# Fastaxx/Penguin.jl

Hardware: AMD Instinct MI355X
Metric: time-steps/sec + SpMV GB/s (% HBM roofline), 3D mono diffusion 512^3 (higher is better)
Workload: dtype f64

## Files before the change

### penguin/jl_amd/csrc/pg_common.h

```cpp
#pragma once
#include <hip/hip_runtime.h>
#include "pg_rccl.h"

#include <chrono>
#include <cstdint>
#include <cstdio>
#include <cstring>
#include <stdexcept>
#include <string>
#include <vector>

#include "../../../include/penguin_hip.h"

namespace pg {

using i64 = int64_t;
using i32 = int32_t;

struct Error : std::runtime_error {
  using std::runtime_error::runtime_error;
};

void set_last_error(const std::string& msg);

#define PG_HIP(expr)                                                                              \
  do {                                                                                            \
    hipError_t _e = (expr);                                                                       \
    if (_e != hipSuccess)                                                                         \
      throw pg::Error(std::string("HIP error: ") + hipGetErrorString(_e) + " at " + __FILE__ + ":" + \
                      std::to_string(__LINE__) + " (" #expr ")");                                 \
  } while (0)

#define PG_NCCL(expr)                                                                             \
  do {                                                                                            \
    ncclResult_t _e = (expr);                                                                     \
    if (_e != ncclSuccess)                                                                        \
      throw pg::Error(std::string("RCCL error: ") + pg::rccl::api().GetErrorString(_e) + " at " + __FILE__ + ":" + \
                      std::to_string(__LINE__) + " (" #expr ")");                                 \
  } while (0)

#define PG_REQUIRE(cond, msg)                                   \
  do {                                                          \
    if (!(cond)) throw pg::Error(std::string(msg));             \
  } while (0)

#define PG_API_BEGIN try {
#define PG_API_END                                  \
  return 0;                                         \
  }                                                 \
  catch (const std::exception& e) {                 \
    pg::set_last_error(e.what());                   \
    return 1;                                       \
  }                                                 \
  catch (...) {                                     \
    pg::set_last_error("unknown exception");        \
    return 2;                                       \
  }

struct Config {
  bool debug = false;
  int alloc_poison = 0;
  int async_alloc = 0;
  int alloc_guard = 0;
  long long pool_limit_mb = 0;
  bool poly = true;
  int poly_degree = 6;
  bool poly_adapt = true;
  double poly_margin = 1.0;
  double poly_slack = -1.0;
  int poly_hist = 3;
  bool poly_trend = true;
  int poly_maxdeg = 0;
  int poly_mindeg = 4;
  bool poly_f32 = true;
  int poly_f32_tail = -1;
  int profile_sample = 3;
  bool gamma_elim = true;
  bool diag_elim = true;
  double diag_elim_frac = 0.0005;
  int spmv_variant = 70;
  int spmv_xcd = 1;
  int spmv_strip = 16;
  int spmv_march_k = 0;
  int spmv_minrun = 24;
  bool spmv_march = true;
  bool spmv_edges = true;
  int spmv_tile_units = 0;
  int spmv_blocks_per_cu = 0;
  bool halo_overlap = true;
  int guess_n = 4;
  int guess_depth = 7;
  bool guess_defer = true;
  bool guess_always = false;
  int guess_monitor = 256;
  double guess_pass_cost = 0.34;
  double guess_gain = 0.8;
  bool speculate_product = true;
  int mg_tail_rows = 2048;
  int unit_order = 0;
};
const Config& config();

struct LocalComm;

struct Context {
  bool inited = false;
  LocalComm* local = nullptr;
  int device = 0;
  hipStream_t stream = nullptr;
  hipStream_t comm_stream = nullptr;
  hipEvent_t ev_fork = nullptr, ev_join = nullptr;
  int rank = 0, nranks = 1;
  ncclComm_t comm = nullptr;
  ncclComm_t comm_halo = nullptr;
  bool profiling = false;
  std::string device_name;
};
Context& ctx();
void require_init();
void set_thread_context(Context* c);
Context* thread_context();
LocalComm* local_comm_create(int nranks);
void local_comm_destroy(LocalComm* c);
void comm_allreduce_sum_f64(double* dev, int count, hipStream_t st);
void comm_allreduce_max_f64(double* dev, int count, hipStream_t st);
void comm_allreduce_sum_u64(unsigned long long* dev, i64 count, hipStream_t st);

void* dev_alloc(size_t bytes);
void dev_free(void* p);
void dev_cache_release();
struct AsyncAllocScope {
  AsyncAllocScope();
  ~AsyncAllocScope();
};

template <class T>
struct DevBuf {
  T* p = nullptr;
  i64 n = 0;
  DevBuf() = default;
  explicit DevBuf(i64 n_) { alloc(n_); }
  DevBuf(const DevBuf&) = delete;
  DevBuf& operator=(const DevBuf&) = delete;
  DevBuf(DevBuf&& o) noexcept : p(o.p), n(o.n) { o.p = nullptr; o.n = 0; }
  DevBuf& operator=(DevBuf&& o) noexcept {
    if (this != &o) { release(); p = o.p; n = o.n; o.p = nullptr; o.n = 0; }
    return *this;
  }
  ~DevBuf() { release(); }
  void release() {
    if (p) dev_free(p);
    p = nullptr; n = 0;
  }
  void alloc(i64 n_) {
    release();
    n = n_;
    if (n > 0) p = static_cast<T*>(dev_alloc(sizeof(T) * static_cast<size_t>(n) + 64));
  }
  void zero() {
    if (n > 0) PG_HIP(hipMemsetAsync(p, 0, sizeof(T) * static_cast<size_t>(n), ctx().stream));
  }
  void upload(const T* h, i64 count, i64 offset = 0) {
    if (count > 0) {
      PG_HIP(hipMemcpyAsync(p + offset, h, sizeof(T) * static_cast<size_t>(count), hipMemcpyHostToDevice, ctx().stream));
      PG_HIP(hipStreamSynchronize(ctx().stream));
    }
  }
  void download(T* h, i64 count, i64 offset = 0) const {
    if (count > 0) {
      PG_HIP(hipMemcpyAsync(h, p + offset, sizeof(T) * static_cast<size_t>(count), hipMemcpyDeviceToHost, ctx().stream));
      PG_HIP(hipStreamSynchronize(ctx().stream));
    }
  }
};

inline void* pinned_scratch(int slot, size_t bytes) {
  static thread_local void* buf[2] = {nullptr, nullptr};
  static thread_local size_t cap[2] = {0, 0};
  if (bytes > cap[slot]) {
    if (buf[slot]) (void)hipHostFree(buf[slot]);
    PG_HIP(hipHostMalloc(&buf[slot], bytes + (bytes >> 2)));
    cap[slot] = bytes + (bytes >> 2);
  }
  return buf[slot];
}

struct Laps {
  bool on;
  std::chrono::steady_clock::time_point t0;
  explicit Laps() : on(config().debug), t0(std::chrono::steady_clock::now()) {}
  void lap(const char* what) {
    if (!on) return;
    (void)hipDeviceSynchronize();
    const auto t1 = std::chrono::steady_clock::now();
    fprintf(stderr, "[pg_laps] %-34s %8.2f ms\n", what, std::chrono::duration<double, std::milli>(t1 - t0).count());
    t0 = t1;
  }
};

struct EventPair {
  hipEvent_t e0 = nullptr, e1 = nullptr;
  EventPair() {
    PG_HIP(hipEventCreate(&e0));
    if (hipEventCreate(&e1) != hipSuccess) {
      (void)hipEventDestroy(e0);
      throw Error("hipEventCreate failed");
    }
  }
  ~EventPair() {
    if (e0) (void)hipEventDestroy(e0);
    if (e1) (void)hipEventDestroy(e1);
  }
  EventPair(const EventPair&) = delete;
  EventPair& operator=(const EventPair&) = delete;
};

inline int grid_for(i64 n, int block, int cap = 256 * 8) {
  i64 g = (n + block - 1) / block;
  if (g < 1) g = 1;
  if (g > cap) g = cap;
  return static_cast<int>(g);
}

constexpr int CAP_HALO = 3;

struct Slab {
  int N = 0;
  i64 n[3] = {1, 1, 1};
  i64 ext[3] = {1, 1, 1};
  i64 stride[3] = {1, 1, 1};
  i64 plane = 1;
  i64 nplanes = 1;
  i64 M = 1;
  i64 p0 = 0, p1 = 1;
  i64 s0 = 0, s1 = 1;
  i64 Mloc() const { return (s1 - s0) * plane; }
  i64 first_cell() const { return s0 * plane; }
  void set_own(i64 a, i64 b) {
    p0 = a; p1 = b;
    s0 = p0 - CAP_HALO; if (s0 < 0) s0 = 0;
    s1 = p1 + CAP_HALO; if (s1 > nplanes) s1 = nplanes;
  }
};

}

struct pg_mesh {
  int N = 0;
  pg::i64 n[3] = {1, 1, 1};
// ... 29 lines not shown
```

### penguin/jl_amd/csrc/pg_context.hip

```cpp
#include "pg_common.h"

#include <cxxabi.h>
#include <execinfo.h>

#include <atomic>
#include <map>
#include <mutex>
#include <unordered_map>
#include <unordered_set>
#include "pg_host_algos.h"

#include <algorithm>
#include <array>
#include <memory>
#include <set>

namespace pg {

static thread_local std::string g_last_error;
void set_last_error(const std::string& msg) { g_last_error = msg; }

Context& ctx() {
  static Context c;
  Context* t = thread_context();
  return t ? *t : c;
}

const Config& config() {
  static const Config c = [] {
    Config k;
    auto geti = [](const char* name, long long dflt) { const char* v = getenv(name); return v ? atoll(v) : dflt; };
    auto getd = [](const char* name, double dflt) { const char* v = getenv(name); return v ? atof(v) : dflt; };
    k.debug = getenv("PG_DEBUG") != nullptr;
    k.alloc_poison = (int)geti("PG_ALLOC_POISON", 0);
    k.async_alloc = (int)geti("PG_ASYNC_ALLOC", 0);
    k.alloc_guard = (int)geti("PG_ALLOC_GUARD", 0);
    k.pool_limit_mb = geti("PG_POOL_LIMIT_MB", 0);
    k.poly = geti("PG_POLY", 1) != 0;
    k.poly_degree = (int)geti("PG_POLY_DEGREE", 6);
    k.poly_adapt = geti("PG_POLY_ADAPT", getenv("PG_POLY_DEGREE") ? 0 : 1) != 0;
    k.poly_margin = getd("PG_POLY_MARGIN", 1.0);
    k.poly_slack = getd("PG_POLY_SLACK", -1.0);
    k.poly_hist = (int)std::max<long long>(1, std::min<long long>(3, geti("PG_POLY_HIST", 3)));
    k.poly_maxdeg = (int)geti("PG_POLY_MAXDEG", 0);
    k.poly_mindeg = (int)std::max<long long>(2, std::min<long long>(8, geti("PG_POLY_MINDEG", 4)));
    k.poly_trend = geti("PG_POLY_TREND", 1) != 0;
    k.poly_f32 = geti("PG_POLY_F32", 1) != 0;
    k.poly_f32_tail = (int)std::max<long long>(-1, std::min<long long>(64, geti("PG_POLY_F32_TAIL", -1)));
    k.profile_sample = (int)std::max<long long>(1, geti("PG_PROFILE_SAMPLE", 3));
    k.gamma_elim = geti("PG_GAMMA_ELIM", 1) != 0;
    k.diag_elim = geti("PG_DIAG_ELIM", 1) != 0;
    k.diag_elim_frac = getd("PG_DIAG_ELIM_FRAC", 0.0005);
    k.spmv_variant = (int)geti("PG_SPMV_VARIANT", 70);
    k.spmv_xcd = (int)geti("PG_SPMV_XCD", 1);
    k.spmv_strip = (int)geti("PG_SPMV_STRIP", 16);
    k.spmv_march_k = (int)geti("PG_SPMV_MARCH_K", 0);
    k.spmv_minrun = (int)geti("PG_SPMV_MINRUN", 24);
    k.spmv_march = geti("PG_SPMV_MARCH", 1) != 0;
    k.spmv_edges = geti("PG_SPMV_EDGES", 1) != 0;
    k.spmv_tile_units = (int)geti("PG_SPMV_TILE_UNITS", 0);
    k.spmv_blocks_per_cu = (int)geti("PG_SPMV_BLOCKS_PER_CU", 0);
    k.halo_overlap = geti("PG_HALO_OVERLAP", 1) != 0;
    k.speculate_product = geti("PG_SPECULATE", 1) != 0;
    k.guess_n = (int)std::max<long long>(0, std::min<long long>(4, geti("PG_GUESS_STATES", 4)));
    k.guess_depth = (int)std::max<long long>(1, std::min<long long>(7, geti("PG_GUESS_DEPTH", 7)));
    k.mg_tail_rows = (int)std::max<long long>(0, geti("PG_MG_TAIL_ROWS", 2048));
    k.guess_monitor = (int)std::max<long long>(1, geti("PG_GUESS_MONITOR", 256));
    k.guess_pass_cost = getd("PG_GUESS_PASS_COST", 0.34);
    k.guess_always = geti("PG_GUESS_ALWAYS", 0) != 0;
    k.guess_defer = geti("PG_GUESS_DEFER", 1) != 0;
    k.guess_gain = getd("PG_GUESS_GAIN", 0.8);
    k.unit_order = (int)geti("PG_SPMV_UNIT_ORDER", 0);
    return k;
  }();
  return c;
}

void require_init() {
  if (!ctx().inited)
    throw Error("penguin_hip: not initialised (call pg_init / pg_init_distributed first)");
}

static void init_device(int device_id) {
  Context& c = ctx();
  int ndev = 0;
  hipError_t e = hipGetDeviceCount(&ndev);
  if (e != hipSuccess || ndev <= 0)
    throw Error("penguin_hip: no HIP device visible -- this library has no CPU fallback");
  PG_REQUIRE(device_id >= 0 && device_id < ndev, "penguin_hip: device id out of range");
  PG_HIP(hipSetDevice(device_id));
  hipDeviceProp_t prop;
  PG_HIP(hipGetDeviceProperties(&prop, device_id));
  c.device = device_id;
  c.device_name = std::string(prop.name) + " (" + prop.gcnArchName + ")";
  if (!c.stream) PG_HIP(hipStreamCreateWithFlags(&c.stream, hipStreamNonBlocking));
  if (!c.comm_stream) PG_HIP(hipStreamCreateWithFlags(&c.comm_stream, hipStreamNonBlocking));
  c.inited = true;
}

}

using namespace pg;

namespace pg {
namespace {
thread_local int t_async_scope = 0;
std::mutex g_alloc_mutex;
struct BlockCache {
  std::multimap<size_t, void*> free_blocks;
  std::unordered_map<void*, size_t> owned;
  size_t free_bytes = 0;
};
BlockCache g_cache;
constexpr size_t CACHE_TRIM_BYTES = (size_t)48 << 30;

size_t round_block(size_t bytes) {
  const size_t q = bytes >= ((size_t)2 << 20) ? ((size_t)2 << 20) : 4096;
  return (bytes + q - 1) / q * q;
}

bool cache_wanted(const Context& c, size_t bytes) {
  const int mode = config().async_alloc;
  if (mode < 0 || !c.inited || !c.stream || c.local) return false;
  if (!(t_async_scope > 0 || mode > 0)) return false;
  const long long lim = config().pool_limit_mb;
  return lim <= 0 || bytes < ((size_t)lim << 20);
}

void poison(void* p, size_t bytes) {
  if (!config().alloc_poison || !p || bytes == 0) return;
  Context& c = ctx();
  if (c.inited && c.stream) PG_HIP(hipMemsetAsync(p, 0xFF, bytes, c.stream));
  else PG_HIP(hipMemset(p, 0xFF, bytes));
}

void cache_trim_locked() {
  if (g_cache.free_blocks.empty()) return;
  (void)hipDeviceSynchronize();
  for (auto& kv : g_cache.free_blocks) {
    g_cache.owned.erase(kv.second);
    (void)hipFree(kv.second);
  }
  g_cache.free_blocks.clear();
  g_cache.free_bytes = 0;
}

void* dev_alloc_raw(size_t bytes) {
  void* p = nullptr;
  Context& c = ctx();
  if (cache_wanted(c, bytes)) {
    const size_t want = round_block(bytes);
    {
      std::lock_guard<std::mutex> lk(g_alloc_mutex);
      auto it = g_cache.free_blocks.lower_bound(want);
      if (it != g_cache.free_blocks.end() && it->first <= want + want / 8) {
        p = it->second;
        g_cache.free_bytes -= it->first;
        g_cache.free_blocks.erase(it);
      }
    }
    if (!p) {
      if (hipMalloc(&p, want) != hipSuccess || !p) {
        (void)hipGetLastError();
        { std::lock_guard<std::mutex> lk(g_alloc_mutex); cache_trim_locked(); }
        PG_HIP(hipMalloc(&p, want));
      }
      std::lock_guard<std::mutex> lk(g_alloc_mutex);
      g_cache.owned[p] = want;
    }
    poison(p, bytes);
    return p;
  }
  PG_HIP(hipMalloc(&p, bytes));
  poison(p, bytes);
  return p;
}

void dev_free_raw(void* p) {
  if (!p) return;
  {
    std::lock_guard<std::mutex> lk(g_alloc_mutex);
    auto it = g_cache.owned.find(p);
    if (it != g_cache.owned.end()) {
      g_cache.free_blocks.emplace(it->second, p);
      g_cache.free_bytes += it->second;
      if (g_cache.free_bytes > CACHE_TRIM_BYTES) cache_trim_locked();
      return;
    }
  }
  (void)hipFree(p);
}

constexpr size_t GUARD = 4096;
struct GuardInfo { char* raw; size_t bytes; unsigned long long seq; std::string where; };
std::unordered_map<void*, GuardInfo> g_guarded;
unsigned long long g_alloc_seq = 0;
std::string call_stack() {
  void* frames[24];
  const int nf = backtrace(frames, 24);
  char** sym = backtrace_symbols(frames, nf);
  std::string s;
  for (int i = 2; sym && i < nf && i < 12; ++i) {
    std::string f = sym[i];
    const size_t a = f.find('('), b = f.find('+', a == std::string::npos ? 0 : a);
    if (a != std::string::npos && b != std::string::npos && b > a + 1) {
      std::string mangled = f.substr(a + 1, b - a - 1);
      int st = 0;
      char* dem = abi::__cxa_demangle(mangled.c_str(), nullptr, nullptr, &st);
      f = st == 0 && dem ? dem : mangled;
      free(dem);
      const size_t par = f.find('(');
      if (par != std::string::npos) f = f.substr(0, par);
    }
    s += (s.empty() ? "" : " <- ") + f;
  }
  free(sym);
  return s;
}
}

AsyncAllocScope::AsyncAllocScope() { ++t_async_scope; }
AsyncAllocScope::~AsyncAllocScope() { --t_async_scope; }

void dev_cache_release() {
  std::lock_guard<std::mutex> lk(g_alloc_mutex);
  cache_trim_locked();
}

void* dev_alloc(size_t bytes) {
  if (!config().alloc_guard) return dev_alloc_raw(bytes);
  char* raw = static_cast<char*>(dev_alloc_raw(bytes + 2 * GUARD));
  Context& c = ctx();
  hipStream_t st = (c.inited && c.stream) ? c.stream : nullptr;
  PG_HIP(hipMemsetAsync(raw, 0xA5, GUARD, st));
  PG_HIP(hipMemsetAsync(raw + GUARD + bytes, 0xA5, GUARD, st));
  void* user = raw + GUARD;
  std::lock_guard<std::mutex> lk(g_alloc_mutex);
  g_guarded[user] = GuardInfo{raw, bytes, ++g_alloc_seq, call_stack()};
  return user;
}

void dev_free(void* p) {
  if (!config().alloc_guard) { dev_free_raw(p); return; }
  GuardInfo gi;
  {
    std::lock_guard<std::mutex> lk(g_alloc_mutex);
    auto it = g_guarded.find(p);
    if (it == g_guarded.end()) { gi.raw = nullptr; }
    else { gi = it->second; g_guarded.erase(it); }
  }
  if (!gi.raw) { dev_free_raw(p); return; }
  (void)hipDeviceSynchronize();
  std::vector<unsigned char> lo(GUARD), hi(GUARD);
  (void)hipMemcpy(lo.data(), gi.raw, GUARD, hipMemcpyDeviceToHost);
  (void)hipMemcpy(hi.data(), gi.raw + GUARD + gi.bytes, GUARD, hipMemcpyDeviceToHost);
  auto first_bad = [](const std::vector<unsigned char>& g, bool from_end) -> long {
    if (from_end) { for (long i = (long)g.size() - 1; i >= 0; --i) if (g[i] != 0xA5) return i; }
    else { for (size_t i = 0; i < g.size(); ++i) if (g[i] != 0xA5) return (long)i; }
    return -1;
  };
  const long bl = first_bad(lo, true), bh = first_bad(hi, false);
  if (bl >= 0 || bh >= 0) {
    long nl = 0, nh = 0;
    for (unsigned char v : lo) nl += v != 0xA5;
    for (unsigned char v : hi) nh += v != 0xA5;
    fprintf(stderr, "[pg_alloc] GUARD DAMAGED: block #%llu of %zu bytes (incl. 64 of slack): %ld bytes written BELOW it (nearest %ld bytes "
            "before the start), %ld bytes written ABOVE it (first %ld bytes past the end); allocated by: %s\n", gi.seq, gi.bytes, nl,
            bl >= 0 ? (long)GUARD - bl : 0, nh, bh >= 0 ? bh : 0, gi.where.c_str());
  }
  dev_free_raw(gi.raw);
}
}

extern "C" {

int32_t pg_last_error(char* buf, size_t n) {
  if (buf && n > 0) {
    std::strncpy(buf, g_last_error.c_str(), n - 1);
    buf[n - 1] = 0;
  }
  return 0;
}

int32_t pg_init(int32_t device_id) {
  PG_API_BEGIN
  Context& c = ctx();
  init_device(device_id);
  c.rank = 0;
  c.nranks = 1;
  PG_API_END
}

int32_t pg_get_unique_id(void* out128) {
  PG_API_BEGIN
  static_assert(sizeof(ncclUniqueId) == 128, "ncclUniqueId is expected to be 128 bytes");
  ncclUniqueId id;
  PG_NCCL(rccl::api().GetUniqueId(&id));
  std::memcpy(out128, &id, sizeof(id));
  PG_API_END
}

int32_t pg_init_distributed(int32_t device_id, int32_t rank, int32_t nranks, const void* unique_id128) {
  PG_API_BEGIN
  Context& c = ctx();
  PG_REQUIRE(nranks >= 1 && rank >= 0 && rank < nranks, "pg_init_distributed: bad rank / nranks");
  init_device(device_id);
  c.rank = rank;
  c.nranks = nranks;
  if (nranks > 1 || unique_id128 != nullptr) {
    PG_REQUIRE(unique_id128 != nullptr, "pg_init_distributed: unique id required when nranks > 1");
    ncclUniqueId id;
    std::memcpy(&id, unique_id128, sizeof(id));
    const rccl::Api& R = rccl::api();
    PG_NCCL(R.CommInitRank(&c.comm, nranks, id, rank));
    bool split_ok = false;
    if (R.CommSplit) {
      split_ok = R.CommSplit(c.comm, 0, rank, &c.comm_halo, nullptr) == ncclSuccess && c.comm_halo != nullptr;
      if (!split_ok) c.comm_halo = nullptr;
    }
    if (!split_ok) {
      ncclUniqueId id2;
      if (rank == 0) PG_NCCL(R.GetUniqueId(&id2));
      DevBuf<char> buf((i64)sizeof(id2));
      if (rank == 0) buf.upload(reinterpret_cast<const char*>(&id2), (i64)sizeof(id2));
      PG_NCCL(R.Broadcast(buf.p, buf.p, sizeof(id2), ncclChar, 0, c.comm, c.stream));
      buf.download(reinterpret_cast<char*>(&id2), (i64)sizeof(id2));
      PG_NCCL(R.CommInitRank(&c.comm_halo, nranks, id2, rank));
    }
  }
  PG_API_END
}

int32_t pg_finalize(void) {
  PG_API_BEGIN
  Context& c = ctx();
  if (c.inited) {
    (void)hipDeviceSynchronize();
    if (c.comm_halo) { (void)rccl::api().CommDestroy(c.comm_halo); c.comm_halo = nullptr; }
    if (c.comm) { (void)rccl::api().CommDestroy(c.comm); c.comm = nullptr; }
    dev_cache_release();
    if (c.stream) { (void)hipStreamDestroy(c.stream); c.stream = nullptr; }
    if (c.comm_stream) { (void)hipStreamDestroy(c.comm_stream); c.comm_stream = nullptr; }
    if (c.ev_fork) { (void)hipEventDestroy(c.ev_fork); c.ev_fork = nullptr; }
    if (c.ev_join) { (void)hipEventDestroy(c.ev_join); c.ev_join = nullptr; }
    c.inited = false;
  }
  PG_API_END
}

int32_t pg_device_synchronize(void) {
  PG_API_BEGIN
  require_init();
  PG_HIP(hipDeviceSynchronize());
  PG_API_END
}

int32_t pg_set_profiling(int32_t on) {
  PG_API_BEGIN
  ctx().profiling = on != 0;
  PG_API_END
}

int32_t pg_config_string(char* buf, size_t n) {
  PG_API_BEGIN
  const Config& k = config();
  char tmp[1024];
  snprintf(tmp, sizeof(tmp),
           "spmv_variant=%d spmv_xcd=%d spmv_strip=%d spmv_unit_order=%d spmv_march=%d spmv_edges=%d spmv_march_k=%d spmv_minrun=%d spmv_tile_units=%d "
           "spmv_blocks_per_cu=%d halo_overlap=%d speculate=%d poly=%d poly_degree=%d poly_adapt=%d "
           "poly_margin=%g poly_slack=%g poly_hist=%d poly_trend=%d poly_maxdeg=%d poly_f32=%d poly_f32_tail=%d gamma_elim=%d diag_elim=%d "
           "guess_states=%d guess_depth=%d guess_defer=%d async_alloc=%d cache_limit_mb=%lld alloc_poison=%d alloc_guard=%d profile_sample=%d debug=%d",
           k.spmv_variant, k.spmv_xcd, k.spmv_strip, k.unit_order, (int)k.spmv_march, (int)k.spmv_edges, k.spmv_march_k, k.spmv_minrun, k.spmv_tile_units,
           k.spmv_blocks_per_cu, (int)k.halo_overlap, (int)k.speculate_product, (int)k.poly, k.poly_degree, (int)k.poly_adapt,
           k.poly_margin, k.poly_slack, k.poly_hist, (int)k.poly_trend, k.poly_maxdeg, (int)k.poly_f32, k.poly_f32_tail,
           (int)k.gamma_elim, (int)k.diag_elim, k.guess_n, k.guess_depth, (int)k.guess_defer, k.async_alloc, k.pool_limit_mb, k.alloc_poison, k.alloc_guard, k.profile_sample, (int)k.debug);
  if (buf && n > 0) {
    std::strncpy(buf, tmp, n - 1);
    buf[n - 1] = 0;
  }
  PG_API_END
}

int32_t pg_device_name(char* buf, size_t n) {
  PG_API_BEGIN
  require_init();
  if (buf && n > 0) {
    std::strncpy(buf, ctx().device_name.c_str(), n - 1);
    buf[n - 1] = 0;
  }
  PG_API_END
}

int32_t pg_mesh_create(int32_t N, const int64_t* n, const double* L, const double* x0, pg_mesh** out) {
  PG_API_BEGIN
  PG_REQUIRE(N >= 1 && N <= 3, "pg_mesh_create: N must be 1, 2 or 3");
  PG_REQUIRE(out != nullptr, "pg_mesh_create: out is NULL");
  PG_REQUIRE(n != nullptr && L != nullptr, "pg_mesh_create: n / L is NULL");
  std::unique_ptr<pg_mesh> guard(new pg_mesh());
  pg_mesh* m = guard.get();
  m->N = N;
  for (int d = 0; d < N; ++d) {
    PG_REQUIRE(n[d] >= 1, "pg_mesh_create: n_d must be >= 1");
    m->n[d] = n[d];
    m->L[d] = L[d];
    m->x0[d] = x0 ? x0[d] : 0.0;
    const double h = L[d] / static_cast<double>(n[d]);
    m->centers[d].resize(n[d]);
    m->nodes[d].resize(n[d] + 1);
    for (i64 j = 0; j < n[d]; ++j) m->centers[d][j] = m->x0[d] + static_cast<double>(j) * h;
    for (i64 j = 0; j <= n[d]; ++j) m->nodes[d][j] = m->x0[d] + (static_cast<double>(j) + 0.5) * h;
  }
  if (ctx().inited) {
    for (int d = 0; d < N; ++d) {
      m->d_nodes[d].alloc(n[d] + 1);
      m->d_nodes[d].upload(m->nodes[d].data(), n[d] + 1);
    }
  }
  *out = guard.release();
  PG_API_END
}

int32_t pg_mesh_destroy(pg_mesh* m) {
  PG_API_BEGIN
  delete m;
  PG_API_END
}

int32_t pg_mesh_get_centers(const pg_mesh* m, int32_t d, double* out, int64_t len) {
  PG_API_BEGIN
  PG_REQUIRE(m && d >= 0 && d < m->N && len == m->n[d], "pg_mesh_get_centers: bad arguments");
  std::memcpy(out, m->centers[d].data(), sizeof(double) * len);
  PG_API_END
}

int32_t pg_mesh_get_nodes(const pg_mesh* m, int32_t d, double* out, int64_t len) {
  PG_API_BEGIN
  PG_REQUIRE(m && d >= 0 && d < m->N && len == m->n[d] + 1, "pg_mesh_get_nodes: bad arguments");
  std::memcpy(out, m->nodes[d].data(), sizeof(double) * len);
  PG_API_END
}

int32_t pg_mesh_num_border_cells(const pg_mesh* m, int64_t* out) {
  PG_API_BEGIN
  PG_REQUIRE(m && out, "pg_mesh_num_border_cells: bad arguments");
  i64 all = 1, inner = 1;
  for (int d = 0; d < m->N; ++d) {
    all *= m->n[d];
    inner *= std::max<i64>(m->n[d] - 2, 0);
  }
  *out = all - inner;
  PG_API_END
}

int32_t pg_mesh_get_border_cells(const pg_mesh* mc, int64_t* idx, double* pos, int32_t* key) {
  PG_API_BEGIN
  PG_REQUIRE(mc, "pg_mesh_get_border_cells: mesh is NULL");
  pg_mesh* m = const_cast<pg_mesh*>(mc);
  mesh_build_border(m);
  const size_t nb = m->border_key.size();
  if (idx) std::memcpy(idx, m->border_idx.data(), sizeof(i64) * nb * m->N);
  if (pos) std::memcpy(pos, m->border_pos.data(), sizeof(double) * nb * m->N);
  if (key) std::memcpy(key, m->border_key.data(), sizeof(i32) * nb);
  PG_API_END
}

int32_t pg_partition_planes(const int64_t* weight, int64_t nplanes, int32_t nranks, int64_t* bounds) {
  PG_API_BEGIN
  PG_REQUIRE(weight && bounds && nplanes >= 1 && nranks >= 1, "pg_partition_planes: bad arguments");
  PG_REQUIRE(nplanes >= nranks, "pg_partition_planes: fewer planes than ranks");
  pghost::partition_planes(weight, nplanes, nranks, bounds);
  PG_API_END
}

int32_t pg_slab_numbering_host(int32_t K, int64_t plane, int64_t nplanes, int64_t p0, int64_t p1, const uint8_t* active,
                               int64_t* out) {
  PG_API_BEGIN
  PG_REQUIRE(K >= 1 && K <= pghost::SLAB_MAX_KINDS && plane >= 1 && nplanes >= 1 && p0 >= 0 && p1 > p0 && p1 <= nplanes && active && out,
             "pg_slab_numbering_host: bad arguments");
  const pghost::SlabPlanes g = pghost::slab_planes(p0, p1, nplanes, CAP_HALO);
  const i64 Mloc = (g.s1 - g.s0) * plane;
  const i64 lcA0 = (g.a0 - g.s0) * plane, lcA1 = (g.a1 - g.s0) * plane;
  const i64 lcO = (p0 - g.s0) * plane, lcU = (p1 - g.s0) * plane, lcFE = (p0 + 1 - g.s0) * plane, lcLB = (p1 - 1 - g.s0) * plane;
  i64 posO[pghost::SLAB_MAX_KINDS], posU[pghost::SLAB_MAX_KINDS], posFE[pghost::SLAB_MAX_KINDS], posLB[pghost::SLAB_MAX_KINDS],
      tot[pghost::SLAB_MAX_KINDS];
  for (int k = 0; k < K; ++k) {
    i64 c = 0;
    posO[k] = posU[k] = posFE[k] = posLB[k] = -1;
    for (i64 lc = 0; lc <= Mloc; ++lc) {
      if (lc == lcO) posO[k] = c;
      if (lc == lcU) posU[k] = c;
      if (lc == lcFE) posFE[k] = c;
      if (lc == lcLB) posLB[k] = c;
      if (lc < Mloc && lc >= lcA0 && lc < lcA1 && active[(i64)k * Mloc + lc]) ++c;
    }
    tot[k] = c;
  }
  pghost::SlabNumbering sn;
  pghost::slab_numbering(K, posO, posU, posFE, posLB, tot, p0 > 0, p1 < nplanes, sn);
  i64 q = 0;
  out[q++] = sn.n_own;
  out[q++] = sn.n_ghost;
  const i64* arrays[10] = {sn.cnt_own, sn.off_own, sn.cntL, sn.offL, sn.cntU, sn.offU, sn.sendL_off, sn.sendL_cnt, sn.sendU_off, sn.sendU_cnt};
  for (const i64* a : arrays)
    for (int k = 0; k < K; ++k) out[q++] = a[k];
  PG_API_END
}

}

namespace pg {

void mesh_build_border(pg_mesh* m) {
  if (m->border_built) return;
  const int N = m->N;
  std::vector<i64>& bi = m->border_idx;
  std::set<std::array<i64, 3>> seen;
  auto emit = [&](i64 i0, i64 i1, i64 i2) {
    std::array<i64, 3> key{i0, i1, i2};
    if (!seen.insert(key).second) return;
    const i64 id[3] = {i0, i1, i2};
    for (int d = 0; d < N; ++d) {
      bi.push_back(id[d] + 1);
      m->border_pos.push_back(m->centers[d][id[d]]);
    }
    m->border_key.push_back(border_key_of(N, m->n, i0, i1, i2));
  };
  for (int d = 0; d < N; ++d) {
    const i64 faces[2] = {0, m->n[d] - 1};
// ... 32 lines not shown
```

### penguin/jl_amd/csrc/pg_precond.hip

```cpp
#include "pg_scan.h"
#include "pg_system.h"

using namespace pg;

namespace {

struct RowSegs {
  int K;
  i64 off_own[MAX_KINDS];
};

__device__ inline int row_kind_of(const RowSegs& s, i64 r) {
  int k = 0;
  while (k + 1 < s.K && r >= s.off_own[k + 1]) ++k;
  return k;
}

constexpr int NSLOT = 7;

__device__ inline int slot_of(const CapView& c, i64 lc, i64 cl) {
  if (cl == lc) return 0;
  for (int d = 0; d < c.N; ++d) {
    if (cl == lc + c.stride[d]) return 1 + 2 * d;
    if (cl == lc - c.stride[d]) return 2 + 2 * d;
// ... 164 lines not shown
    for (int a = 0; a < MAX_KINDS; ++a) {
      blk_idx[q * MAX_KINDS + a] = a < cb.nk ? cb.rows[a] : -1;
      blk_coef[q * MAX_KINDS + a] = a < cb.nk ? cb.binv[me][a] * cb.dsk[a] : 0.0;
      blk_fw[q * MAX_KINDS + a] = a < cb.nk ? cb.bfw[me][a] : 0.0;
      double cn = 0.0;
      if (a < cb.nk) {
        if (P.nphase == 1) cn = a == me ? 1.0 : 0.0;
        else
          for (int j = 0; j < cb.nk; ++j)
            if ((cb.kinds[j] & 1) == 0) cn += cb.binv[me][j] * cb.bfw[j][a];
      }
      blk_cn[q * MAX_KINDS + a] = cn;
    }
  }
}

__global__ void k_count_ghost_refs(i64 nnz, i64 n_own, const int* __restrict__ col, unsigned long long* __restrict__ out) {
  unsigned long long c = 0;
  for (i64 k = blockIdx.x * (i64)blockDim.x + threadIdx.x; k < nnz; k += (i64)gridDim.x * blockDim.x) c += col[k] >= n_own ? 1 : 0;
  if (c) atomicAdd(out, c);
}

__global__ void k_gershgorin(i64 n, const int* __restrict__ rowptr, const int* __restrict__ col,
                             const double* __restrict__ val, const double* __restrict__ ds, double* __restrict__ out) {
  double worst = 0.0;
  for (i64 r = blockIdx.x * (i64)blockDim.x + threadIdx.x; r < n; r += (i64)gridDim.x * blockDim.x) {
    const int a = rowptr[r], b = rowptr[r + 1];
    if (b - a <= 1) {
      const double d = b > a && col[a] == r ? fabs(1.0 - val[a]) : 1.0;
      worst = d > worst ? d : worst;
      continue;
    }
    double diag = 0.0, off = 0.0;
    for (int k = a; k < b; ++k) {
      const int c = col[k];
      if (c == r) { diag = val[k]; continue; }
      if (c < n && rowptr[c + 1] - rowptr[c] == 1 && col[rowptr[c]] == c) continue;
      off += fabs(val[k]) * (ds[r] / ds[c]);
    }
    const double rad = fabs(1.0 - diag) + off;
    worst = rad > worst ? rad : worst;
  }
  for (int o = 32; o > 0; o >>= 1) {
    const double other = __shfl_down(worst, o, 64);
    worst = other > worst ? other : worst;
  }
  if ((threadIdx.x & 63) == 0)
    atomicMax(reinterpret_cast<unsigned long long*>(out), (unsigned long long)__double_as_longlong(worst));
}

__global__ void k_pl_simple(i64 n, const double* __restrict__ ds, const double* __restrict__ in, double* __restrict__ out) {
  for (i64 r = blockIdx.x * (i64)blockDim.x + threadIdx.x; r < n; r += (i64)gridDim.x * blockDim.x) out[r] = ds[r] * in[r];
}

__global__ void k_pl_block(i64 nblk, const int* __restrict__ blk_rows, const int* __restrict__ blk_idx,
                           const double* __restrict__ blk_coef, const double* __restrict__ in, double* __restrict__ out) {
  for (i64 q = blockIdx.x * (i64)blockDim.x + threadIdx.x; q < nblk; q += (i64)gridDim.x * blockDim.x) {
    double s = 0.0;
#pragma unroll
    for (int a = 0; a < MAX_KINDS; ++a) {
      const int j = blk_idx[q * MAX_KINDS + a];
      if (j >= 0) s += blk_coef[q * MAX_KINDS + a] * in[j];
    }
    out[blk_rows[q]] = s;
  }
}

__global__ void k_point_scale(SysParams P, int K, i64 Mloc, const int* red, double* ds) {
  const CapView& c = P.cap[0];
  const i64 total = (i64)K * Mloc;
  for (i64 q = blockIdx.x * (i64)blockDim.x + threadIdx.x; q < total; q += (i64)gridDim.x * blockDim.x) {
    const int r = red[q];
    if (r < 0) continue;
    const int k = (int)(q / Mloc);
    const i64 lc = q % Mloc;
    i64 idx[3];
    decode_cell(c.N, c.ext, c.plane, c.s0, lc, idx);
    double diag = 0.0, rowmax = 0.0;
    eval_row(P, k, lc, idx, [&](int ck, i64 cl, double v) {
      if (ck == k && cl == lc) diag = v;
      rowmax = fmax(rowmax, fabs(v));
    });
    const double a = fabs(diag);
    ds[r] = (a > 1e-13 * rowmax && a < 1e300) ? 1.0 / sqrt(a) : 1.0;
  }
}

}

namespace pg {

static void set_geo(CsrMatrix& A, const Slab& slab, const Numbering& nb) {
  A.geo_cell = nb.row_cell.p;
  A.geo_map = nullptr;
  A.geo_ext0 = slab.N == 3 ? slab.ext[0] : 0;
  A.geo_lines = slab.N == 3 ? slab.ext[1] : 0;
}

void assemble_csr_preconditioned(const SysParams& P, const Slab& s, const Numbering& nb, CsrMatrix& A,
                                 const bool* inherit_halo) {
  hipStream_t st = ctx().stream;
  Laps laps;
  const i64 n = nb.n_own;
  A.n = n;
  A.rowptr.alloc(n + 1);
  A.ds.alloc(nb.n_vec() > 0 ? nb.n_vec() : 1);
  A.n_blk = 0;
  A.halo_needed = true;
  RowSegs seg;
  seg.K = nb.K;
  for (int k = 0; k < MAX_KINDS; ++k) seg.off_own[k] = nb.off_own[k];
  if (n == 0) {
    A.rowptr.zero();
    A.nnz = 0;
    if (inherit_halo) A.halo_needed = *inherit_halo;
    else if (ctx().nranks > 1) {
      DevBuf<unsigned long long> nref(1);
      nref.zero();
      comm_allreduce_sum_u64(nref.p, 1, st);
      unsigned long long h = 0;
      nref.download(&h, 1);
      A.halo_needed = h != 0;
    }
    decide_poly(A);
    return;
  }
  hipLaunchKernelGGL(k_point_scale, dim3(grid_for((i64)nb.K * nb.Mloc, 256, 256 * 16)), dim3(256), 0, st, P, nb.K, nb.Mloc,
                     nb.red.p, A.ds.p);
  PG_HIP(hipGetLastError());
  DevBuf<int> cnt(n);
  A.isblk.alloc(n);
  DevBuf<unsigned char>& isblk = A.isblk;
  DevBuf<unsigned long long> nraw(1);
  nraw.zero();
  const int gr = grid_for(n, 256, 256 * 16);
  hipLaunchKernelGGL(HIP_KERNEL_NAME(k_asm_p<false>), dim3(gr), dim3(256), 0, st, P, seg, nb.Mloc, n, nb.row_cell.p, nb.red.p,
                     A.ds.p, cnt.p, isblk.p, nraw.p, (const int*)nullptr, (int*)nullptr, (double*)nullptr);
  PG_HIP(hipGetLastError());
  scan_exclusive<int>(cnt.p, A.rowptr.p, n, A.rowptr.p + n, st);
  int nnz = 0;
  A.rowptr.download(&nnz, 1, n);
  PG_REQUIRE(nnz >= 0, "nnz overflow");
  A.nnz = nnz;
  unsigned long long hraw = 0;
  nraw.download(&hraw, 1);
  A.nnz_raw = (i64)hraw;
  A.col.alloc(nnz + 8);
  A.val.alloc(nnz + 8);
  A.col.zero();
  A.val.zero();
  hipLaunchKernelGGL(HIP_KERNEL_NAME(k_asm_p<true>), dim3(gr), dim3(256), 0, st, P, seg, nb.Mloc, n, nb.row_cell.p, nb.red.p,
                     A.ds.p, (int*)nullptr, (unsigned char*)nullptr, (unsigned long long*)nullptr, (const int*)A.rowptr.p, A.col.p, A.val.p);
  PG_HIP(hipGetLastError());
  DevBuf<int> pos(n), total(1);
  scan_exclusive<unsigned char>(isblk.p, pos.p, n, total.p, st);
  int nblk = 0;
  total.download(&nblk, 1);
  A.n_blk = nblk;
  A.blk_rows.alloc(nblk > 0 ? nblk : 1);
  A.blk_idx.alloc((i64)MAX_KINDS * (nblk > 0 ? nblk : 1));
  A.blk_coef.alloc((i64)MAX_KINDS * (nblk > 0 ? nblk : 1));
  A.blk_cn.alloc((i64)MAX_KINDS * (nblk > 0 ? nblk : 1));
  A.blk_fw.alloc((i64)MAX_KINDS * (nblk > 0 ? nblk : 1));
  if (nblk > 0) {
    hipLaunchKernelGGL(k_blk_table, dim3(gr), dim3(256), 0, st, P, seg, nb.Mloc, n, nb.row_cell.p, nb.red.p, A.ds.p, isblk.p,
                       pos.p, A.blk_rows.p, A.blk_idx.p, A.blk_coef.p, A.blk_cn.p, A.blk_fw.p);
    PG_HIP(hipGetLastError());
  }
  PG_HIP(hipStreamSynchronize(st));
  if (inherit_halo) A.halo_needed = *inherit_halo;
  else if (ctx().nranks > 1) {
    DevBuf<unsigned long long> nref(1);
    nref.zero();
    hipLaunchKernelGGL(k_count_ghost_refs, dim3(grid_for(nnz, 256, 4096)), dim3(256), 0, st, (i64)nnz, n, A.col.p, nref.p);
    PG_HIP(hipGetLastError());
    comm_allreduce_sum_u64(nref.p, 1, st);
    unsigned long long h = 0;
    nref.download(&h, 1);
    A.halo_needed = h != 0;
    if (config().debug)
      fprintf(stderr, "[pg_precond] rank %d: %llu ghost-column references over all ranks => halo %s\n", ctx().rank, h,
              A.halo_needed ? "exchanged" : "skipped");
  }
  laps.lap("  asm: count/fill/table kernels");
  set_geo(A, s, nb);
  build_spmv_chunks(A);
  laps.lap("  asm: SpMV chunks + slices");
  decide_poly(A);
}

__global__ void k_structure_differs(i64 n, const int* __restrict__ cnt, const int* __restrict__ rowptr,
                                    const unsigned char* __restrict__ blk_a, const unsigned char* __restrict__ blk_b,
                                    unsigned long long* __restrict__ out) {
  unsigned long long c = 0;
  for (i64 r = blockIdx.x * (i64)blockDim.x + threadIdx.x; r < n; r += (i64)gridDim.x * blockDim.x)
    c += (cnt[r] != rowptr[r + 1] - rowptr[r] || blk_a[r] != blk_b[r]) ? 1 : 0;
  if (c) atomicAdd(out, c);
}

void assemble_csr_like(const SysParams& P, const Slab& s, const Numbering& nb, const CsrMatrix& T, CsrMatrix& A) {
  hipStream_t st = ctx().stream;
  Laps laps;
  const i64 n = nb.n_own;
  const bool halo = T.halo_needed;
  if (n == 0 || T.n != n || !T.rowptr.p) {
    assemble_csr_preconditioned(P, s, nb, A, &halo);
    return;
  }
  RowSegs seg;
  seg.K = nb.K;
  for (int k = 0; k < MAX_KINDS; ++k) seg.off_own[k] = nb.off_own[k];
  A.n = n;
  A.ds.alloc(nb.n_vec() > 0 ? nb.n_vec() : 1);
  hipLaunchKernelGGL(k_point_scale, dim3(grid_for((i64)nb.K * nb.Mloc, 256, 256 * 16)), dim3(256), 0, st, P, nb.K, nb.Mloc,
                     nb.red.p, A.ds.p);
  PG_HIP(hipGetLastError());
  DevBuf<int> cnt(n);
  A.isblk.alloc(n);
  DevBuf<unsigned long long> nraw(2);
  nraw.zero();
  const int gr = grid_for(n, 256, 256 * 16);
  hipLaunchKernelGGL(HIP_KERNEL_NAME(k_asm_p<false>), dim3(gr), dim3(256), 0, st, P, seg, nb.Mloc, n, nb.row_cell.p, nb.red.p,
                     A.ds.p, cnt.p, A.isblk.p, nraw.p, (const int*)nullptr, (int*)nullptr, (double*)nullptr);
  hipLaunchKernelGGL(k_structure_differs, dim3(grid_for(n, 256, 4096)), dim3(256), 0, st, n, cnt.p, T.rowptr.p, A.isblk.p,
                     T.isblk.p, nraw.p + 1);
  PG_HIP(hipGetLastError());
  unsigned long long h[2] = {0, 0};
  nraw.download(h, 2);
  if (h[1] != 0) {
    assemble_csr_preconditioned(P, s, nb, A, &halo);
    return;
  }
  A.nnz = T.nnz;
  A.nnz_raw = (i64)h[0];
  A.halo_needed = halo;
  A.rowptr.alloc(n + 1);
  PG_HIP(hipMemcpyAsync(A.rowptr.p, T.rowptr.p, sizeof(int) * (n + 1), hipMemcpyDeviceToDevice, st));
  A.col.alloc(A.nnz + 8);
  A.val.alloc(A.nnz + 8);
  A.col.zero();
  A.val.zero();
  hipLaunchKernelGGL(HIP_KERNEL_NAME(k_asm_p<true>), dim3(gr), dim3(256), 0, st, P, seg, nb.Mloc, n, nb.row_cell.p, nb.red.p,
                     A.ds.p, (int*)nullptr, (unsigned char*)nullptr, (unsigned long long*)nullptr, (const int*)A.rowptr.p, A.col.p, A.val.p);
  PG_HIP(hipGetLastError());
  const i64 nblk = T.n_blk, nb1 = nblk > 0 ? nblk : 1;
  A.n_blk = nblk;
  A.blk_rows.alloc(nb1);
  A.blk_idx.alloc((i64)MAX_KINDS * nb1);
  A.blk_coef.alloc((i64)MAX_KINDS * nb1);
  A.blk_cn.alloc((i64)MAX_KINDS * nb1);
  A.blk_fw.alloc((i64)MAX_KINDS * nb1);
  if (nblk > 0) {
    DevBuf<int> pos(n), total(1);
    scan_exclusive<unsigned char>(A.isblk.p, pos.p, n, total.p, st);
    hipLaunchKernelGGL(k_blk_table, dim3(gr), dim3(256), 0, st, P, seg, nb.Mloc, n, nb.row_cell.p, nb.red.p, A.ds.p, A.isblk.p,
                       pos.p, A.blk_rows.p, A.blk_idx.p, A.blk_coef.p, A.blk_cn.p, A.blk_fw.p);
    PG_HIP(hipGetLastError());
    PG_HIP(hipStreamSynchronize(st));
  }
  laps.lap("  asm-like: values on the ctor matrix' pattern");
  set_geo(A, s, nb);
  if (!build_slices_like(T, A)) build_spmv_chunks(A);
  laps.lap("  asm-like: slices");
  decide_poly(A);
}

void decide_poly(CsrMatrix& A) {
  hipStream_t st = ctx().stream;
  DevBuf<double> worst(1);
  worst.zero();
  if (A.n > 0) {
    hipLaunchKernelGGL(k_gershgorin, dim3(grid_for(A.n, 256, 4096)), dim3(256), 0, st, A.n, A.rowptr.p, A.col.p, A.val.p, A.ds.p,
                       worst.p);
    PG_HIP(hipGetLastError());
  }
  comm_allreduce_max_f64(worst.p, 1, st);
  double h = 0.0;
  worst.download(&h, 1);
  A.gersh = h;
  A.est = SpecEst();
  A.poly_gave_up = false;
  A.poly_ok = h < 0.95;
  if (config().debug && !(h < 1e300) && A.n > 0) {
    std::vector<int> rp(A.n + 1), cl(A.nnz);
    std::vector<double> vl(A.nnz), dsv(A.ds.n);
    A.rowptr.download(rp.data(), A.n + 1); A.col.download(cl.data(), A.nnz); A.val.download(vl.data(), A.nnz);
    A.ds.download(dsv.data(), A.ds.n);
    int shown = 0;
    for (i64 r = 0; r < A.n && shown < 4; ++r) {
      bool bad = !(dsv[r] > 0.0) || !(dsv[r] < 1e300);
      for (int k = rp[r]; k < rp[r + 1]; ++k) bad = bad || !(std::fabs(vl[k]) < 1e300);
      if (!bad) continue;
      ++shown;
      fprintf(stderr, "[pg_precond] row %lld: ds %.3e entries", (long long)r, dsv[r]);
      for (int k = rp[r]; k < rp[r + 1]; ++k) fprintf(stderr, " (%d: %.3e, ds %.3e)", cl[k], vl[k], dsv[cl[k]]);
      fprintf(stderr, "\n");
    }
  }
  if (config().debug)
    fprintf(stderr, "[pg_precond] rank %d: largest Gershgorin radius %.4f => Neumann preconditioner %s\n", ctx().rank, h,
            A.poly_ok ? "admissible" : "not used");
}

void apply_left(const CsrMatrix& A, const double* in, double* out, hipStream_t st) {
  if (A.n == 0) return;
  hipLaunchKernelGGL(k_pl_simple, dim3(grid_for(A.n, 256)), dim3(256), 0, st, A.n, A.ds.p, in, out);
  if (A.n_blk > 0)
    hipLaunchKernelGGL(k_pl_block, dim3(grid_for(A.n_blk, 256)), dim3(256), 0, st, A.n_blk, A.blk_rows.p, A.blk_idx.p,
                       A.blk_coef.p, in, out);
  PG_HIP(hipGetLastError());
}

}
```

### penguin/jl_amd/csrc/pg_solver.hip

```cpp
#include <algorithm>
#include <cmath>
#include <memory>

#include "pg_krylov.h"
#include "pg_reduce.h"
#include "pg_multigrid.h"
#include "pg_program.h"
#include "pg_scan.h"
#include "pg_solver_internal.h"
#include "pg_spmv.h"
#include "pg_specest.h"

using namespace pg;

namespace pg { extern double g_host_wait_us; }

struct pg_solver {
  int nphase = 1;
  pg_capacity* cap[2] = {nullptr, nullptr};
  pg_diffops* ops[2] = {nullptr, nullptr};
  Slab slab;
  int K = 2;
  i64 Mloc = 0, M = 0;
  double dt = 0.0, t = 0.0;
  int scheme_ctor = PG_SCHEME_BE;
  pg_bc_desc bc_i{};
  pg_jump_desc ic{};
  int border_kind[6] = {0, 0, 0, 0, 0, 0};
  double border_value[6] = {0, 0, 0, 0, 0, 0};
  double inv_dx = 0.0;
  DevBuf<double> Id[2];
  DevBuf<double> f_n[2], f_np1[2];
  DevBuf<double> g_n, g_np1;
  DevBuf<double> g_arr, h_arr;
  Numbering nb;
  CsrMatrix A_ctor, A_run;
  GammaElim elim_ctor, elim_run;
  DiagElim diag_ctor, diag_run;
  bool have_run = false;
  int scheme_run = -1;
  DevBuf<double> mass, bconst, bcv;
  DevBuf<unsigned char> fixed;
  int bconst_scheme = -1;
  bool bconst_dirty = true;
  long long bconst_version = 0;
  struct TdSlot {
    int K = 0;
    i64 nrows = 0;
    DevBuf<double> mode[PG_TD_MAX_TERMS];
    std::vector<double> coef;
    struct Prog {
      pg_program prog;
      int key = -1;
      i64 n = 0;
      DevBuf<int> row;
      DevBuf<double> w, p[3];
      i64 nrows = 0;
      std::vector<double> times;
    };
    std::vector<Prog> progs;
    bool empty() const { return K == 0 && progs.empty(); }
  };
  TdSlot td[4];
  DevBuf<double> td_base;
  int td_base_scheme = -1;
  i64 td_cursor = 0;
  i64 td_row = -1;
  DevBuf<double> blk_wz, blk_c0;
  const CsrMatrix* blk_cache_matrix = nullptr;
  int blk_cache_scheme = -1;
  long long blk_cache_version = -1;
  DevBuf<double> x, b, y;
  DevBuf<double> z, ysol;
  bool x_valid = true;
  const CsrMatrix* z_matrix = nullptr;
  DevBuf<double> T0pad;
  KrylovWork work;
  MgHierarchy mg;
  MgHierarchy mg_cell;
  bool spec_y_valid = false, spec_pending = false, hint_more_steps = false;
  const CsrMatrix* spec_matrix = nullptr;
  DevBuf<double> zh[8], yh[8], guess_coef, guess_partials;
  DevBuf<unsigned> guess_ticket;
  int hist_cnt = 0, hist_k = 0;
  bool plain_guess_on[2] = {false, false};
  double plain_last_products[2] = {0.0, 0.0};
  const void* hist_de = nullptr;
  bool initial_done = false;
  std::vector<DevBuf<double>> states;
  i64 steps_done = 0;
  DevBuf<double> red_scratch;
  DevBuf<i64> border_cells_lin;
  bool moving = false;
  DevBuf<double> psi_p[2], psi_m[2];
  bool advdiff = false;
  bool convection = false;
  DevBuf<double> psi_cp[2], psi_cm[2];
  bool stefan = false;
  bool solved_once = false;
  pg_solver* init_from = nullptr;
  struct Monitors {
    int K = 0;
    int kind[PG_MON_MAX] = {};
    bool sparse[PG_MON_MAX] = {};
    i64 stored[PG_MON_MAX] = {};
    DevBuf<double> w[PG_MON_MAX];
    DevBuf<int> row[PG_MON_MAX];
    int G = 0;
    DevBuf<double> series;
    i64 rows = 0, cap = 0;
    std::vector<double> times;
  };
  Monitors mon;
  MgHierarchy mg_step[2];
};

namespace {

using pg::BLOCK;

struct RowSegs {
  int K;
  i64 off_own[MAX_KINDS];
};

__device__ inline int seg_kind(const RowSegs& s, i64 r) {
  int k = 0;
  while (k + 1 < s.K && r >= s.off_own[k + 1]) ++k;
  return k;
}

RowSegs make_segs(const Numbering& nb) {
  RowSegs s;
  s.K = nb.K;
  for (int k = 0; k < MAX_KINDS; ++k) s.off_own[k] = nb.off_own[k];
  return s;
}

struct KeyVals {
  double v[6];
};

__global__ void k_row_static(SysParams P, RowSegs seg, i64 n_own, const int* row_cell, KeyVals kv, double* mass,
                             unsigned char* fixed, double* bcv) {
  const CapView& c = P.cap[0];
  for (i64 r = blockIdx.x * (i64)blockDim.x + threadIdx.x; r < n_own; r += (i64)gridDim.x * blockDim.x) {
    const int k = seg_kind(seg, r);
    const i64 lc = row_cell[r];
    i64 idx[3];
    decode_cell(c.N, c.ext, c.plane, c.s0, lc, idx);
    double m = 0.0, bv = 0.0;
    unsigned char fx = 0;
    if ((k & 1) == 0) {
      const int ph = k >> 1;
      int key = -1;
      const int bk = border_row_kind(P, ph, lc, idx, &key);
      if (bk != PG_BC_NONE) {
        fx = 1;
        bv = (bk == PG_BC_PERIODIC) ? 0.0 : kv.v[key];
      } else {
        m = P.mv_psi_w[0] ? P.mv_v1[ph][lc] : P.mass * P.cap[ph].V[lc];
      }
    } else if (P.nphase == 2) {
      fx = 1;
    }
    mass[r] = m;
    fixed[r] = fx;
    bcv[r] = bv;
  }
}

struct SrcView {
  const double* f_n[2];
  const double* f_np1[2];
  const double* g_n;
  const double* g_np1;
  double g_const, h_const;
};

__global__ void k_bconst(SysParams P, RowSegs seg, i64 n_own, const int* row_cell, SrcView s, int scheme, double dt,
                         const unsigned char* fixed, const double* bcv, double* bconst, int moving) {
  for (i64 r = blockIdx.x * (i64)blockDim.x + threadIdx.x; r < n_own; r += (i64)gridDim.x * blockDim.x) {
    const int k = seg_kind(seg, r);
    const i64 lc = row_cell[r];
    const int ph = k >> 1;
    double v;
    if ((k & 1) == 0) {
      if (fixed[r]) v = bcv[r];
      else {
        const double V = P.cap[ph].V[lc];
        const double f1 = s.f_np1[ph] ? s.f_np1[ph][lc] : 0.0;
        if (scheme == PG_SCHEME_CN) {
          const double f0 = s.f_n[ph] ? s.f_n[ph][lc] : f1;
          v = dt / 2 * V * (f0 + f1);
        } else {
          v = dt * V * f1;
        }
      }
    } else if (P.nphase == 1) {
      const double G = P.cap[0].G[lc];
      const double g1 = s.g_np1 ? s.g_np1[lc] : s.g_const;
      if (scheme == PG_SCHEME_CN && !moving) {
        const double g0 = s.g_n ? s.g_n[lc] : s.g_const;
        v = dt / 2 * G * (g0 + g1);
      } else {
        v = G * g1;
      }
    } else if (k == 1 || P.mv_stefan) {
      v = s.g_n ? s.g_n[lc] : s.g_const;
    } else {
      v = P.cap[1].G[lc] * (s.g_np1 ? s.g_np1[lc] : s.h_const);
    }
    bconst[r] = v;
  }
}

__global__ void k_rhs(i64 n, int scheme, const double* __restrict__ x, const double* __restrict__ yhat,
                      const double* __restrict__ ds, const double* __restrict__ mass, const double* __restrict__ bconst,
                      const unsigned char* __restrict__ fixed, double* __restrict__ b) {
  for (i64 r = blockIdx.x * (i64)blockDim.x + threadIdx.x; r < n; r += (i64)gridDim.x * blockDim.x) {
    double v;
    if (fixed[r]) v = ds[r] * bconst[r];
    else if (scheme == PG_SCHEME_CN) v = ds[r] * (2.0 * (mass[r] * x[r]) + bconst[r]) - yhat[r];
    else v = ds[r] * (mass[r] * x[r] + bconst[r]);
    b[r] = v;
  }
}

__global__ void k_rhs_block(i64 nblk, int scheme, const int* __restrict__ blk_rows, const int* __restrict__ blk_idx,
                            const double* __restrict__ blk_coef, const double* __restrict__ blk_cn,
                            const double* __restrict__ x, const double* __restrict__ ds, const double* __restrict__ yhat,
                            const double* __restrict__ mass, const double* __restrict__ bconst,
                            const unsigned char* __restrict__ fixed, double* __restrict__ b) {
  const double fac = scheme == PG_SCHEME_CN ? 2.0 : 1.0;
  for (i64 q = blockIdx.x * (i64)blockDim.x + threadIdx.x; q < nblk; q += (i64)gridDim.x * blockDim.x) {
    double v = 0.0;
#pragma unroll
    for (int a = 0; a < MAX_KINDS; ++a) {
      const int j = blk_idx[q * MAX_KINDS + a];
      if (j < 0) continue;
      const double xj = ds ? ds[j] * x[j] : x[j];
      const double cj = fixed[j] ? bconst[j] : fac * (mass[j] * xj) + bconst[j];
      v += blk_coef[q * MAX_KINDS + a] * cj;
      if (scheme == PG_SCHEME_CN) v -= blk_cn[q * MAX_KINDS + a] * yhat[j];
    }
    b[blk_rows[q]] = v;
  }
}

__global__ void k_blk_cache(i64 nblk, int scheme, const int* __restrict__ blk_idx, const double* __restrict__ blk_coef,
                            const double* __restrict__ ds, const double* __restrict__ mass, const double* __restrict__ bconst,
                            const unsigned char* __restrict__ fixed, double* __restrict__ wz, double* __restrict__ c0) {
  const double fac = scheme == PG_SCHEME_CN ? 2.0 : 1.0;
  for (i64 q = blockIdx.x * (i64)blockDim.x + threadIdx.x; q < nblk; q += (i64)gridDim.x * blockDim.x) {
    double c = 0.0;
#pragma unroll
    for (int a = 0; a < MAX_KINDS; ++a) {
      const int j = blk_idx[q * MAX_KINDS + a];
      double w = 0.0;
      if (j >= 0) {
        const double cf = blk_coef[q * MAX_KINDS + a];
        c += cf * bconst[j];
        if (!fixed[j]) w = cf * (fac * (mass[j] * ds[j]));
      }
      wz[q * MAX_KINDS + a] = w;
    }
    c0[q] = c;
  }
}

__global__ void k_rhs_block_c(i64 nblk, int scheme, const int* __restrict__ blk_rows, const int* __restrict__ blk_idx,
                              const double* __restrict__ wz, const double* __restrict__ c0, const double* __restrict__ blk_cn,
                              const double* __restrict__ z, const double* __restrict__ yhat, double* __restrict__ b) {
  for (i64 q = blockIdx.x * (i64)blockDim.x + threadIdx.x; q < nblk; q += (i64)gridDim.x * blockDim.x) {
    int j[MAX_KINDS];
    double zz[MAX_KINDS], yy[MAX_KINDS];
#pragma unroll
    for (int a = 0; a < MAX_KINDS; ++a) j[a] = blk_idx[q * MAX_KINDS + a];
#pragma unroll
    for (int a = 0; a < MAX_KINDS; ++a) {
      zz[a] = j[a] >= 0 ? z[j[a]] : 0.0;
      yy[a] = (j[a] >= 0 && scheme == PG_SCHEME_CN) ? yhat[j[a]] : 0.0;
    }
    double v = c0[q];
#pragma unroll
    for (int a = 0; a < MAX_KINDS; ++a) v += wz[q * MAX_KINDS + a] * zz[a] - (scheme == PG_SCHEME_CN ? blk_cn[q * MAX_KINDS + a] * yy[a] : 0.0);
    b[blk_rows[q]] = v;
  }
}

__global__ void k_rhs_block_mf(SysParams P, RowSegs seg, i64 Mloc, i64 nblk, const int* __restrict__ blk_rows,
                               const int* __restrict__ blk_idx, const double* __restrict__ blk_coef,
                               const int* __restrict__ row_cell, const int* __restrict__ red, const double* __restrict__ ds,
                               const double* __restrict__ z, const double* __restrict__ mass, const double* __restrict__ bconst,
                               const unsigned char* __restrict__ fixed, double* __restrict__ b) {
  const CapView& c = P.cap[0];
  for (i64 q = blockIdx.x * (i64)blockDim.x + threadIdx.x; q < nblk; q += (i64)gridDim.x * blockDim.x) {
    const i64 lc = row_cell[blk_rows[q]];
    i64 idx[3];
    decode_cell(c.N, c.ext, c.plane, c.s0, lc, idx);
    double v = 0.0;
    for (int a = 0; a < MAX_KINDS; ++a) {
      const int j = blk_idx[q * MAX_KINDS + a];
      if (j < 0) continue;
      const int k = seg_kind(seg, j);
      double ca;
      if (fixed[j]) {
        ca = bconst[j];
      } else {
        double ax = 0.0;
        eval_row(P, k, lc, idx, [&](int ck, i64 cl, double val) {
          const int col = red[(i64)ck * Mloc + cl];
          if (val != 0.0 && col >= 0) ax += val * (ds[col] * z[col]);
        });
        ca = 2.0 * (mass[j] * (ds[j] * z[j])) + bconst[j] - ax;
      }
      v += blk_coef[q * MAX_KINDS + a] * ca;
    }
    b[blk_rows[q]] = v;
  }
}

struct GuessArgs {
  const double* zr[8];
  const double* yr[8];
  double* znew;
  double* coef;
  int defer;
};
constexpr int GUESS_USED = 64;

__device__ inline const double* ring_pick(const double* const (&r)[8], int i) {
  const double* p = r[0];
#pragma unroll
  for (int q = 1; q < 8; ++q) p = i == q ? r[q] : p;
  return p;
}

typedef double rd2_t __attribute__((ext_vector_type(2)));
typedef unsigned char ruc2_t __attribute__((ext_vector_type(2)));

__device__ inline void rhs_init_one(int scheme, double z, double yh, double d, double ms, double bc, bool fx, bool blk, double bold,
                                    double& bi, double& ri) {
  if (blk) bi = bold;
  else if (fx) bi = d * bc;
  else if (scheme == PG_SCHEME_CN) bi = d * (2.0 * (ms * (d * z)) + bc) - yh;
  else bi = d * (ms * (d * z) + bc);
  ri = bi - yh;
}

template <int KH>
__global__ __launch_bounds__(BLOCK) void k_rhs_init(i64 n, i64 nvec, int scheme, const double* __restrict__ z,
                                                    const double* __restrict__ yhat, const double* __restrict__ ds,
                                                    const double* __restrict__ mass, const double* __restrict__ bconst,
                                                    const unsigned char* __restrict__ fixed,
                                                    const unsigned char* __restrict__ isblk, double* __restrict__ b,
                                                    double* __restrict__ r, double* __restrict__ rhat,
                                                    double* __restrict__ p, double* __restrict__ partials, GuessArgs g) {
  __shared__ double s_red[BLOCK / 64];
  double acc = 0.0, accb = 0.0, accw = 0.0;
  double cj[KH > 0 ? KH : 1];
  const double* zo[KH > 0 ? KH : 1];
  const double* yo[KH > 0 ? KH : 1];
  int ku = 0;
  if (KH > 0) {
    ku = min(KH, (int)g.coef[4]);
#pragma unroll
    for (int j = 0; j < KH; ++j) {
      const int sel = j < ku ? (int)g.coef[5 + j] : 0;
      cj[j] = j < ku ? g.coef[j] : 0.0;
      zo[j] = ring_pick(g.zr, sel);
      yo[j] = ring_pick(g.yr, sel);
    }
    if (blockIdx.x == 0 && threadIdx.x == 0) g.coef[13] += (double)ku;
  }
  const i64 npair = (nvec + 1) / 2;
  for (i64 q = blockIdx.x * (i64)BLOCK + threadIdx.x; q < npair; q += (i64)gridDim.x * BLOCK) {
    const i64 i = 2 * q;
    if (i + 1 < n) {
      const rd2_t yh = __builtin_nontemporal_load(reinterpret_cast<const rd2_t*>(yhat + i));
      const rd2_t d = __builtin_nontemporal_load(reinterpret_cast<const rd2_t*>(ds + i));
      const rd2_t bc = __builtin_nontemporal_load(reinterpret_cast<const rd2_t*>(bconst + i));
      const rd2_t ms = __builtin_nontemporal_load(reinterpret_cast<const rd2_t*>(mass + i));
      const rd2_t zz = *reinterpret_cast<const rd2_t*>(z + i);
      const ruc2_t fx = *reinterpret_cast<const ruc2_t*>(fixed + i);
      const ruc2_t bk = *reinterpret_cast<const ruc2_t*>(isblk + i);
      rd2_t bold;
      bold.x = 0.0; bold.y = 0.0;
      if (bk.x | bk.y) bold = *reinterpret_cast<const rd2_t*>(b + i);
      double b0, r0, b1, r1;
      rhs_init_one(scheme, zz.x, yh.x, d.x, ms.x, bc.x, fx.x != 0, bk.x != 0, bold.x, b0, r0);
      rhs_init_one(scheme, zz.y, yh.y, d.y, ms.y, bc.y, fx.y != 0, bk.y != 0, bold.y, b1, r1);
      if (KH > 0) {
        rd2_t zg = zz;
#pragma unroll
        for (int j = 0; j < KH; ++j) {
          if (j < ku) {
            const rd2_t a = *reinterpret_cast<const rd2_t*>(zo[j] + i);
            const rd2_t y2 = *reinterpret_cast<const rd2_t*>(yo[j] + i);
            r0 -= cj[j] * (y2.x - yh.x); r1 -= cj[j] * (y2.y - yh.y);
            zg.x += cj[j] * (a.x - zz.x); zg.y += cj[j] * (a.y - zz.y);
          }
        }
        *reinterpret_cast<rd2_t*>(g.znew + i) = zg;
      }
      rd2_t bi, ri;
      bi.x = b0; bi.y = b1; ri.x = r0; ri.y = r1;
      __builtin_nontemporal_store(bi, reinterpret_cast<rd2_t*>(b + i));
      *reinterpret_cast<rd2_t*>(r + i) = ri;
      *reinterpret_cast<rd2_t*>(rhat + i) = ri;
      *reinterpret_cast<rd2_t*>(p + i) = ri;
      acc += ri.x * ri.x + ri.y * ri.y;
      accb += (d.x * bi.x) * (d.x * bi.x) + (d.y * bi.y) * (d.y * bi.y);
      accw += (d.x * ri.x) * (d.x * ri.x) + (d.y * ri.y) * (d.y * ri.y);
    } else {
      for (i64 k = i; k < i + 2 && k < nvec; ++k) {
        if (k < n) {
          double bi, ri;
          rhs_init_one(scheme, z[k], yhat[k], ds[k], mass[k], bconst[k], fixed[k] != 0, isblk[k] != 0, isblk[k] ? b[k] : 0.0, bi, ri);
          if (KH > 0) {
            double zg = z[k];
#pragma unroll
            for (int j = 0; j < KH; ++j)
              if (j < ku) { ri -= cj[j] * (yo[j][k] - yhat[k]); zg += cj[j] * (zo[j][k] - z[k]); }
            g.znew[k] = zg;
          }
          b[k] = bi;
          r[k] = ri; rhat[k] = ri; p[k] = ri;
          acc += ri * ri;
          accb += (ds[k] * bi) * (ds[k] * bi);
          accw += (ds[k] * ri) * (ds[k] * ri);
        } else {
          p[k] = 0.0;
        }
      }
    }
  }
  const double t = block_sum(acc, s_red);
  if (threadIdx.x == 0) partials[blockIdx.x] = t;
  const double tb = block_sum(accb, s_red);
  if (threadIdx.x == 0) partials[gridDim.x + blockIdx.x] = tb;
  const double tw = block_sum(accw, s_red);
  if (threadIdx.x == 0) partials[2 * (size_t)gridDim.x + blockIdx.x] = tw;
}

template <int KH>
__global__ __launch_bounds__(BLOCK) void k_rhs_init_c(i64 n, int scheme, const double* z,
                                                      const double* __restrict__ yhat, const double* __restrict__ ds,
                                                      const double* __restrict__ mass, const double* __restrict__ bconst,
                                                      const unsigned char* __restrict__ fixed,
                                                      const unsigned char* __restrict__ isblk, const int* __restrict__ cmap,
                                                      double* __restrict__ b, const double* __restrict__ gdiag,
                                                      double* __restrict__ delta, int* __restrict__ flag, int stamp,
                                                      double* __restrict__ rhat, double* __restrict__ partials,
                                                      unsigned* __restrict__ ticket, double* __restrict__ sc, double reltol2,
                                                      double abstol2, int coupled, GuessArgs g) {
  __shared__ double s_red[BLOCK / 64];
  double acc = 0.0, accb = 0.0, accw = 0.0, acch = 0.0;
  const bool hold = ticket != nullptr;
  double cj[KH > 0 ? KH : 1];
  const double* zo[KH > 0 ? KH : 1];
  const double* yo[KH > 0 ? KH : 1];
  int ku = 0;
  const bool defer = KH > 0 && g.defer != 0;
  if (KH > 0) {
    ku = min(KH, (int)g.coef[4]);
#pragma unroll
    for (int j = 0; j < KH; ++j) {
      const int sel = j < ku ? (int)g.coef[5 + j] : 0;
      cj[j] = j < ku ? g.coef[j] : 0.0;
      zo[j] = ring_pick(g.zr, sel);
      yo[j] = ring_pick(g.yr, sel);
    }
    if (defer && blockIdx.x == 0 && threadIdx.x < 9) g.coef[GUESS_USED + threadIdx.x] = g.coef[threadIdx.x];
  }
  int moved = 0;
  double* zw = KH > 0 ? g.znew : const_cast<double*>(z);
  auto one = [&](i64 i, double zi, double yh, double d, double ms, double bc, bool fx, bool blk, double bold, int c, double& bi,
                 const double* zh, const double* yv) {
    double ri;
    rhs_init_one(scheme, zi, yh, d, ms, bc, fx, blk, bold, bi, ri);
    accb += (d * bi) * (d * bi);
    if (c >= 0) {
      if (KH > 0) {
        double zg = zi, corr = 0.0;
#pragma unroll
        for (int j = 0; j < KH; ++j) {
          corr += cj[j] * (yv[j] - yh);
          zg += cj[j] * (zh[j] - zi);
        }
        ri -= corr;
        if (!defer) zw[i] = zg;
      }
      rhat[c] = ri;
      acc += ri * ri;
      accw += (d * ri) * (d * ri);
    } else {
      const int e = -1 - c;
      double dl = ri / gdiag[e];
      const bool beyond = fabs(dl) > 1e-12 * fabs(zi);
      if (hold && !beyond) {
        acch += (d * ri) * (d * ri);
        dl = 0.0;
      }
      delta[e] = dl;
      if (KH > 0 || dl != 0.0) zw[i] = zi + dl;
      if (coupled ? dl != 0.0 : beyond) moved = 1;
    }
  };
  const i64 npair = (n + 1) / 2;
  for (i64 q = blockIdx.x * (i64)BLOCK + threadIdx.x; q < npair; q += (i64)gridDim.x * BLOCK) {
    const i64 i = 2 * q;
    double zh0[KH > 0 ? KH : 1], zh1[KH > 0 ? KH : 1], yv0[KH > 0 ? KH : 1], yv1[KH > 0 ? KH : 1];
    if (i + 1 < n) {
      const rd2_t yh = __builtin_nontemporal_load(reinterpret_cast<const rd2_t*>(yhat + i));
      const rd2_t d = __builtin_nontemporal_load(reinterpret_cast<const rd2_t*>(ds + i));
      const rd2_t bc = __builtin_nontemporal_load(reinterpret_cast<const rd2_t*>(bconst + i));
      const rd2_t ms = __builtin_nontemporal_load(reinterpret_cast<const rd2_t*>(mass + i));
      const rd2_t zz = *reinterpret_cast<const rd2_t*>(z + i);
      const ruc2_t fx = *reinterpret_cast<const ruc2_t*>(fixed + i);
      const ruc2_t bk = *reinterpret_cast<const ruc2_t*>(isblk + i);
      const int c0 = cmap[i], c1 = cmap[i + 1];
      if (KH > 0) {
#pragma unroll
        for (int j = 0; j < KH; ++j) {
          rd2_t a = zz, y2 = yh;
          if (j < ku && (c0 >= 0 || c1 >= 0)) {
            if (!defer) a = *reinterpret_cast<const rd2_t*>(zo[j] + i);
            y2 = *reinterpret_cast<const rd2_t*>(yo[j] + i);
          }
          zh0[j] = a.x; zh1[j] = a.y; yv0[j] = y2.x; yv1[j] = y2.y;
        }
      }
      rd2_t bold;
      bold.x = 0.0; bold.y = 0.0;
      if (bk.x | bk.y) bold = *reinterpret_cast<const rd2_t*>(b + i);
      rd2_t bi;
      double b0, b1;
      one(i, zz.x, yh.x, d.x, ms.x, bc.x, fx.x != 0, bk.x != 0, bold.x, c0, b0, zh0, yv0);
      one(i + 1, zz.y, yh.y, d.y, ms.y, bc.y, fx.y != 0, bk.y != 0, bold.y, c1, b1, zh1, yv1);
      bi.x = b0; bi.y = b1;
      __builtin_nontemporal_store(bi, reinterpret_cast<rd2_t*>(b + i));
    } else if (i < n) {
      const double zi = z[i], yh = yhat[i];
      if (KH > 0) {
#pragma unroll
        for (int j = 0; j < KH; ++j) {
          zh0[j] = (j < ku && !defer) ? zo[j][i] : zi;
          yv0[j] = j < ku ? yo[j][i] : yh;
        }
      }
      double b0;
      one(i, zi, yh, ds[i], mass[i], bconst[i], fixed[i] != 0, isblk[i] != 0, isblk[i] ? b[i] : 0.0, cmap[i], b0, zh0, yv0);
      b[i] = b0;
    }
  }
  if (__any(moved) && (threadIdx.x & 63) == 0) atomicMax(flag, stamp);
  const double t = block_sum(acc, s_red);
  const double tb = block_sum(accb, s_red);
  const double tw = block_sum(accw, s_red);
  if (!ticket) {
    if (threadIdx.x == 0) {
      partials[blockIdx.x] = t;
      partials[gridDim.x + blockIdx.x] = tb;
      partials[2 * (size_t)gridDim.x + blockIdx.x] = tw;
      if (KH > 0 && blockIdx.x == 0) g.coef[13] += (double)ku;
    }
    return;
  }
  if (threadIdx.x == 0) {
    pg::store_partial(partials + blockIdx.x, t);
    pg::store_partial(partials + gridDim.x + blockIdx.x, tb);
    pg::store_partial(partials + 2 * (size_t)gridDim.x + blockIdx.x, tw);
  }
  const double th = block_sum(acch, s_red);
  if (threadIdx.x == 0) pg::store_partial(partials + 3 * (size_t)gridDim.x + blockIdx.x, th);
  if (!pg::last_block_arrives(ticket, gridDim.x, s_red)) return;
  if (threadIdx.x < pg::S_COUNT) sc[threadIdx.x] = threadIdx.x == pg::S_RELTOL2 ? reltol2 : (threadIdx.x == pg::S_ABSTOL2 ? abstol2 : 0.0);
  __syncthreads();
  for (int sl = 0; sl < 4; ++sl) {
    double a = 0.0;
    for (int i = threadIdx.x; i < (int)gridDim.x; i += BLOCK) a += pg::load_partial(partials + (size_t)sl * gridDim.x + i);
    const double sum = block_sum(a, s_red);
    if (threadIdx.x == 0) sc[pg::S_RED0 + sl] = sum;
  }
  if (threadIdx.x == 0) {
    pg::derive(pg::PH_INIT, sc);
    sc[pg::S_MOVED] = __hip_atomic_load(flag, __ATOMIC_RELAXED, __HIP_MEMORY_SCOPE_AGENT) == stamp ? 1.0 : 0.0;
    const double held = sc[pg::S_RED0 + 3];
    if (held > 0.0) {
      if (2.0 * held >= sc[pg::S_TOL2]) sc[pg::S_MOVED] = 1.0;
      else {
        sc[pg::S_HELD] = held;
        sc[pg::S_TOL2] -= held;
        sc[pg::S_DONE] = sc[pg::S_RR] <= sc[pg::S_TOL2] ? 1.0 : 0.0;
      }
    }
    if (KH > 0) g.coef[13] += (double)ku;
  }
}

constexpr int GUESS_RM = 7;
constexpr int GUESS_NS = GUESS_RM * (GUESS_RM + 1) / 2 + GUESS_RM + 2;
struct GuessFit {
  const double* yr[8];
  double* partials;
  unsigned* ticket;
  double* coef;
  int stride, avail, kmax;
  double rate2, pass_cost, gain;
  double* sums;
};

__device__ inline int guess_tri(int j, int l) { return j * GUESS_RM - j * (j - 1) / 2 + (l - j); }

__device__ inline void guess_decide(const double* s_g, const GuessFit& f) {
  constexpr int RM = GUESS_RM, NS = GUESS_NS;
  __shared__ double s_left[128], s_net[128];
  __shared__ double s_c[128][4];
  const double ru = s_g[NS - 2], rw = s_g[NS - 1];
  if (threadIdx.x < 128) {
    const int mask = threadIdx.x, m = __popc(mask);
    double left = ru, cc[4] = {0.0, 0.0, 0.0, 0.0};
    if (mask != 0 && m <= f.kmax && m <= 4 && (mask >> f.avail) == 0 && ru > 0.0) {
      int idx[4] = {0, 0, 0, 0};
      for (int j = 0, a = 0; j < RM; ++j) if (mask >> j & 1) { if (a < 4) idx[a] = j; ++a; }
      double L[4][4], wv[4];
      bool ok = true;
#pragma unroll
      for (int a = 0; a < 4; ++a) {
        wv[a] = 0.0;
#pragma unroll
        for (int e = 0; e < 4; ++e) L[a][e] = 0.0;
      }
#pragma unroll
      for (int a = 0; a < 4; ++a) {
        if (a >= m || !ok) continue;
        const double g0 = s_g[guess_tri(idx[a], idx[a])];
        double dj = g0;
#pragma unroll
        for (int e = 0; e < 4; ++e) if (e < a) dj -= L[a][e] * L[a][e];
        if (!(g0 > 0.0) || !(dj > 1e-12 * g0)) { ok = false; continue; }
        const double lj = sqrt(dj);
        L[a][a] = lj;
#pragma unroll
        for (int l = 0; l < 4; ++l) {
          if (l <= a || l >= m) continue;
          double v = s_g[guess_tri(idx[a], idx[l])];
#pragma unroll
          for (int e = 0; e < 4; ++e) if (e < a) v -= L[l][e] * L[a][e];
          L[l][a] = v / lj;
        }
        double v = s_g[RM * (RM + 1) / 2 + idx[a]];
#pragma unroll
        for (int e = 0; e < 4; ++e) if (e < a) v -= L[a][e] * wv[e];
        wv[a] = v / lj;
        left -= wv[a] * wv[a];
      }
      if (ok) {
#pragma unroll
        for (int aa = 0; aa < 4; ++aa) {
          const int a = 3 - aa;
          if (a >= m) continue;
          double v = wv[a];
#pragma unroll
          for (int e = 0; e < 4; ++e) if (e > a && e < m) v -= L[e][a] * cc[e];
          cc[a] = v / L[a][a];
        }
#pragma unroll
        for (int a = 0; a < 4; ++a) ok = ok && isfinite(cc[a]) && fabs(cc[a]) < 256.0;
      }
      if (!ok) { left = ru; cc[0] = cc[1] = cc[2] = cc[3] = 0.0; }
      if (!(left > 1e-30 * ru)) left = 1e-30 * ru;
    }
    s_left[threadIdx.x] = left;
#pragma unroll
    for (int a = 0; a < 4; ++a) s_c[threadIdx.x][a] = cc[a];
    const bool live = ru > 0.0 && f.rate2 > 0.0 && rw <= ru * (1.0 + 1e-12) && left < ru;
    s_net[threadIdx.x] = live ? f.gain * log(ru / left) / f.rate2 - 2.0 * m * f.pass_cost : 0.0;
  }
  __syncthreads();
  if (threadIdx.x < 64) {
    int pick = threadIdx.x;
    double best = s_net[pick];
    if (s_net[pick + 64] > best) { best = s_net[pick + 64]; pick += 64; }
#pragma unroll
    for (int off = 32; off > 0; off >>= 1) {
      const double ob = __shfl_down(best, off, 64);
      const int op = __shfl_down(pick, off, 64);
      if (ob > best || (ob == best && op < pick)) { best = ob; pick = op; }
    }
    if (!(best > 0.0)) pick = 0;
    if (threadIdx.x != 0) return;
    int a = 0;
    for (int j = 0; j < RM; ++j)
      if (pick >> j & 1) { f.coef[a] = s_c[pick][a]; f.coef[5 + a] = (double)j; ++a; }
    f.coef[4] = (double)a;
    for (; a < 4; ++a) { f.coef[a] = 0.0; f.coef[5 + a] = 0.0; }
    f.coef[9] = ru; f.coef[10] = rw; f.coef[11] = pick ? s_left[pick] : ru;
  }
}

__global__ __launch_bounds__(BLOCK) void k_guess_fit(i64 n, const int* __restrict__ cmap, const double* __restrict__ ds,
                                                     const double* __restrict__ b, const double* __restrict__ yn,
                                                     const double* __restrict__ rhat, GuessFit f) {
  constexpr int RM = GUESS_RM, NS = GUESS_NS;
  __shared__ double s_red[BLOCK / 64];
  __shared__ double s_g[NS];
  double gs[NS];
#pragma unroll
  for (int j = 0; j < NS; ++j) gs[j] = 0.0;
  const i64 nchunk = (n + BLOCK - 1) / BLOCK;
  for (i64 ch = (i64)blockIdx.x * f.stride; ch < nchunk; ch += (i64)gridDim.x * f.stride) {
    const i64 i = ch * BLOCK + threadIdx.x;
    const int c = i < n ? (cmap ? cmap[i] : (int)i) : -1;
    if (c < 0) continue;
    const double d = ds[i], w = d * d, y0 = yn[i], ru = b[i] - y0, ra = rhat[c];
    double q[RM];
#pragma unroll
    for (int j = 0; j < RM; ++j) q[j] = j < f.avail ? f.yr[j][i] - y0 : 0.0;
    int t = 0;
#pragma unroll
    for (int j = 0; j < RM; ++j)
#pragma unroll
      for (int l = j; l < RM; ++l) gs[t++] += w * q[j] * q[l];
#pragma unroll
    for (int j = 0; j < RM; ++j) gs[t++] += w * q[j] * ru;
    gs[t++] += w * ru * ru;
    gs[t] += w * ra * ra;
  }
  {
    __shared__ double s_w[BLOCK / 64][NS];
    const int lane = threadIdx.x & 63, wave = threadIdx.x >> 6;
#pragma unroll
    for (int off = 32; off > 0; off >>= 1)
#pragma unroll
      for (int j = 0; j < NS; ++j) gs[j] += __shfl_down(gs[j], off, 64);
    if (lane == 0) {
#pragma unroll
      for (int j = 0; j < NS; ++j) s_w[wave][j] = gs[j];
    }
    __syncthreads();
    if (threadIdx.x < NS) {
      double a = 0.0;
#pragma unroll
      for (int q = 0; q < BLOCK / 64; ++q) a += s_w[q][threadIdx.x];
      pg::store_partial(f.partials + (size_t)threadIdx.x * gridDim.x + blockIdx.x, a);
    }
  }
  if (!pg::last_block_arrives(f.ticket, gridDim.x, s_red)) return;
  {
    constexpr int PW = (NS + BLOCK / 64 - 1) / (BLOCK / 64);
    const int lane = threadIdx.x & 63, wave = threadIdx.x >> 6, G = (int)gridDim.x;
    double a0[PW], a1[PW];
#pragma unroll
    for (int k = 0; k < PW; ++k) {
      const int sl = wave + k * (BLOCK / 64);
      a0[k] = (sl < NS && lane < G) ? pg::load_partial(f.partials + (size_t)sl * G + lane) : 0.0;
      a1[k] = (sl < NS && lane + 64 < G) ? pg::load_partial(f.partials + (size_t)sl * G + lane + 64) : 0.0;
    }
#pragma unroll
    for (int k = 0; k < PW; ++k) a0[k] += a1[k];
#pragma unroll
    for (int off = 32; off > 0; off >>= 1)
#pragma unroll
      for (int k = 0; k < PW; ++k) a0[k] += __shfl_down(a0[k], off, 64);
    if (lane == 0) {
#pragma unroll
      for (int k = 0; k < PW; ++k) {
        const int sl = wave + k * (BLOCK / 64);
        if (sl < NS) s_g[sl] = a0[k];
      }
    }
  }
  __syncthreads();
  if (f.sums) {
    if (threadIdx.x < NS) f.sums[threadIdx.x] = s_g[threadIdx.x];
    return;
  }
  guess_decide(s_g, f);
}

__global__ __launch_bounds__(BLOCK) void k_guess_decide(GuessFit f) {
  __shared__ double s_g[GUESS_NS];
  if (threadIdx.x < GUESS_NS) s_g[threadIdx.x] = f.sums[threadIdx.x];
  __syncthreads();
  guess_decide(s_g, f);
}

__global__ void k_rescale_state(i64 n, const double* __restrict__ ds_old, const double* __restrict__ ds_new,
                                double* __restrict__ z) {
  for (i64 r = blockIdx.x * (i64)blockDim.x + threadIdx.x; r < n; r += (i64)gridDim.x * blockDim.x)
    z[r] = (ds_old[r] * z[r]) / ds_new[r];
}

__global__ void k_scale_state(i64 n, const double* __restrict__ ds, const double* __restrict__ in, double* __restrict__ out,
                              int divide) {
  for (i64 r = blockIdx.x * (i64)blockDim.x + threadIdx.x; r < n; r += (i64)gridDim.x * blockDim.x)
    out[r] = divide ? in[r] / ds[r] : in[r] * ds[r];
}

__global__ void k_rhs_first(RowSegs seg, i64 n, i64 Mloc, int scheme, const int* row_cell, const double* T0pad,
                            const double* ypad, const double* mass, const double* bconst,
                            const unsigned char* fixed, double* braw, double* x0, int moving) {
  for (i64 r = blockIdx.x * (i64)blockDim.x + threadIdx.x; r < n; r += (i64)gridDim.x * blockDim.x) {
    const int k = seg_kind(seg, r);
    const i64 q = (i64)k * Mloc + row_cell[r];
    const double T = T0pad[q];
    double v;
    if (fixed[r]) v = bconst[r];
    else if (moving && (k & 1)) v = bconst[r];
    else if (moving && ypad) v = mass[r] * T - ypad[q] + bconst[r];
    else if (scheme == PG_SCHEME_CN) v = 2.0 * (mass[r] * T) - ypad[q] + bconst[r];
    else v = mass[r] * T + bconst[r];
    braw[r] = v;
    x0[r] = T;
  }
}

__global__ void k_psi(i64 Mloc, int scheme, const double* __restrict__ vn_1 , const double* __restrict__ vn,
                      double* __restrict__ psip, double* __restrict__ psim, double* __restrict__ psicp,
                      double* __restrict__ psicm) {
  for (i64 i = blockIdx.x * (i64)blockDim.x + threadIdx.x; i < Mloc; i += (i64)gridDim.x * blockDim.x) {
    const bool z1 = vn[i] == 0.0, z2 = vn_1[i] == 0.0;
    double pp, pm;
    if (scheme == PG_SCHEME_CN) {
      pp = (z1 && z2) ? 0.0 : (!z1 && !z2) ? 0.5 : (z1 && !z2) ? 0.5 : 1.0;
      pm = (z1 && z2) ? 0.0 : (!z1 && !z2) ? 0.5 : (z1 && !z2) ? 0.5 : 0.0;
    } else {
      pp = (z1 && z2) ? 0.0 : 1.0;
      pm = 0.0;
    }
    psip[i] = pp;
    psim[i] = pm;
    if (psicp) {
      psicp[i] = (z1 && !z2) ? 1.0 : 0.0;
      psicm[i] = (!z1 && !z2) || (!z1 && z2) ? 1.0 : 0.0;
    }
  }
}

__global__ void k_scatter_active(RowSegs seg, i64 n, i64 Mloc, const int* row_cell, const double* x, double* padded) {
  for (i64 r = blockIdx.x * (i64)blockDim.x + threadIdx.x; r < n; r += (i64)gridDim.x * blockDim.x) {
    const int k = seg_kind(seg, r);
    padded[(i64)k * Mloc + row_cell[r]] = x[r];
  }
}

__global__ void k_maxabs(i64 n, const double* x, const double* ds , double* partials) {
  __shared__ double sh[BLOCK];
  double m = 0.0;
  for (i64 i = blockIdx.x * (i64)blockDim.x + threadIdx.x; i < n; i += (i64)gridDim.x * blockDim.x) {
    const double a = fabs(ds ? ds[i] * x[i] : x[i]);
    m = a > m ? a : m;
  }
  sh[threadIdx.x] = m;
  __syncthreads();
  for (int s = BLOCK / 2; s > 0; s >>= 1) {
    if ((int)threadIdx.x < s) sh[threadIdx.x] = sh[threadIdx.x] > sh[threadIdx.x + s] ? sh[threadIdx.x] : sh[threadIdx.x + s];
    __syncthreads();
  }
  if (threadIdx.x == 0) partials[blockIdx.x] = sh[0];
}

constexpr int STEFAN_OUT = 8;
constexpr int STEFAN_BLOCKS = 64;
struct StefanArgs {
  SysParams P[2];
  const double* v0[2];
  const double* v1[2];
  const double* Id[2];
  const int* red;
  const double* x;
  const double* ds;
  const double* Tpad;
  i64 Mloc;
  int nphase;
};

__global__ __launch_bounds__(BLOCK) void k_stefan_partials(StefanArgs a, double* __restrict__ partials) {
  double acc[STEFAN_OUT];
#pragma unroll
  for (int j = 0; j < STEFAN_OUT; ++j) acc[j] = 0.0;
  const CapView& c = a.P[0].cap[0];
  for (i64 lc = blockIdx.x * (i64)blockDim.x + threadIdx.x; lc < a.Mloc; lc += (i64)gridDim.x * blockDim.x) {
    i64 idx[3];
    decode_cell(c.N, c.ext, c.plane, c.s0, lc, idx);
    for (int ph = 0; ph < a.nphase; ++ph) {
      const int* red = a.red + (i64)(2 * ph) * a.Mloc;
      double row = 0.0;
      eval_row(a.P[ph], 1, lc, idx, [&](int k, i64 col, double v) {
        const i64 q = (i64)k * a.Mloc + col;
        if (a.Tpad) {
          row += v * a.Tpad[(i64)(2 * ph) * a.Mloc + q];
        } else {
          const int r = red[q];
          if (r >= 0) row += v * (a.ds ? a.ds[r] * a.x[r] : a.x[r]);
        }
      });
      const double q = (a.Id[ph] ? a.Id[ph][lc] : 1.0) * row;
      acc[4 * ph + 0] += a.v0[ph][lc];
      acc[4 * ph + 1] += a.v1[ph][lc];
      acc[4 * ph + 2] += q;
      acc[4 * ph + 3] = fmax(acc[4 * ph + 3], fabs(q));
    }
  }
#pragma unroll
  for (int j = 0; j < STEFAN_OUT; ++j)
    for (int off = 32; off > 0; off >>= 1) {
      const double o = __shfl_down(acc[j], off, 64);
      acc[j] = (j & 3) == 3 ? fmax(acc[j], o) : acc[j] + o;
    }
  __shared__ double sh[BLOCK / 64][STEFAN_OUT];
  const int wave = threadIdx.x >> 6, lane = threadIdx.x & 63;
  if (lane == 0)
#pragma unroll
    for (int j = 0; j < STEFAN_OUT; ++j) sh[wave][j] = acc[j];
  __syncthreads();
  if (threadIdx.x < STEFAN_OUT) {
    const int j = threadIdx.x;
    double v = sh[0][j];
    for (int w = 1; w < BLOCK / 64; ++w) v = (j & 3) == 3 ? fmax(v, sh[w][j]) : v + sh[w][j];
    partials[(i64)blockIdx.x * STEFAN_OUT + j] = v;
  }
}

__global__ void k_stefan_final(const double* __restrict__ partials, int nblk, double* __restrict__ out) {
  if (threadIdx.x < STEFAN_OUT) {
    const int j = threadIdx.x;
    double v = partials[j];
    for (int b = 1; b < nblk; ++b) v = (j & 3) == 3 ? fmax(v, partials[(i64)b * STEFAN_OUT + j]) : v + partials[(i64)b * STEFAN_OUT + j];
    out[j] = v;
  }
// ... 658 lines not shown

void mon_reserve(pg_solver* s, i64 more) {
  pg_solver::Monitors& M = s->mon;
  if (M.K == 0 || M.rows + more <= M.cap) return;
  hipStream_t st = ctx().stream;
  const i64 per_row = (i64)M.G * M.K;
  i64 cap = M.cap > 0 ? 2 * M.cap : 64;
  while (cap < M.rows + more) cap *= 2;
  DevBuf<double> grown(cap * per_row);
  if (M.rows > 0)
    PG_HIP(hipMemcpyAsync(grown.p, M.series.p, sizeof(double) * (size_t)(M.rows * per_row), hipMemcpyDeviceToDevice, st));
  M.series = std::move(grown);
  M.cap = cap;
}

void mon_record(pg_solver* s) {
  pg_solver::Monitors& M = s->mon;
  if (M.K == 0) return;
  hipStream_t st = ctx().stream;
  const i64 per_row = (i64)M.G * M.K;
  mon_reserve(s, 1);
  mon_launch(s, M.series.p + M.rows * per_row, st);
  M.times.push_back(s->t);
  ++M.rows;
}

pg_krylov_opts default_opts() {
  pg_krylov_opts o;
  o.method = PG_METHOD_BICGSTAB;
  o.reltol = 1e-12;
  o.abstol = 0.0;
  o.maxiter = 0;
  o.check_every = 4;
  o.warm_start = 1;
  o.restart = 0;
  o.precond = 0;
  return o;
}

void mg_conditions(const pg_solver* s, int method, MgRule rule = MG_RULE_KIND) {
  const std::string who = std::string("multigrid preconditioner (precond = ") + mg_precond_name(rule) + ") refused: ";
  mg_require_one_rank(rule);
  PG_REQUIRE(s->scheme_ctor == PG_SCHEME_STEADY && !s->moving,
             who + (rule == MG_RULE_CELL ? "the system is an unsteady one (steady monophasic diffusion only)"
                                         : "the system is an unsteady one (steady monophasic diffusion and the stream-function solve only)"));
  PG_REQUIRE(s->nphase == 1, who + "the system is diphasic (its jump rows need the cell-block left preconditioner)");
  PG_REQUIRE(!s->advdiff && !(s->ops[0] && s->ops[0]->has_velocity), who + "the operator is a ConvectionOps (DiffusionOps only)");
  PG_REQUIRE(rule == MG_RULE_CELL || s->bc_i.kind == PG_BC_DIRICHLET,
             who + (s->bc_i.kind == PG_BC_ROBIN ? "the interface condition is Robin (Dirichlet only)"
                                                : "the interface condition is Neumann (Dirichlet only)"));
  PG_REQUIRE(method == PG_METHOD_BICGSTAB, who + krylov_method_refusal(method));
}

MgHierarchy& mg_of(pg_solver* s, MgRule rule) { return rule == MG_RULE_CELL ? s->mg_cell : s->mg; }

MgHierarchy& mg_ensure(pg_solver* s, MgRule rule = MG_RULE_KIND) {
  MgHierarchy& H = mg_of(s, rule);
  if (H.matrix != &s->A_ctor || H.lev.empty()) mg_build(H, s->A_ctor, s->nb, s->slab, rule);
  return H;
}

MgHierarchy* mg_prepare(pg_solver* s, const pg_krylov_opts& o) {
  if (!mg_is_precond(o.precond)) return nullptr;
  const MgRule rule = mg_rule_of(o.precond);
  mg_conditions(s, o.method, rule);
  return &mg_ensure(s, rule);
}

void mg_step_conditions(const pg_solver* s, int method) {
  const std::string who = "multigrid preconditioner (precond = PG_PRECOND_MG_STEP) refused: ";
  mg_require_one_rank_of(PG_PRECOND_MG_STEP);
  PG_REQUIRE(s->scheme_ctor != PG_SCHEME_STEADY,
             who + "the system is a steady one (the time loop of the unsteady monophasic diffusion solver only; steady solves are "
                   "served by PG_PRECOND_MG and PG_PRECOND_MG_CELL)");
  PG_REQUIRE(!s->moving, who + "a moving-body solver (every space-time slab is a new matrix that is solved once)");
  PG_REQUIRE(!s->solved_once, who + "the vorticity solver of a pg_streamvort step (a new matrix every step, solved once)");
  PG_REQUIRE(!s->advdiff && !s->convection && !(s->ops[0] && s->ops[0]->has_velocity),
             who + "the operator is a ConvectionOps (DiffusionOps only)");
  PG_REQUIRE(method == PG_METHOD_BICGSTAB, who + krylov_method_refusal(method));
}

MgHierarchy& mg_step_ensure(pg_solver* s, const CsrMatrix& A) {
  MgHierarchy& H = s->mg_step[&A == &s->A_ctor ? 0 : 1];
  if (H.matrix == &A && !H.lev.empty()) return H;
  try {
    mg_build(H, A, s->nb, s->slab, MG_RULE_CELL);
  } catch (...) {
    H = MgHierarchy();
    throw;
  }
  return H;
}

void specest_conditions(const pg_solver* s, int method) {
  const std::string who = "estimated polynomial preconditioner (precond = PG_PRECOND_POLY_EST) refused: ";
  specest_require_one_rank();
  PG_REQUIRE(!s->moving, who + "a moving-body solver (every space-time slab is a new matrix that is solved once)");
  PG_REQUIRE(!s->advdiff && !s->convection, who + "the operator is a ConvectionOps (DiffusionOps only)");
  PG_REQUIRE(method == PG_METHOD_BICGSTAB, who + krylov_method_refusal(method));
}

void specest_prepare(pg_solver* s, const CsrMatrix& A, const pg_krylov_opts& o) {
  if (o.precond != PG_PRECOND_POLY_EST) return;
  specest_conditions(s, o.method);
  if (A.poly_ok || A.est.tried || A.poly_gave_up) return;
  specest_run(const_cast<CsrMatrix&>(A), s->nb, s->slab);
}

void solve_ctor_system(pg_solver* s, const pg_krylov_opts& o, SolveStats& st, bool from_state, bool first, MgHierarchy* mg) {
  const i64 n = s->nb.n_own;
  KrylovCall call;
  call.mg = mg;
  if (from_state) {
    hipStream_t stream = ctx().stream;
    if (first) hipLaunchKernelGGL(k_scale_state, dim3(grid_for(n, BLOCK)), dim3(BLOCK), 0, stream, n, s->A_ctor.ds.p, s->x.p, s->z.p, 1);
    spmv_halo(s->A_ctor, s->nb, s->slab, s->z.p, s->y.p, stream);
    PG_HIP(hipGetLastError());
    call.x0 = s->z.p; call.Ax0 = s->y.p;
  }
  krylov_solve(s->A_ctor, s->nb, s->slab, s->b.p, s->ysol.p, s->work, o, st, call);
  std::swap(s->z.p, s->ysol.p);
  s->z_matrix = &s->A_ctor;
  s->x_valid = false;
  if (!first) return;
  s->initial_done = true;
  s->diag_ctor.snapped_version = s->diag_run.snapped_version = -1;
  s->hist_cnt = 0;
  s->spec_y_valid = false;
}

void do_initial(pg_solver* s, const pg_krylov_opts* opts, SolveStats& st) {
  const pg_krylov_opts o = opts ? *opts : default_opts();
  MgHierarchy* mg = mg_prepare(s, o);
  if (mg_is_step(o.precond)) {
    mg_step_conditions(s, o.method);
    mg = &mg_step_ensure(s, s->A_ctor);
  }
  specest_prepare(s, s->A_ctor, o);
  const bool from_state = s->moving && o.warm_start != 0 && o.method == PG_METHOD_BICGSTAB && s->nb.n_own > 0;
  solve_ctor_system(s, o, st, from_state, true, mg);
}

void guess_policy(bool& on, double last_products, double bytes_per_product) {
  const Config& cfg = config();
  if (on || cfg.guess_n <= 0 || last_products <= 0.0) return;
  const double t_prod_us = std::max(5.0, bytes_per_product / 5.0e6);
  if (cfg.guess_always || (bytes_per_product >= 256.0 * 1024.0 && last_products >= 6.0 + 3.0 * (20.0 / t_prod_us))) on = true;
}

struct GuessPlan {
  int KH = 0, R = 0, hist_had = 0;
  bool refit = true;
  GuessArgs ga{};
};

GuessPlan guess_prepare(pg_solver* s, const void* owner, bool allowed, double last_products, hipStream_t stream) {
  const Config& cfg = config();
  GuessPlan gp;
  gp.refit = last_products > 4.0 || s->steps_done % 8 == 0;
  gp.KH = allowed ? cfg.guess_n : 0;
  gp.R = gp.KH > 0 ? cfg.guess_depth : 0;
  gp.hist_had = (s->hist_de == owner && s->hist_k == gp.R) ? s->hist_cnt : 0;
  s->hist_cnt = 0;
  if (gp.KH == 0) return gp;
  const int R = gp.R;
  const i64 nva = s->z.n;
  if (s->guess_coef.n == 0) { s->guess_coef.alloc(GUESS_USED + 16); s->guess_coef.zero(); s->guess_ticket.alloc(1); s->guess_ticket.zero(); }
  for (int j = 0; j <= R; ++j) {
    if (j < R && s->zh[j].n != nva) { s->zh[j].alloc(nva); s->zh[j].zero(); }
    if (s->yh[j].n != nva) { s->yh[j].alloc(nva); s->yh[j].zero(); }
  }
  if (gp.hist_had == 0) PG_HIP(hipMemsetAsync(s->guess_coef.p, 0, 12 * sizeof(double), stream));
  for (int j = 0; j < 8; ++j) { gp.ga.zr[j] = s->zh[std::min(j, R - 1)].p; gp.ga.yr[j] = s->yh[std::min(j, R - 1)].p; }
  gp.ga.znew = s->zh[R - 1].p;
  gp.ga.coef = s->guess_coef.p;
  return gp;
}

void guess_after_rhs(pg_solver* s, const GuessPlan& gp, i64 n, const int* cmap, const double* ds, const double* rhat, bool single,
                     KrylovWork& w, hipStream_t stream) {
  if (gp.KH == 0) return;
  const Config& cfg = config();
  const int R = gp.R;
  if (gp.hist_had > 0 && gp.refit) {
    GuessFit gf{};
    for (int j = 0; j < 8; ++j) gf.yr[j] = s->yh[std::min(j, R - 1)].p;
    const i64 nchunk = (n + BLOCK - 1) / BLOCK;
    gf.stride = (int)std::max<i64>(1, std::min<i64>(cfg.guess_monitor, nchunk / 128));
    const int gfit = (int)std::min<i64>(128, (nchunk + gf.stride - 1) / gf.stride);
    if (s->guess_partials.n != (i64)GUESS_NS * std::max(gfit, 1)) s->guess_partials.alloc((i64)GUESS_NS * std::max(gfit, 1));
    gf.partials = s->guess_partials.p;
    gf.ticket = s->guess_ticket.p;
    gf.coef = s->guess_coef.p;
    gf.avail = std::min(gp.hist_had, GUESS_RM);
    gf.kmax = gp.KH;
    gf.rate2 = w.last_rate2;
    gf.pass_cost = cfg.guess_pass_cost;
    gf.gain = cfg.guess_gain;
    gf.sums = single ? nullptr : s->guess_coef.p + 16;
    hipLaunchKernelGGL(k_guess_fit, dim3(std::max(gfit, 1)), dim3(BLOCK), 0, stream, n, cmap, ds, (const double*)s->b.p,
                       (const double*)s->y.p, rhat, gf);
    if (!single) {
      comm_allreduce_sum_f64(gf.sums, GUESS_NS, stream);
      hipLaunchKernelGGL(k_guess_decide, dim3(1), dim3(BLOCK), 0, stream, gf);
    }
    PG_HIP(hipGetLastError());
  }
  double* znew = s->zh[R - 1].p;
  double* yspare = s->yh[R].p;
  double* yretire = s->yh[R - 1].p;
  for (int j = R - 1; j > 0; --j) { s->zh[j].p = s->zh[j - 1].p; s->yh[j].p = s->yh[j - 1].p; }
  s->zh[0].p = s->z.p; s->z.p = znew;
  s->yh[0].p = s->y.p; s->y.p = yspare;
  s->yh[R].p = yretire;
}

void guess_commit(pg_solver* s, const GuessPlan& gp, const void* owner) {
  if (gp.KH == 0) return;
  if (config().debug) {
    double hc[16];
    s->guess_coef.download(hc, 16);
    fprintf(stderr, "[pg_solver] extrapolated start: %d older states kept; sampled (r,r)_W plain %.3e, taken %.3e; next step: %d states",
            gp.hist_had, hc[9], hc[10], (int)hc[4]);
    for (int j = 0; j < (int)hc[4]; ++j) fprintf(stderr, " z(n-%d)*%.4f", (int)hc[5 + j] + 1, hc[j]);
    fprintf(stderr, ", fit leaves %.3e\n", hc[11]);
  }
  s->hist_cnt = std::min(gp.hist_had + 1, gp.R);
  s->hist_k = gp.R;
  s->hist_de = owner;
}

void launch_rhs_block_mf(pg_solver* s, int scheme, const CsrMatrix& A, hipStream_t stream) {
  hipLaunchKernelGGL(k_rhs_block_mf, dim3(grid_for(A.n_blk, BLOCK)), dim3(BLOCK), 0, stream, make_params(s, scheme), make_segs(s->nb),
                     s->Mloc, A.n_blk, A.blk_rows.p, A.blk_idx.p, A.blk_coef.p, s->nb.row_cell.p, s->nb.red.p, A.ds.p,
                     (const double*)s->z.p, s->mass.p, s->bconst.p, s->fixed.p, s->b.p);
}

void step_compact(pg_solver* s, int scheme, const pg_krylov_opts& o, const CsrMatrix& A, DiagElim& DE, const DiagElim*& used_de,
                  SolveStats& st) {
  hipStream_t stream = ctx().stream;
  const i64 n = s->nb.n_own;
  KrylovWork& w = s->work;
  const int stamp = (int)((s->steps_done % 2000000000) + 1);
  const bool single = ctx().nranks == 1 && !ctx().comm;
  const bool same_data = DE.snapped_version == s->bconst_version;
  const bool quiet = same_data && single;
  guess_policy(DE.guess_on, DE.last_products, DE.bytes_per_rank);
  GuessPlan gp = guess_prepare(s, &DE, same_data && DE.guess_on, DE.last_products, stream);
  const int KH = gp.KH;
  const Config& cfg = config();
  const bool defer = KH > 0 && cfg.guess_defer && DE.last_products > 0.0;
  gp.ga.defer = defer ? 1 : 0;
  const GuessArgs& ga = gp.ga;
  const double* zprev = s->z.p;
#define PG_RHS_INIT_C(KHV)                                                                                                        \
  hipLaunchKernelGGL(HIP_KERNEL_NAME(k_rhs_init_c<KHV>), dim3(w.grid), dim3(BLOCK), 0, stream, n, scheme, s->z.p, s->y.p, A.ds.p,   \
                     s->mass.p, s->bconst.p, s->fixed.p, A.isblk.p, DE.cmap.p, s->b.p, (const double*)DE.gdiag.p, DE.delta.p,     \
                     DE.flag.p, stamp, w.rhat.p, w.partials.p, quiet ? w.ticket.p : nullptr, w.sc.p, o.reltol * o.reltol,          \
                     o.abstol * o.abstol, same_data ? 0 : 1, ga)
  switch (KH) {
    case 1: PG_RHS_INIT_C(1); break;
    case 2: PG_RHS_INIT_C(2); break;
    case 3: PG_RHS_INIT_C(3); break;
    case 4: PG_RHS_INIT_C(4); break;
    default: PG_RHS_INIT_C(0); break;
  }
#undef PG_RHS_INIT_C
  PG_HIP(hipGetLastError());
  guess_after_rhs(s, gp, n, (const int*)DE.cmap.p, (const double*)A.ds.p, (const double*)w.rhat.p, single, w, stream);
  if (!same_data) diag_fix(DE, s->nb, s->slab, stamp, !single, w.rhat.p, w.partials.p, w.grid, stream);
  KrylovCall call;
  call.preinit = call.p_in_rhat = true;
  call.start_folded = quiet;
  call.scatter = DE.rlist.p;
  if (same_data && !single) { call.moved_flag = DE.flag.p; call.moved_stamp = stamp; }
  DE.snapped_version = s->bconst_version;
  used_de = &DE;
  s->spec_pending = false;
  if (quiet && s->hint_more_steps && config().speculate_product)
    call.after_first_batch = [s, &A, stream]() {
      spmv_halo(A, s->nb, s->slab, s->z.p, s->y.p, stream);
      s->spec_pending = true;
      s->spec_matrix = &A;
    };
  if (defer) {
    call.xguess.zbase = zprev;
    for (int j = 0; j < 8; ++j) call.xguess.zr[j] = ga.zr[j];
    call.xguess.coef = s->guess_coef.p + GUESS_USED;
  }
  krylov_solve(DE.A, DE.nb, s->slab, nullptr, s->z.p, w, o, st, call);
  s->spec_y_valid = s->spec_pending && st.polls == 1 && st.converged && st.poly_degree >= 0;
  s->spec_pending = false;
  const bool solved = st.poly_degree >= 0;
  DE.last_products = (double)st.products;

  const bool moved_unseen = solved && same_data && w.h_sc[S_MOVED] != 0.0;
  if (!solved || moved_unseen) {
    s->spec_y_valid = false;
    if (!solved) {
      DE.active = false;
      poly_record_stagnation(A);
    }
    used_de = nullptr;
    const SolveStats first = st;
    st = SolveStats();
    spmv_halo(A, s->nb, s->slab, s->z.p, s->y.p, stream);
    KrylovCall full;
    full.x0 = s->z.p; full.Ax0 = s->y.p;
    krylov_solve(A, s->nb, s->slab, s->b.p, s->ysol.p, w, o, st, full);
    std::swap(s->z.p, s->ysol.p);
    st.iters += first.iters;
    st.products += first.products;
  }
  else guess_commit(s, gp, &DE);
  s->x_valid = false;
}

void step_warm(pg_solver* s, int scheme, const pg_krylov_opts& o, const CsrMatrix& A, bool mgs, SolveStats& st) {
  hipStream_t stream = ctx().stream;
  const i64 n = s->nb.n_own;
  KrylovWork& w = s->work;
  GammaElim& E = (&A == &s->A_ctor) ? s->elim_ctor : s->elim_run;
  if (!mgs && !E.tried) build_gamma_elim(A, s->nb, E);
  const bool e_active = !mgs && E.active;
  const bool single = ctx().nranks == 1 && !ctx().comm;
  const int which = (&A == &s->A_ctor) ? 0 : 1;
  if (single && !e_active) guess_policy(s->plain_guess_on[which], s->plain_last_products[which], (double)A.spmv_bytes);
  const GuessPlan gp = guess_prepare(s, &A, single && !e_active && s->plain_guess_on[which], s->plain_last_products[which], stream);
#define PG_RHS_INIT(KHV)                                                                                                          \
  hipLaunchKernelGGL(HIP_KERNEL_NAME(k_rhs_init<KHV>), dim3(w.grid), dim3(BLOCK), 0, stream, n, s->nb.n_vec(), scheme, s->z.p,     \
                     s->y.p, A.ds.p, s->mass.p, s->bconst.p, s->fixed.p, A.isblk.p, s->b.p, w.r.p, w.rhat.p, w.p.p, w.partials.p, \
                     gp.ga)
  switch (gp.KH) {
    case 1: PG_RHS_INIT(1); break;
    case 2: PG_RHS_INIT(2); break;
    case 3: PG_RHS_INIT(3); break;
    case 4: PG_RHS_INIT(4); break;
    default: PG_RHS_INIT(0); break;
  }
#undef PG_RHS_INIT
  PG_HIP(hipGetLastError());
  guess_after_rhs(s, gp, n, nullptr, (const double*)A.ds.p, (const double*)w.rhat.p, true, w, stream);
  KrylovCall call;
  call.preinit = true;
  if (e_active) {
    gamma_fix(E, s->z.p, w.r.p, w.rhat.p, w.p.p, w.partials.p, w.grid, stream);
    pg_krylov_opts oe = o;
    if (oe.precond == PG_PRECOND_POLY_EST) oe.precond = 0;
    krylov_solve(E.A, E.nb, s->slab, s->b.p, s->z.p, w, oe, st, call);
  } else {
    if (mgs) call.mg = &mg_step_ensure(s, A);
    krylov_solve(A, s->nb, s->slab, s->b.p, s->z.p, w, o, st, call);
    s->plain_last_products[which] = (double)st.products;
    guess_commit(s, gp, &A);
  }
  s->x_valid = false;
}

void step_cold(pg_solver* s, int scheme, const pg_krylov_opts& o, const CsrMatrix& A, bool mgs, SolveStats& st) {
  hipStream_t stream = ctx().stream;
  const i64 n = s->nb.n_own;
  s->hist_cnt = 0;
  materialize_x(s);
  const bool idr_warm = o.warm_start != 0 && o.method == PG_METHOD_IDRS && n > 0;
  if (n > 0) {
    if (scheme == PG_SCHEME_CN || idr_warm) {
      hipLaunchKernelGGL(k_scale_state, dim3(grid_for(n, BLOCK)), dim3(BLOCK), 0, stream, n, A.ds.p, s->x.p, s->z.p, 1);
      spmv_halo(A, s->nb, s->slab, s->z.p, s->y.p, stream);
    }
    hipLaunchKernelGGL(k_rhs, dim3(grid_for(n, BLOCK)), dim3(BLOCK), 0, stream, n, scheme, s->x.p, s->y.p, A.ds.p, s->mass.p,
                       s->bconst.p, s->fixed.p, s->b.p);
    if (A.n_blk > 0 && s->nphase == 2 && scheme == PG_SCHEME_CN)
      launch_rhs_block_mf(s, scheme, A, stream);
    else if (A.n_blk > 0)
      hipLaunchKernelGGL(k_rhs_block, dim3(grid_for(A.n_blk, BLOCK)), dim3(BLOCK), 0, stream, A.n_blk, scheme, A.blk_rows.p,
                         A.blk_idx.p, A.blk_coef.p, A.blk_cn.p, s->x.p, (const double*)nullptr, s->y.p, s->mass.p,
                         s->bconst.p, s->fixed.p, s->b.p);
    PG_HIP(hipGetLastError());
  }
  KrylovCall call;
  if (mgs) call.mg = &mg_step_ensure(s, A);
  if (idr_warm) { call.x0 = s->z.p; call.Ax0 = s->y.p; }
  krylov_solve(A, s->nb, s->slab, s->b.p, s->ysol.p, s->work, o, st, call);
  std::swap(s->z.p, s->ysol.p);
  s->z_matrix = &A;
  s->x_valid = false;
}

void do_step(pg_solver* s, int scheme, const pg_krylov_opts* opts, SolveStats& st) {
  PG_REQUIRE(s->scheme_ctor != PG_SCHEME_STEADY, "a steady solver has no time loop");
  PG_REQUIRE(!s->moving, "a moving-body solver is one space-time step: create the next one from the next time slab");
  PG_REQUIRE(s->initial_done, "Solver is not initialized. Call pg_solver_initial_solve first.");
  const pg_krylov_opts o = opts ? *opts : default_opts();
  if (mg_is_precond(o.precond)) mg_conditions(s, o.method, mg_rule_of(o.precond));
  const bool mgs = mg_is_step(o.precond);
  if (mgs) {
    mg_step_conditions(s, o.method);
    ensure_run_matrix(s, scheme);
    mg_step_ensure(s, run_matrix(s));
  }
  for (const auto& t : s->td) {
    PG_REQUIRE(t.K == 0 || s->td_cursor < t.nrows,
               "time-separable data: this step is past the last row of the coefficient table (" + std::to_string(t.nrows) +
               " rows, all consumed); install a longer table with pg_solver_set_separable");
    for (const auto& pr : t.progs)
      PG_REQUIRE(s->td_cursor < pr.nrows,
                 "device function: this step is past the last row of the table of times (" + std::to_string(pr.nrows) +
                 " rows, all consumed); install a longer table with pg_solver_set_program");
  }
  if (td_installed(s)) s->td_row = s->td_cursor++;
  hipStream_t stream = ctx().stream;
  ensure_run_matrix(s, scheme);
  const CsrMatrix& A = run_matrix(s);
  specest_prepare(s, A, o);
  const i64 n = s->nb.n_own;
  const bool warm = o.warm_start != 0 && o.method == PG_METHOD_BICGSTAB && n > 0;
  const DiagElim* used_de = nullptr;
  struct QuietGuard {
    pg_solver* s; const DiagElim*& used;
    ~QuietGuard() {
      if (used != &s->diag_ctor) s->diag_ctor.snapped_version = -1;
      if (used != &s->diag_run) s->diag_run.snapped_version = -1;
    }
  } quiet_guard{s, used_de};
  s->t += s->dt;
  ensure_bconst(s, scheme);
  if (warm) {
    if (s->z_matrix != &A) {
      hipLaunchKernelGGL(k_rescale_state, dim3(grid_for(n, BLOCK)), dim3(BLOCK), 0, stream, n, s->z_matrix->ds.p, A.ds.p, s->z.p);
      s->z_matrix = &A;
    }
    const bool have_y = s->spec_y_valid && s->spec_matrix == &A;
    s->spec_y_valid = false;
    if (!have_y) spmv_halo(A, s->nb, s->slab, s->z.p, s->y.p, stream);
    const bool blk_mf = s->nphase == 2 && scheme == PG_SCHEME_CN;
    if (A.n_blk > 0 && blk_mf) launch_rhs_block_mf(s, scheme, A, stream);
    else if (A.n_blk > 0) {
      if (s->blk_cache_matrix != &A || s->blk_cache_scheme != scheme || s->blk_cache_version != s->bconst_version) {
        if (s->blk_wz.n != A.n_blk * MAX_KINDS) s->blk_wz.alloc(A.n_blk * MAX_KINDS);
        if (s->blk_c0.n != A.n_blk) s->blk_c0.alloc(A.n_blk);
        hipLaunchKernelGGL(k_blk_cache, dim3(grid_for(A.n_blk, BLOCK)), dim3(BLOCK), 0, stream, A.n_blk, scheme, A.blk_idx.p,
                           A.blk_coef.p, A.ds.p, s->mass.p, s->bconst.p, s->fixed.p, s->blk_wz.p, s->blk_c0.p);
        s->blk_cache_matrix = &A; s->blk_cache_scheme = scheme; s->blk_cache_version = s->bconst_version;
      }
      hipLaunchKernelGGL(k_rhs_block_c, dim3(grid_for(A.n_blk, BLOCK)), dim3(BLOCK), 0, stream, A.n_blk, scheme, A.blk_rows.p,
                         A.blk_idx.p, (const double*)s->blk_wz.p, (const double*)s->blk_c0.p, A.blk_cn.p, (const double*)s->z.p,
                         (const double*)s->y.p, s->b.p);
    }
    DiagElim& DE = (&A == &s->A_ctor) ? s->diag_ctor : s->diag_run;
    if (!mgs && !DE.tried) build_diag_elim(A, s->nb, s->slab, DE);
    if (!mgs && DE.active && krylov_uses_polynomial(DE.A, o)) step_compact(s, scheme, o, A, DE, used_de, st);
    else step_warm(s, scheme, o, A, mgs, st);
  } else step_cold(s, scheme, o, A, mgs, st);
  s->steps_done += 1;
}

}

extern "C" {

struct SolverSpec {
  const char* entry;
  int nphase = 1;
  pg_capacity* cap[2] = {nullptr, nullptr};
  pg_diffops* ops[2] = {nullptr, nullptr};
  const double* D[2] = {nullptr, nullptr};
  const double* f_n[2] = {nullptr, nullptr};
  const double* f_np1[2] = {nullptr, nullptr};
  const pg_bc_desc* bc_interface = nullptr;
  const pg_jump_desc* ic = nullptr;
  const pg_border_desc* borders = nullptr;
  int32_t nborders = 0;
  double dt = 1.0;
  const double* T0 = nullptr;
  pg_solver* previous = nullptr;
  int32_t scheme = PG_SCHEME_BE;
  bool steady = false;
  bool moving = false, advdiff = false, stefan = false;
  const pg::SolverDeviceData* dev = nullptr;
  bool solved_once = false;
  pg_solver** out = nullptr;
};

static int32_t create_solver(const SolverSpec& d) {
  PG_API_BEGIN
  require_init();
  const std::string who = std::string(d.entry) + ": ";
  const bool mono = d.nphase == 1;
  std::unique_ptr<AsyncAllocScope> pool(d.moving ? new AsyncAllocScope() : nullptr);
  PG_REQUIRE(d.steady || d.scheme == PG_SCHEME_BE || d.scheme == PG_SCHEME_CN, who + "scheme must be BE or CN");
  PG_REQUIRE(d.out && (mono ? d.bc_interface != nullptr : d.ic != nullptr), who + "NULL argument");
  for (int q = 0; q < d.nphase; ++q) {
    PG_REQUIRE(d.cap[q] && d.ops[q], who + "NULL argument");
    PG_REQUIRE(d.ops[q]->cap == d.cap[q], who + "operators were built from a different capacity");
  }
  if (!mono) {
    PG_REQUIRE(d.cap[0]->mesh == d.cap[1]->mesh, "Phase capacities must share the same mesh.");
    PG_REQUIRE(d.cap[0]->slab.p0 == d.cap[1]->slab.p0 && d.cap[0]->slab.p1 == d.cap[1]->slab.p1,
               who + "phase capacities must share the slab partition");
  }
  if (d.moving) {
    for (int q = 0; q < d.nphase; ++q) {
      PG_REQUIRE(d.cap[q]->spacetime, who + "every phase needs a space-time capacity (pg_capacity_create_spacetime)");
      if (d.advdiff)
        PG_REQUIRE(d.ops[q]->st_velocity, who + "the moving advection-diffusion solver needs the ConvectionOps of its "
                   "space-time capacity (pg_diffops_set_velocity_spacetime)");
      else
        PG_REQUIRE(!d.ops[q]->has_velocity, who + "the moving diffusion solver takes no convection operators");
    }
    PG_REQUIRE(ctx().nranks == 1 && !ctx().comm, who + "space-time steps are single-rank");
    PG_REQUIRE(!d.previous || d.previous->initial_done, who + "the previous slab has not been solved");
  } else {
    PG_REQUIRE(d.dt > 0.0, who + "dt must be positive");
    if (d.previous) {
      PG_REQUIRE(!d.steady, who + "a steady solver has no previous state");
      PG_REQUIRE(ctx().nranks == 1 && !ctx().comm, who + "a state is handed from solver to solver on one rank only");
      PG_REQUIRE(d.previous->initial_done, who + "the previous solver has not been solved");
    }
  }
  auto* s = new pg_solver();
  std::unique_ptr<pg_solver> guard(s);
  s->nphase = d.nphase;
  s->slab = d.cap[0]->slab;
  s->dt = d.moving ? 1.0 : d.dt;
  s->moving = d.moving;
  s->advdiff = d.advdiff;
  s->stefan = d.stefan;
  s->scheme_ctor = d.steady ? PG_SCHEME_STEADY : d.scheme;
  const i64 Ml = s->slab.Mloc();
  for (int q = 0; q < d.nphase; ++q) {
    s->cap[q] = d.cap[q];
    s->ops[q] = d.ops[q];
    s->convection = s->convection || (d.ops[q] && d.ops[q]->has_velocity);
    if (d.moving) {
      s->psi_p[q].alloc(Ml);
      s->psi_m[q].alloc(Ml);
      if (d.advdiff) {
        s->psi_cp[q].alloc(Ml);
        s->psi_cm[q].alloc(Ml);
      }
      hipLaunchKernelGGL(k_psi, dim3(grid_for(Ml, BLOCK)), dim3(BLOCK), 0, ctx().stream, Ml, (int)d.scheme, d.cap[q]->Vt[0].p,
                         d.cap[q]->Vt[1].p, s->psi_p[q].p, s->psi_m[q].p, s->psi_cp[q].p, s->psi_cm[q].p);
      PG_HIP(hipGetLastError());
    }
    if (d.D[q]) upload_local(s->Id[q], d.D[q], s->slab);
    if (d.f_np1[q]) upload_local(s->f_np1[q], d.f_np1[q], s->slab);
    if (d.f_n[q]) upload_local(s->f_n[q], d.f_n[q], s->slab);
  }
  if (d.dev) {
    PG_REQUIRE(mono, who + "device-resident data: one phase only");
    auto take = [&](DevBuf<double>& dst, const double* src) {
      if (!src) return;
      dst.alloc(Ml);
      PG_HIP(hipMemcpyAsync(dst.p, src, sizeof(double) * (size_t)Ml, hipMemcpyDeviceToDevice, ctx().stream));
    };
    take(s->Id[0], d.dev->D);
    take(s->f_n[0], d.dev->f_n);
    take(s->f_np1[0], d.dev->f_np1);
  }
  if (mono) {
    s->bc_i = *d.bc_interface;
    if (d.bc_interface->value_array) {
      upload_local(s->g_np1, d.bc_interface->value_array, s->slab);
      upload_local(s->g_n, d.bc_interface->value_array, s->slab);
    }
    s->bc_i.value_array = nullptr;
    if (d.dev && d.dev->g_np1) {
      s->g_np1.alloc(Ml);
      s->g_n.alloc(Ml);
      PG_HIP(hipMemcpyAsync(s->g_np1.p, d.dev->g_np1, sizeof(double) * (size_t)Ml, hipMemcpyDeviceToDevice, ctx().stream));
      PG_HIP(hipMemcpyAsync(s->g_n.p, d.dev->g_n ? d.dev->g_n : d.dev->g_np1, sizeof(double) * (size_t)Ml, hipMemcpyDeviceToDevice,
                            ctx().stream));
    }
  } else {
    s->ic = *d.ic;
    if (d.ic->g_array) upload_local(s->g_arr, d.ic->g_array, s->slab);
    if (d.ic->h_array) upload_local(s->h_arr, d.ic->h_array, s->slab);
    s->ic.g_array = s->ic.h_array = nullptr;
  }
  s->init_from = d.previous;
  s->A_ctor.want_units = !d.moving && !d.solved_once;
  s->solved_once = d.solved_once;
  setup_common(s, d.borders, d.nborders, d.T0);
  *d.out = guard.release();
  PG_API_END
}

static SolverSpec spec_mono(const char* entry, pg_capacity* c, pg_diffops* o, const pg_bc_desc* bc_interface,
                            const pg_border_desc* borders, int32_t nborders, const double* Dcoef, const double* f_n,
                            const double* f_np1, pg_solver** out) {
  SolverSpec d;
  d.entry = entry;
  d.cap[0] = c; d.ops[0] = o; d.D[0] = Dcoef; d.f_n[0] = f_n; d.f_np1[0] = f_np1;
  d.bc_interface = bc_interface;
  d.borders = borders; d.nborders = nborders;
  d.out = out;
  return d;
}

static SolverSpec spec_diph(const char* entry, pg_capacity* c1, pg_diffops* o1, pg_capacity* c2, pg_diffops* o2,
                            const pg_jump_desc* ic, const pg_border_desc* borders, int32_t nborders, const double* D1,
// ... 1167 lines not shown
             "pg_debug_spmv_apply: mode 8, a separate dot operand and the folded scalar phase exist in the slice kernel (variant 70) only");
  PG_REQUIRE(!fold || (mode >= 1 && mode <= 3), "pg_debug_spmv_apply: only the modes with dots (1, 2, 3) fold a scalar phase");
  PG_REQUIRE((mode == 1 || mode == 3) == (aux != nullptr), "pg_debug_spmv_apply: aux goes with modes 1 and 3, and only with them");
  PG_REQUIRE(!dotx || mode == 2 || mode == 3, "pg_debug_spmv_apply: dotx goes with modes 2 and 3");
  PG_REQUIRE(!base || mode == 8, "pg_debug_spmv_apply: base goes with mode 8");
  i64 nv = 0;
  const CsrMatrix& A = debug_matrix(s, which, &nv);
  const i64 n = A.n;
  PG_REQUIRE(n > 0, "pg_debug_spmv_apply: the matrix has no rows");
  PG_REQUIRE(!slices || A.srec.p, "pg_debug_spmv_apply: the matrix has no slice image");
  nv = std::max(nv, n);
  hipStream_t st = ctx().stream;
  const int grid = spmv_default_grid(n);
  constexpr i64 GUARD = 64;
  double sentinel;
  const unsigned long long sbits = PG_DEBUG_SPMV_SENTINEL;
  std::memcpy(&sentinel, &sbits, sizeof(double));
  DevBuf<double> dx(nv), daux(nv), ddot(nv), dbase(nv), dy(n + GUARD), dpart(5 * (i64)grid), dsc(S_COUNT);
  DevBuf<unsigned> dticket(1);
  daux.zero(); ddot.zero(); dbase.zero(); dsc.zero(); dticket.zero();
  dx.upload(x, nv);
  if (aux) daux.upload(aux, n);
  if (dotx) ddot.upload(dotx, n);
  if (base) dbase.upload(base, n);
  {
    std::vector<double> fill((size_t)std::max<i64>(n + GUARD, 5 * (i64)grid), sentinel);
    dy.upload(fill.data(), n + GUARD);
    if (fold && mode == 3) std::fill(fill.begin() + 2 * (size_t)grid, fill.begin() + 4 * (size_t)grid, 0.0);
    dpart.upload(fill.data(), 5 * (i64)grid);
    std::vector<double> hsc(S_COUNT, 0.0);
    for (int k = 0; k < 5; ++k) hsc[S_RED0 + k] = sentinel;
    hsc[S_DONE] = (double)done;
    dsc.upload(hsc.data(), S_COUNT);
  }
  FinArgs f{fold ? dticket.p : nullptr, fold ? dsc.p : nullptr, PH_NONE, fold ? (mode == 1 ? 1 : (mode == 2 ? 2 : 5)) : 0, 0,
            dotx ? ddot.p : nullptr};
  if (mode == 8) { f.pc0 = pc0; f.pc1 = pc1; f.pc2 = pc2; f.base = base ? dbase.p : dx.p; }
  const bool with_fin = mode == 8 || fold || dotx;
  for (int r = 0; r < repeat; ++r) {
    const bool folded_here = launch_spmv_as(variant, mode, A, dx.p, dy.p, aux ? daux.p : nullptr, mode >= 1 && mode <= 3 ? dpart.p : nullptr,
                                            dsc.p, grid, st, with_fin ? &f : nullptr);
    PG_REQUIRE(folded_here == (fold != 0), "pg_debug_spmv_apply: the launch did not report the scalar phase as asked");
  }
  PG_HIP(hipGetLastError());
  dy.download(y, n + GUARD);
  std::vector<double> hp(5 * (size_t)grid), hsc(S_COUNT);
  dpart.download(hp.data(), 5 * (i64)grid);
  dsc.download(hsc.data(), S_COUNT);
  if (partials) std::memcpy(partials, hp.data(), sizeof(double) * hp.size());
  for (int k = 0; k < 5; ++k) {
    double a = 0.0;
    for (int i = 0; i < grid; ++i) a += hp[(size_t)k * grid + i];
    slot_sums[k] = a;
    folded[k] = hsc[S_RED0 + k];
  }
  unsigned ht = 0;
  dticket.download(&ht, 1);
  *ticket = (int64_t)ht;
  PG_API_END
}

int32_t pg_debug_spmv_apply_typed(pg_solver* s, int32_t which, int32_t kind, const void* x, const void* base, double pc0, double pc1,
                                  double pc2, double sigma, int32_t done, double* y64, float* y32, float* p32) {
  PG_API_BEGIN
  require_init();
  PG_REQUIRE(s && x, "pg_debug_spmv_apply_typed: NULL argument");
  PG_REQUIRE(ctx().nranks == 1 && !ctx().comm, "pg_debug_spmv_apply_typed: one rank");
  PG_REQUIRE(kind == TYPED_FIRST || kind == TYPED_MIDDLE || kind == TYPED_HANDOVER, "pg_debug_spmv_apply_typed: kinds 1 (first), 2 (middle), 3 (hand-over)");
  PG_REQUIRE((kind == TYPED_FIRST) == (base == nullptr), "pg_debug_spmv_apply_typed: the first launch's base is its x; the others take one");
  PG_REQUIRE((kind == TYPED_FIRST) == (p32 != nullptr), "pg_debug_spmv_apply_typed: p32 is the first launch's output, and only its");
  PG_REQUIRE(kind == TYPED_HANDOVER ? (y64 && !y32) : (y32 && !y64), "pg_debug_spmv_apply_typed: y32 for kinds 1 and 2, y64 for kind 3");
  PG_REQUIRE(spmv_supports_typed_chain(), "pg_debug_spmv_apply_typed: the typed launches exist in the slice kernel with the stream hint only");
  i64 nv = 0;
  const CsrMatrix& A = debug_matrix(s, which, &nv);
  const i64 n = A.n;
  PG_REQUIRE(n > 0 && A.srec.p, "pg_debug_spmv_apply_typed: the matrix has no rows or no slice image");
  nv = std::max(nv, n);
  hipStream_t st = ctx().stream;
  const int grid = spmv_default_grid(n);
  constexpr i64 GUARD = 64;
  double sentinel;
  const unsigned long long sbits = PG_DEBUG_SPMV_SENTINEL;
  std::memcpy(&sentinel, &sbits, sizeof(double));
  float sentinel32;
  const unsigned sbits32 = PG_DEBUG_SPMV_SENTINEL_F32;
  std::memcpy(&sentinel32, &sbits32, sizeof(float));
  DevBuf<double> dx64(nv), db64(nv), dy64(n + GUARD), dsc(S_COUNT);
  DevBuf<float> dx32(nv), db32(nv), dy32(n + GUARD), dp32(n + GUARD);
  db64.zero(); db32.zero();
  if (kind == TYPED_FIRST) dx64.upload(static_cast<const double*>(x), nv);
  else dx32.upload(static_cast<const float*>(x), nv);
  if (kind == TYPED_MIDDLE) db32.upload(static_cast<const float*>(base), n);
  if (kind == TYPED_HANDOVER) db64.upload(static_cast<const double*>(base), n);
  {
    std::vector<double> f64((size_t)(n + GUARD), sentinel);
    std::vector<float> f32((size_t)(n + GUARD), sentinel32);
    dy64.upload(f64.data(), n + GUARD);
    dy32.upload(f32.data(), n + GUARD);
    dp32.upload(f32.data(), n + GUARD);
    std::vector<double> hsc(S_COUNT, 0.0);
    hsc[S_DONE] = (double)done;
    dsc.upload(hsc.data(), S_COUNT);
  }
  FinArgs f{nullptr, nullptr, PH_NONE, 0, 0, nullptr};
  f.pc0 = pc0; f.pc1 = pc1; f.pc2 = pc2;
  if (kind == TYPED_FIRST) {
    f.base = dx64.p; f.p32 = dp32.p; f.psig = sigma;
    launch_spmv_typed(kind, A, dx64.p, dy32.p, dsc.p, grid, st, f);
  } else if (kind == TYPED_MIDDLE) {
    f.base = reinterpret_cast<const double*>(db32.p);
    launch_spmv_typed(kind, A, dx32.p, dy32.p, dsc.p, grid, st, f);
  } else {
    f.base = db64.p;
    launch_spmv_typed(kind, A, dx32.p, dy64.p, dsc.p, grid, st, f);
  }
  PG_HIP(hipGetLastError());
  if (y64) dy64.download(y64, n + GUARD);
  if (y32) dy32.download(y32, n + GUARD);
  if (p32) dp32.download(p32, n + GUARD);
  PG_API_END
}

__global__ void k_scale_rows(i64 n_e, const int* __restrict__ elist, double factor, double* __restrict__ z) {
  for (i64 q = blockIdx.x * (i64)blockDim.x + threadIdx.x; q < n_e; q += (i64)gridDim.x * blockDim.x) z[elist[q]] *= factor;
}

int32_t pg_debug_scale_diagonal_rows(pg_solver* s, double factor) {
  PG_API_BEGIN
  require_init();
  PG_REQUIRE(s && s->have_run, "pg_debug_scale_diagonal_rows: no run matrix yet");
  const CsrMatrix& A = run_matrix(s);
  DiagElim& DE = (&A == &s->A_ctor) ? s->diag_ctor : s->diag_run;
  PG_REQUIRE(DE.active && DE.n_e > 0, "pg_debug_scale_diagonal_rows: the loop of this solver is not the compact one");
  hipLaunchKernelGGL(k_scale_rows, dim3(grid_for(DE.n_e, BLOCK)), dim3(BLOCK), 0, ctx().stream, DE.n_e, (const int*)DE.elist.p, factor,
                     s->z.p);
  PG_HIP(hipGetLastError());
  PG_HIP(hipStreamSynchronize(ctx().stream));
  s->x_valid = false;
  s->spec_y_valid = false;
  PG_API_END
}

int32_t pg_solver_guess_info(pg_solver* s, int32_t* kept, int32_t* nstates, int32_t* offsets, double* coef, double* rr_plain,
                             double* rr_taken) {
  PG_API_BEGIN
  require_init();
  PG_REQUIRE(s && kept && nstates && offsets && coef && rr_plain && rr_taken, "pg_solver_guess_info: NULL argument");
  *kept = s->hist_cnt;
  *nstates = 0;
  *rr_plain = *rr_taken = 0.0;
  for (int j = 0; j < 4; ++j) { offsets[j] = 0; coef[j] = 0.0; }
  if (s->guess_coef.n >= 16 && s->hist_cnt > 0) {
    double hc[16];
    s->guess_coef.download(hc, 16);
    *nstates = (int32_t)hc[4];
    for (int j = 0; j < *nstates && j < 4; ++j) { offsets[j] = (int32_t)hc[5 + j] + 1; coef[j] = hc[j]; }
    *rr_plain = hc[9];
    *rr_taken = hc[10];
  }
  PG_API_END
}

int32_t pg_solver_time_spmv(pg_solver* s, int32_t which, int32_t reps, double* avg_ms) {
  PG_API_BEGIN
  require_init();
  PG_REQUIRE(s && avg_ms && reps > 0, "pg_solver_time_spmv: bad arguments");
  const int sel = which & 1, mode = (which & 2048) ? 8 : ((which >> 4) & 7);
  PG_REQUIRE(mode <= 3 || mode == 8, "pg_solver_time_spmv: unknown launch mode");
  if (sel == 1) PG_REQUIRE(s->have_run, "run matrix not assembled yet");
  const CsrMatrix& Afull = sel == 0 ? s->A_ctor : run_matrix(s);
  GammaElim& E = (&Afull == &s->A_ctor) ? s->elim_ctor : s->elim_run;
  if ((which & 512) && !E.tried) build_gamma_elim(Afull, s->nb, E);
  DiagElim& DE = (&Afull == &s->A_ctor) ? s->diag_ctor : s->diag_run;
  if ((which & 4096) && !DE.tried) build_diag_elim(Afull, s->nb, s->slab, DE);
  const CsrMatrix& A = ((which & 4096) && DE.active) ? DE.A : (((which & 512) && E.active) ? E.A : Afull);
  const bool chained = (which & 1024) != 0;
  hipStream_t st = ctx().stream;
  EventPair ev;
  KrylovWork& w = s->work;
  const bool cold = (which & 256) != 0;
  constexpr int RING = 7;
  std::vector<DevBuf<double>> ring;
  const i64 nv = s->nb.n_vec();
  if (cold) {
    ring.resize(RING);
    for (auto& b : ring) {
      b.alloc(nv > 0 ? nv : 1);
      if (nv > 0) PG_HIP(hipMemcpyAsync(b.p, s->z.p, sizeof(double) * (size_t)nv, hipMemcpyDeviceToDevice, st));
    }
  }
  int it = 0;
  auto one = [&]() {
    const double* xin = cold ? ring[it % RING].p : (chained && (it & 1) ? s->y.p : s->z.p);
    double* yout = cold ? ring[(it + 3) % RING].p : (chained && (it & 1) ? s->z.p : s->y.p);
    const double* ax = cold ? ring[(it + 5) % RING].p : w.rhat.p;
    ++it;
    if (mode == 0) spmv(A, xin, yout, st);
    else if (mode == 8) {
      FinArgs f{nullptr, nullptr, PH_NONE, 0, 0, nullptr};
      f.pc0 = 1.0; f.pc1 = -0.5; f.pc2 = 0.5; f.base = s->b.p;
      launch_spmv(8, A, xin, yout, nullptr, nullptr, nullptr, w.grid, st, &f);
    }
    else launch_spmv(mode, A, xin, yout, ax, w.partials.p, nullptr, w.grid, st);
  };
  for (int i = 0; i < 3; ++i) one();
  PG_HIP(hipEventRecord(ev.e0, st));
  for (int i = 0; i < reps; ++i) one();
  PG_HIP(hipEventRecord(ev.e1, st));
  PG_HIP(hipEventSynchronize(ev.e1));
  PG_HIP(hipGetLastError());
  float ms = 0.f;
  PG_HIP(hipEventElapsedTime(&ms, ev.e0, ev.e1));
  *avg_ms = ms / reps;
  PG_API_END
}

}

namespace pg {

int32_t solver_create_unsteady_mono_dev(pg_capacity* c, pg_diffops* o, const pg_bc_desc* bc_interface, const pg_border_desc* borders,
                                        int32_t nborders, const SolverDeviceData& dev, double dt, const double* T0,
                                        pg_solver* previous, int32_t scheme, pg_solver** out) {
  SolverSpec d = spec_mono("pg_streamvort_step", c, o, bc_interface, borders, nborders, nullptr, nullptr, nullptr, out);
  d.dt = dt; d.T0 = T0; d.previous = previous; d.scheme = scheme;
  d.dev = &dev;
  d.solved_once = true;
  return create_solver(d);
}

i64 solver_mloc(const pg_solver* s) { return s->Mloc; }

double* solver_source_dev(pg_solver* s) {
  if (s->f_np1[0].n != s->Mloc) { s->f_np1[0].alloc(s->Mloc); s->f_np1[0].zero(); }
  return s->f_np1[0].p;
}

void solver_data_changed(pg_solver* s) { s->bconst_dirty = true; }

void solver_solve_again(pg_solver* s, const pg_krylov_opts* opts, SolveStats& st) {
  PG_REQUIRE(s->scheme_ctor == PG_SCHEME_STEADY && !s->moving, "solve again: a steady solver is expected");
  if (!s->initial_done) {
    build_first_rhs(s);
    do_initial(s, opts, st);
    return;
  }
  const pg_krylov_opts o = opts ? *opts : default_opts();
  MgHierarchy* const mg = mg_prepare(s, o);
  if (mg_is_step(o.precond)) mg_step_conditions(s, o.method);
  specest_prepare(s, s->A_ctor, o);
  const i64 n = s->nb.n_own;
  ensure_bconst(s, PG_SCHEME_STEADY);
  if (n > 0) apply_left(s->A_ctor, s->bconst.p, s->b.p, ctx().stream);
  const bool from_state = o.warm_start != 0 && (o.method == PG_METHOD_BICGSTAB || o.method == PG_METHOD_IDRS) && n > 0;
  solve_ctor_system(s, o, st, from_state, false, mg);
}

constexpr double REFINE_RELTOL = 1e-6;

__global__ void k_refine_residual(i64 n, i64 nvec, const double* __restrict__ b, const double* __restrict__ y, double* __restrict__ r) {
  for (i64 i = blockIdx.x * (i64)blockDim.x + threadIdx.x; i < nvec; i += (i64)gridDim.x * blockDim.x) r[i] = i < n ? b[i] - y[i] : 0.0;
}

__global__ void k_refine_add(i64 n, const double* __restrict__ d, double* __restrict__ z) {
  for (i64 i = blockIdx.x * (i64)blockDim.x + threadIdx.x; i < n; i += (i64)gridDim.x * blockDim.x) z[i] += d[i];
}

static void refine_once(pg_solver* s, const pg_krylov_opts& o, SolveStats& st) {
  const i64 n = s->nb.n_own, nv = s->nb.n_vec();
  if (n <= 0) return;
  hipStream_t stream = ctx().stream;
  const CsrMatrix& A = s->A_ctor;
  spmv_halo(A, s->nb, s->slab, s->z.p, s->y.p, stream);
  DevBuf<double> r(nv);
  hipLaunchKernelGGL(k_refine_residual, dim3(grid_for(nv, BLOCK)), dim3(BLOCK), 0, stream, n, nv, (const double*)s->b.p,
                     (const double*)s->y.p, r.p);
  PG_HIP(hipGetLastError());
  pg_krylov_opts oc = o;
  oc.reltol = REFINE_RELTOL;
  oc.abstol = 0.0;
  SolveStats more;
  krylov_solve(A, s->nb, s->slab, r.p, s->ysol.p, s->work, oc, more);
  hipLaunchKernelGGL(k_refine_add, dim3(grid_for(n, BLOCK)), dim3(BLOCK), 0, stream, n, (const double*)s->ysol.p, s->z.p);
  PG_HIP(hipGetLastError());
  st.iters += more.iters;
  st.products += more.products + 1;
  s->x_valid = false;
}

void solver_first_solve_from_state(pg_solver* s, const pg_krylov_opts* opts, SolveStats& st) {
  const pg_krylov_opts o = opts ? *opts : default_opts();
  if (mg_is_precond(o.precond)) mg_conditions(s, o.method, mg_rule_of(o.precond));
  if (mg_is_step(o.precond)) mg_step_conditions(s, o.method);
  specest_prepare(s, s->A_ctor, o);
  const i64 n = s->nb.n_own;
  if (!(o.warm_start != 0 && o.method == PG_METHOD_BICGSTAB && n > 0) || s->initial_done) {
    do_initial(s, opts, st);
    refine_once(s, o, st);
    return;
  }
  solve_ctor_system(s, o, st, true, true, nullptr);
  refine_once(s, o, st);
}

void solver_state_padded(pg_solver* s, double* padded) {
  hipStream_t st = ctx().stream;
  materialize_x(s);
// ... 16 lines not shown
```

### penguin/jl_amd/csrc/pg_system.h

```cpp
#pragma once
#include <vector>

#include "pg_stencil.h"

namespace pg {

struct SpecEst {
  bool tried = false;
  bool admitted = false;
  int steps = 0;
  double g_ritz = 0.0, g_used = 0.0;
  double re_min = 0.0, re_max = 0.0, im_max = 0.0;
  double ms = 0.0;
  std::vector<double> H;
};

struct Numbering {
  int K = 2;
  i64 Mloc = 0;
  i64 n_own = 0, n_ghost = 0;
  i64 cnt_own[MAX_KINDS] = {0, 0, 0, 0}, off_own[MAX_KINDS] = {0, 0, 0, 0};
  i64 cntL[MAX_KINDS] = {0, 0, 0, 0}, offL[MAX_KINDS] = {0, 0, 0, 0};
  i64 cntU[MAX_KINDS] = {0, 0, 0, 0}, offU[MAX_KINDS] = {0, 0, 0, 0};
  i64 sendL_off[MAX_KINDS] = {0, 0, 0, 0}, sendL_cnt[MAX_KINDS] = {0, 0, 0, 0};
  i64 sendU_off[MAX_KINDS] = {0, 0, 0, 0}, sendU_cnt[MAX_KINDS] = {0, 0, 0, 0};
  DevBuf<int> red;
  DevBuf<int> row_cell;
  i64 n_vec() const { return n_own + n_ghost; }
  int kind_of_row(i64 r) const {
    int k = 0;
    while (k + 1 < K && r >= off_own[k + 1]) ++k;
    return k;
  }
};

struct CsrMatrix {
  i64 n = 0, nnz = 0;
  int scheme = -1;
  DevBuf<int> rowptr, col;
  DevBuf<double> val;
  DevBuf<double> ds;
  DevBuf<int> chunk_desc;
  i64 nchunks = 0;
  DevBuf<int> srec;
  DevBuf<double> pval;
  DevBuf<int> g_rowid, g_rowptr, g_col;
  DevBuf<double> g_val;
  DevBuf<int> mrec;
  i64 nunits = 0, rows_m = 0;
  DevBuf<int> e_meta;
  DevBuf<double> e_val;
  i64 rows_e = 0, e_slots = 0;
  DevBuf<int> tiles;
  int tiles_per_xcd = 0;
  i64 tile_ns = 0;
  const int* geo_cell = nullptr;
  const int* geo_map = nullptr;
  i64 geo_ext0 = 0, geo_lines = 0;
  bool want_units = true;
  i64 nslices = 0;
  i64 nslices_int = 0;
  DevBuf<unsigned char> rowflags;
  i64 rows_u = 0, rows_p = 0, rows_g = 0, nnz_p = 0, nnz_g = 0;
  i64 spmv_bytes = 0;
  bool halo_needed = true;
  bool poly_ok = false;
  double gersh = 0.0;
  SpecEst est;
  bool poly_gave_up = false;
  i64 n_blk = 0;
  i64 nnz_raw = 0;
  DevBuf<int> blk_rows, blk_idx;
  DevBuf<double> blk_coef, blk_cn, blk_fw;
  DevBuf<unsigned char> isblk;
};
inline void poly_record_stagnation(const CsrMatrix& A) {
  CsrMatrix& M = const_cast<CsrMatrix&>(A);
  M.poly_ok = false;
  M.est.admitted = false;
  M.poly_gave_up = true;
}
constexpr int SPMV_CHUNK_ENTRIES = 508;
void build_spmv_chunks(CsrMatrix& A);

void build_numbering(const SysParams& P, const Slab& slab, Numbering& nb);
void assemble_csr(const SysParams& P, const Slab& slab, const Numbering& nb, CsrMatrix& A, bool scale = true);
void assemble_csr_preconditioned(const SysParams& P, const Slab& slab, const Numbering& nb, CsrMatrix& A,
                                 const bool* inherit_halo = nullptr);
void assemble_csr_like(const SysParams& P, const Slab& slab, const Numbering& nb, const CsrMatrix& T, CsrMatrix& A);
bool build_slices_like(const CsrMatrix& T, CsrMatrix& A);
void decide_poly(CsrMatrix& A);
void apply_left(const CsrMatrix& A, const double* in, double* out, hipStream_t st);
void apply_rows_padded(const SysParams& P, const Slab& slab, const double* x, double* y);

}
```

Baseline: 1346.

## Fuse extrapolated-guess fit and coefficient decision into RHS init kernel

Adds a step_fuse mode, on by default, that runs the initial-guess least-squares fit inside the rhs_init kernel. Extra thread blocks compute the Gram sums in five parts, and the last-arriving block solves the small Cholesky systems and picks the best history subset on the GPU. Block-row RHS values are computed inline through a retained blk_pos map, and the coefficient buffer is double-buffered so the fit can write while the current coefficients are read. This is meant to remove separate fit and reduction launches and extra passes over the vectors on every time step, at the cost of heavier kernels and more complex sync through ticket counters.

```diff
diff --git a/penguin/jl_amd/csrc/pg_common.h b/penguin/jl_amd/csrc/pg_common.h
--- a/penguin/jl_amd/csrc/pg_common.h
+++ b/penguin/jl_amd/csrc/pg_common.h
@@ -95,6 +95,7 @@
   int guess_monitor = 256;
   double guess_pass_cost = 0.34;
   double guess_gain = 0.8;
+  bool step_fuse = true;
   bool speculate_product = true;
   int mg_tail_rows = 2048;
   int unit_order = 0;
diff --git a/penguin/jl_amd/csrc/pg_context.hip b/penguin/jl_amd/csrc/pg_context.hip
--- a/penguin/jl_amd/csrc/pg_context.hip
+++ b/penguin/jl_amd/csrc/pg_context.hip
@@ -70,6 +70,7 @@
     k.guess_always = geti("PG_GUESS_ALWAYS", 0) != 0;
     k.guess_defer = geti("PG_GUESS_DEFER", 1) != 0;
     k.guess_gain = getd("PG_GUESS_GAIN", 0.8);
+    k.step_fuse = geti("PG_STEP_FUSE", 1) != 0;
     k.unit_order = (int)geti("PG_SPMV_UNIT_ORDER", 0);
     return k;
   }();
@@ -369,11 +370,11 @@
            "spmv_variant=%d spmv_xcd=%d spmv_strip=%d spmv_unit_order=%d spmv_march=%d spmv_edges=%d spmv_march_k=%d spmv_minrun=%d spmv_tile_units=%d "
            "spmv_blocks_per_cu=%d halo_overlap=%d speculate=%d poly=%d poly_degree=%d poly_adapt=%d "
            "poly_margin=%g poly_slack=%g poly_hist=%d poly_trend=%d poly_maxdeg=%d poly_f32=%d poly_f32_tail=%d gamma_elim=%d diag_elim=%d "
-           "guess_states=%d guess_depth=%d guess_defer=%d async_alloc=%d cache_limit_mb=%lld alloc_poison=%d alloc_guard=%d profile_sample=%d debug=%d",
+           "guess_states=%d guess_depth=%d guess_defer=%d step_fuse=%d async_alloc=%d cache_limit_mb=%lld alloc_poison=%d alloc_guard=%d profile_sample=%d debug=%d",
            k.spmv_variant, k.spmv_xcd, k.spmv_strip, k.unit_order, (int)k.spmv_march, (int)k.spmv_edges, k.spmv_march_k, k.spmv_minrun, k.spmv_tile_units,
            k.spmv_blocks_per_cu, (int)k.halo_overlap, (int)k.speculate_product, (int)k.poly, k.poly_degree, (int)k.poly_adapt,
            k.poly_margin, k.poly_slack, k.poly_hist, (int)k.poly_trend, k.poly_maxdeg, (int)k.poly_f32, k.poly_f32_tail,
-           (int)k.gamma_elim, (int)k.diag_elim, k.guess_n, k.guess_depth, (int)k.guess_defer, k.async_alloc, k.pool_limit_mb, k.alloc_poison, k.alloc_guard, k.profile_sample, (int)k.debug);
+           (int)k.gamma_elim, (int)k.diag_elim, k.guess_n, k.guess_depth, (int)k.guess_defer, (int)k.step_fuse, k.async_alloc, k.pool_limit_mb, k.alloc_poison, k.alloc_guard, k.profile_sample, (int)k.debug);
   if (buf && n > 0) {
     std::strncpy(buf, tmp, n - 1);
     buf[n - 1] = 0;
diff --git a/penguin/jl_amd/csrc/pg_precond.hip b/penguin/jl_amd/csrc/pg_precond.hip
--- a/penguin/jl_amd/csrc/pg_precond.hip
+++ b/penguin/jl_amd/csrc/pg_precond.hip
@@ -340,7 +340,9 @@
   hipLaunchKernelGGL(HIP_KERNEL_NAME(k_asm_p<true>), dim3(gr), dim3(256), 0, st, P, seg, nb.Mloc, n, nb.row_cell.p, nb.red.p,
                      A.ds.p, (int*)nullptr, (unsigned char*)nullptr, (unsigned long long*)nullptr, (const int*)A.rowptr.p, A.col.p, A.val.p);
   PG_HIP(hipGetLastError());
-  DevBuf<int> pos(n), total(1);
+  A.blk_pos.alloc(n);
+  DevBuf<int>& pos = A.blk_pos;
+  DevBuf<int> total(1);
   scan_exclusive<unsigned char>(isblk.p, pos.p, n, total.p, st);
   int nblk = 0;
   total.download(&nblk, 1);
@@ -439,7 +441,9 @@
   A.blk_cn.alloc((i64)MAX_KINDS * nb1);
   A.blk_fw.alloc((i64)MAX_KINDS * nb1);
   if (nblk > 0) {
-    DevBuf<int> pos(n), total(1);
+    A.blk_pos.alloc(n);
+    DevBuf<int>& pos = A.blk_pos;
+    DevBuf<int> total(1);
     scan_exclusive<unsigned char>(A.isblk.p, pos.p, n, total.p, st);
     hipLaunchKernelGGL(k_blk_table, dim3(gr), dim3(256), 0, st, P, seg, nb.Mloc, n, nb.row_cell.p, nb.red.p, A.ds.p, A.isblk.p,
                        pos.p, A.blk_rows.p, A.blk_idx.p, A.blk_coef.p, A.blk_cn.p, A.blk_fw.p);
diff --git a/penguin/jl_amd/csrc/pg_solver.hip b/penguin/jl_amd/csrc/pg_solver.hip
--- a/penguin/jl_amd/csrc/pg_solver.hip
+++ b/penguin/jl_amd/csrc/pg_solver.hip
@@ -82,6 +82,7 @@
   const CsrMatrix* spec_matrix = nullptr;
   DevBuf<double> zh[8], yh[8], guess_coef, guess_partials;
   DevBuf<unsigned> guess_ticket;
+  int guess_buf = 0;
   int hist_cnt = 0, hist_k = 0;
   bool plain_guess_on[2] = {false, false};
   double plain_last_products[2] = {0.0, 0.0};
@@ -269,24 +270,34 @@
   }
 }
 
-__global__ void k_rhs_block_c(i64 nblk, int scheme, const int* __restrict__ blk_rows, const int* __restrict__ blk_idx,
-                              const double* __restrict__ wz, const double* __restrict__ c0, const double* __restrict__ blk_cn,
-                              const double* __restrict__ z, const double* __restrict__ yhat, double* __restrict__ b) {
-  for (i64 q = blockIdx.x * (i64)blockDim.x + threadIdx.x; q < nblk; q += (i64)gridDim.x * blockDim.x) {
-    int j[MAX_KINDS];
-    double zz[MAX_KINDS], yy[MAX_KINDS];
-#pragma unroll
-    for (int a = 0; a < MAX_KINDS; ++a) j[a] = blk_idx[q * MAX_KINDS + a];
-#pragma unroll
-    for (int a = 0; a < MAX_KINDS; ++a) {
-      zz[a] = j[a] >= 0 ? z[j[a]] : 0.0;
-      yy[a] = (j[a] >= 0 && scheme == PG_SCHEME_CN) ? yhat[j[a]] : 0.0;
-    }
-    double v = c0[q];
-#pragma unroll
-    for (int a = 0; a < MAX_KINDS; ++a) v += wz[q * MAX_KINDS + a] * zz[a] - (scheme == PG_SCHEME_CN ? blk_cn[q * MAX_KINDS + a] * yy[a] : 0.0);
-    b[blk_rows[q]] = v;
-  }
+struct BlkTables {
+  const int* idx;
+  const double* wz;
+  const double* c0;
+  const double* cn;
+  const int* pos;
+};
+
+__device__ inline double rhs_block_row(i64 q, int scheme, const BlkTables& t, const double* z, const double* yhat) {
+  int j[MAX_KINDS];
+  double zz[MAX_KINDS], yy[MAX_KINDS];
+#pragma unroll
+  for (int a = 0; a < MAX_KINDS; ++a) j[a] = t.idx[q * MAX_KINDS + a];
+#pragma unroll
+  for (int a = 0; a < MAX_KINDS; ++a) {
+    zz[a] = j[a] >= 0 ? z[j[a]] : 0.0;
+    yy[a] = (j[a] >= 0 && scheme == PG_SCHEME_CN) ? yhat[j[a]] : 0.0;
+  }
+  double v = t.c0[q];
+#pragma unroll
+  for (int a = 0; a < MAX_KINDS; ++a) v += t.wz[q * MAX_KINDS + a] * zz[a] - (scheme == PG_SCHEME_CN ? t.cn[q * MAX_KINDS + a] * yy[a] : 0.0);
+  return v;
+}
+
+__global__ void k_rhs_block_c(i64 nblk, int scheme, const int* __restrict__ blk_rows, BlkTables t, const double* __restrict__ z,
+                              const double* __restrict__ yhat, double* __restrict__ b) {
+  for (i64 q = blockIdx.x * (i64)blockDim.x + threadIdx.x; q < nblk; q += (i64)gridDim.x * blockDim.x)
+    b[blk_rows[q]] = rhs_block_row(q, scheme, t, z, yhat);
 }
 
 __global__ void k_rhs_block_mf(SysParams P, RowSegs seg, i64 Mloc, i64 nblk, const int* __restrict__ blk_rows,
@@ -325,8 +336,10 @@
   const double* zr[8];
   const double* yr[8];
   double* znew;
-  double* coef;
+  const double* coef;
+  double* count;
   int defer;
+  double* used;
 };
 constexpr int GUESS_USED = 64;
 
@@ -335,6 +348,108 @@
 #pragma unroll
   for (int q = 1; q < 8; ++q) p = i == q ? r[q] : p;
   return p;
+}
+
+constexpr int GUESS_RM = 7;
+constexpr int GUESS_NS = GUESS_RM * (GUESS_RM + 1) / 2 + GUESS_RM + 2;
+struct GuessFit {
+  const double* yr[8];
+  double* partials;
+  unsigned* ticket;
+  double* coef;
+  int stride, avail, kmax;
+  double rate2, pass_cost, gain;
+  double* sums;
+  int nblocks;
+};
+
+__device__ inline int guess_tri(int j, int l) { return j * GUESS_RM - j * (j - 1) / 2 + (l - j); }
+
+__device__ inline void guess_decide(const double* s_g, const GuessFit& f) {
+  constexpr int RM = GUESS_RM, NS = GUESS_NS;
+  __shared__ double s_left[128], s_net[128];
+  __shared__ double s_c[128][4];
+  const double ru = s_g[NS - 2], rw = s_g[NS - 1];
+  if (threadIdx.x < 128) {
+    const int mask = threadIdx.x, m = __popc(mask);
+    double left = ru, cc[4] = {0.0, 0.0, 0.0, 0.0};
+    if (mask != 0 && m <= f.kmax && m <= 4 && (mask >> f.avail) == 0 && ru > 0.0) {
+      int idx[4] = {0, 0, 0, 0};
+      for (int j = 0, a = 0; j < RM; ++j) if (mask >> j & 1) { if (a < 4) idx[a] = j; ++a; }
+      double L[4][4], wv[4];
+      bool ok = true;
+#pragma unroll
+      for (int a = 0; a < 4; ++a) {
+        wv[a] = 0.0;
+#pragma unroll
+        for (int e = 0; e < 4; ++e) L[a][e] = 0.0;
+      }
+#pragma unroll
+      for (int a = 0; a < 4; ++a) {
+        if (a >= m || !ok) continue;
+        const double g0 = s_g[guess_tri(idx[a], idx[a])];
+        double dj = g0;
+#pragma unroll
+        for (int e = 0; e < 4; ++e) if (e < a) dj -= L[a][e] * L[a][e];
+        if (!(g0 > 0.0) || !(dj > 1e-12 * g0)) { ok = false; continue; }
+        const double lj = sqrt(dj);
+        L[a][a] = lj;
+#pragma unroll
+        for (int l = 0; l < 4; ++l) {
+          if (l <= a || l >= m) continue;
+          double v = s_g[guess_tri(idx[a], idx[l])];
+#pragma unroll
+          for (int e = 0; e < 4; ++e) if (e < a) v -= L[l][e] * L[a][e];
+          L[l][a] = v / lj;
+        }
+        double v = s_g[RM * (RM + 1) / 2 + idx[a]];
+#pragma unroll
+        for (int e = 0; e < 4; ++e) if (e < a) v -= L[a][e] * wv[e];
+        wv[a] = v / lj;
+        left -= wv[a] * wv[a];
+      }
+      if (ok) {
+#pragma unroll
+        for (int aa = 0; aa < 4; ++aa) {
+          const int a = 3 - aa;
+          if (a >= m) continue;
+          double v = wv[a];
+#pragma unroll
+          for (int e = 0; e < 4; ++e) if (e > a && e < m) v -= L[e][a] * cc[e];
+          cc[a] = v / L[a][a];
+        }
+#pragma unroll
+        for (int a = 0; a < 4; ++a) ok = ok && isfinite(cc[a]) && fabs(cc[a]) < 256.0;
+      }
+      if (!ok) { left = ru; cc[0] = cc[1] = cc[2] = cc[3] = 0.0; }
+      if (!(left > 1e-30 * ru)) left = 1e-30 * ru;
+    }
+    s_left[threadIdx.x] = left;
+#pragma unroll
+    for (int a = 0; a < 4; ++a) s_c[threadIdx.x][a] = cc[a];
+    const bool live = ru > 0.0 && f.rate2 > 0.0 && rw <= ru * (1.0 + 1e-12) && left < ru;
+    s_net[threadIdx.x] = live ? f.gain * log(ru / left) / f.rate2 - 2.0 * m * f.pass_cost : 0.0;
+  }
+  __syncthreads();
+  if (threadIdx.x < 64) {
+    int pick = threadIdx.x;
+    double best = s_net[pick];
+    if (s_net[pick + 64] > best) { best = s_net[pick + 64]; pick += 64; }
+#pragma unroll
+    for (int off = 32; off > 0; off >>= 1) {
+      const double ob = __shfl_down(best, off, 64);
+      const int op = __shfl_down(pick, off, 64);
+      if (ob > best || (ob == best && op < pick)) { best = ob; pick = op; }
+    }
+    if (!(best > 0.0)) pick = 0;
+    if (threadIdx.x != 0) return;
+    int a = 0;
+    for (int j = 0; j < RM; ++j)
+      if (pick >> j & 1) { f.coef[a] = s_c[pick][a]; f.coef[5 + a] = (double)j; ++a; }
+    f.coef[4] = (double)a;
+    for (; a < 4; ++a) { f.coef[a] = 0.0; f.coef[5 + a] = 0.0; }
+    f.coef[9] = ru; f.coef[10] = rw; f.coef[11] = pick ? s_left[pick] : ru;
+  }
 }
 
 typedef double rd2_t __attribute__((ext_vector_type(2)));
@@ -372,7 +487,7 @@
       zo[j] = ring_pick(g.zr, sel);
       yo[j] = ring_pick(g.yr, sel);
     }
-    if (blockIdx.x == 0 && threadIdx.x == 0) g.coef[13] += (double)ku;
+    if (blockIdx.x == 0 && threadIdx.x == 0) *g.count += (double)ku;
   }
   const i64 npair = (nvec + 1) / 2;
   for (i64 q = blockIdx.x * (i64)BLOCK + threadIdx.x; q < npair; q += (i64)gridDim.x * BLOCK) {
@@ -444,8 +559,158 @@
   if (threadIdx.x == 0) partials[2 * (size_t)gridDim.x + blockIdx.x] = tw;
 }
 
+__device__ inline void guess_fit_last(const GuessFit& f, int G, double* s_g) {
+  constexpr int NS = GUESS_NS;
+  {
+    constexpr int PW = (NS + BLOCK / 64 - 1) / (BLOCK / 64);
+    const int lane = threadIdx.x & 63, wave = threadIdx.x >> 6;
+    double a0[PW], a1[PW];
+#pragma unroll
+    for (int k = 0; k < PW; ++k) {
+      const int sl = wave + k * (BLOCK / 64);
+      a0[k] = (sl < NS && lane < G) ? pg::load_partial(f.partials + (size_t)sl * G + lane) : 0.0;
+      a1[k] = (sl < NS && lane + 64 < G) ? pg::load_partial(f.partials + (size_t)sl * G + lane + 64) : 0.0;
+    }
+#pragma unroll
+    for (int k = 0; k < PW; ++k) a0[k] += a1[k];
+#pragma unroll
+    for (int off = 32; off > 0; off >>= 1)
+#pragma unroll
+      for (int k = 0; k < PW; ++k) a0[k] += __shfl_down(a0[k], off, 64);
+    if (lane == 0) {
+#pragma unroll
+      for (int k = 0; k < PW; ++k) {
+        const int sl = wave + k * (BLOCK / 64);
+        if (sl < NS) s_g[sl] = a0[k];
+      }
+    }
+  }
+  __syncthreads();
+  if (f.sums) {
+    if (threadIdx.x < NS) f.sums[threadIdx.x] = s_g[threadIdx.x];
+    return;
+  }
+  guess_decide(s_g, f);
+}
+
 template <int KH>
-__global__ __launch_bounds__(BLOCK) void k_rhs_init_c(i64 n, int scheme, const double* z,
+__device__ inline double guess_corr(const double* cj, const double* yv, double yh) {
+  double corr = 0.0;
+#pragma unroll
+  for (int j = 0; j < KH; ++j) corr += cj[j] * (yv[j] - yh);
+  return corr;
+}
+
+constexpr bool rhs_fuses(int KH, bool DEFER) { return KH >= 2 && DEFER; }
+constexpr int FIT_PARTS = 5, FIT_PER = (GUESS_NS + FIT_PARTS - 1) / FIT_PARTS;
+
+template <int KH, int PART>
+__device__ inline void guess_fit_part(i64 n, int scheme, const double* z, const double* yhat, const double* ds, const double* mass,
+                                      const double* bconst, const unsigned char* fixed, const unsigned char* isblk, const int* cmap,
+                                      const BlkTables& bt, const GuessArgs& g, const GuessFit& f, int bid, int G, const double (&cj)[KH],
+                                      const int (&sel)[KH], int ku, int nld, double (*s_w)[GUESS_NS]) {
+  constexpr int RM = GUESS_RM, NS = GUESS_NS, PER = FIT_PER, T0 = PART * PER, T1 = T0 + PER < NS ? T0 + PER : NS;
+  constexpr bool NEED_RU = T1 > RM * (RM + 1) / 2, NEED_RA = T1 == NS;
+  double gs[PER];
+#pragma unroll
+  for (int k = 0; k < PER; ++k) gs[k] = 0.0;
+  const i64 nchunk = (n + BLOCK - 1) / BLOCK;
+  for (i64 ch = (i64)bid * f.stride; ch < nchunk; ch += (i64)G * f.stride) {
+    const i64 i = ch * BLOCK + threadIdx.x;
+    if (i >= n) continue;
+    const int c = cmap[i];
+    const double d = ds[i], y0 = yhat[i];
+    double zi = 0.0, ms = 0.0, bc = 0.0;
+    bool fx = false, bk = false;
+    if (NEED_RU) { zi = z[i]; ms = mass[i]; bc = bconst[i]; fx = fixed[i] != 0; bk = isblk[i] != 0; }
+    double yr[RM];
+#pragma unroll
+    for (int j = 0; j < RM; ++j) yr[j] = j < nld ? g.yr[j][i] : 0.0;
+    if (c < 0) continue;
+    const double w = d * d;
+    double bi, ru = 0.0, ra = 0.0;
+    if (NEED_RU) rhs_init_one(scheme, zi, y0, d, ms, bc, fx, bk, bk ? rhs_block_row(bt.pos[i], scheme, bt, z, yhat) : 0.0, bi, ru);
+    if (NEED_RA) {
+      double yv[KH];
+#pragma unroll
+      for (int j = 0; j < KH; ++j) {
+        double v = yr[0];
+#pragma unroll
+        for (int q = 1; q < RM; ++q) v = sel[j] == q ? yr[q] : v;
+        yv[j] = j < ku ? v : y0;
+      }
+      ra = ru - guess_corr<KH>(cj, yv, y0);
+    }
+    double q[RM];
+#pragma unroll
+    for (int j = 0; j < RM; ++j) q[j] = j < f.avail ? yr[j] - y0 : 0.0;
+    int t = 0;
+#pragma unroll
+    for (int j = 0; j < RM; ++j)
+#pragma unroll
+      for (int l = j; l < RM; ++l, ++t)
+        if (t >= T0 && t < T1) gs[t - T0] += w * q[j] * q[l];
+#pragma unroll
+    for (int j = 0; j < RM; ++j, ++t)
+      if (t >= T0 && t < T1) gs[t - T0] += w * q[j] * ru;
+    if (t >= T0 && t < T1) gs[t - T0] += w * ru * ru;
+    ++t;
+    if (t >= T0 && t < T1) gs[t - T0] += w * ra * ra;
+  }
+#pragma unroll
+  for (int off = 32; off > 0; off >>= 1)
+#pragma unroll
+    for (int k = 0; k < PER; ++k) gs[k] += __shfl_down(gs[k], off, 64);
+  if ((threadIdx.x & 63) == 0) {
+#pragma unroll
+    for (int k = 0; k < PER; ++k)
+      if (T0 + k < T1) s_w[threadIdx.x >> 6][T0 + k] = gs[k];
+  }
+}
+
+template <int KH>
+__device__ inline void guess_fit_rows(i64 n, int scheme, const double* z, const double* yhat, const double* ds, const double* mass,
+                                      const double* bconst, const unsigned char* fixed, const unsigned char* isblk, const int* cmap,
+                                      const BlkTables& bt, const GuessArgs& g, const GuessFit& f, int bid, int part, int G,
+                                      double* s_red) {
+  constexpr int NS = GUESS_NS, RM = GUESS_RM;
+  __shared__ double s_g[NS];
+  __shared__ double s_w[BLOCK / 64][NS];
+  double cj[KH];
+  int sel[KH];
+  const int ku = min(KH, (int)g.coef[4]);
+  int nld = f.avail;
+#pragma unroll
+  for (int j = 0; j < KH; ++j) {
+    sel[j] = j < ku ? (int)g.coef[5 + j] : 0;
+    cj[j] = j < ku ? g.coef[j] : 0.0;
+    if (j < ku) nld = max(nld, sel[j] + 1);
+  }
+  nld = min(nld, RM);
+#define PG_FIT_PART(P) guess_fit_part<KH, P>(n, scheme, z, yhat, ds, mass, bconst, fixed, isblk, cmap, bt, g, f, bid, G, cj, sel, ku, nld, s_w)
+  static_assert(FIT_PARTS == 5, "guess_fit_rows: one case per group of sums");
+  switch (part) {
+    case 0: PG_FIT_PART(0); break;
+    case 1: PG_FIT_PART(1); break;
+    case 2: PG_FIT_PART(2); break;
+    case 3: PG_FIT_PART(3); break;
+    default: PG_FIT_PART(4); break;
+  }
+#undef PG_FIT_PART
+  __syncthreads();
+  const int t0 = part * FIT_PER;
+  if ((int)threadIdx.x >= t0 && (int)threadIdx.x < min(t0 + FIT_PER, NS)) {
+    double a = 0.0;
+#pragma unroll
+    for (int q = 0; q < BLOCK / 64; ++q) a += s_w[q][threadIdx.x];
+    pg::store_partial(f.partials + (size_t)threadIdx.x * G + bid, a);
+  }
+  if (!pg::last_block_arrives(f.ticket, (unsigned)(FIT_PARTS * G), s_red)) return;
+  guess_fit_last(f, G, s_g);
+}
+
+template <int KH, bool DEFER>
+__global__ __launch_bounds__(BLOCK, (rhs_fuses(KH, DEFER) ? 5 : 1)) void k_rhs_init_c(i64 n, int scheme, const double* z,
                                                       const double* __restrict__ yhat, const double* __restrict__ ds,
                                                       const double* __restrict__ mass, const double* __restrict__ bconst,
                                                       const unsigned char* __restrict__ fixed,
@@ -454,15 +719,23 @@
                                                       double* __restrict__ delta, int* __restrict__ flag, int stamp,
                                                       double* __restrict__ rhat, double* __restrict__ partials,
                                                       unsigned* __restrict__ ticket, double* __restrict__ sc, double reltol2,
-                                                      double abstol2, int coupled, GuessArgs g) {
+                                                      double abstol2, int coupled, GuessArgs g, BlkTables bt, GuessFit gf,
+                                                      int main_grid) {
   __shared__ double s_red[BLOCK / 64];
+  const unsigned G0 = main_grid > 0 ? (unsigned)main_grid : gridDim.x;
+  if (KH > 0 && blockIdx.x >= G0) {
+    if constexpr (rhs_fuses(KH, DEFER))
+      guess_fit_rows<KH>(n, scheme, z, yhat, ds, mass, bconst, fixed, isblk, cmap, bt, g, gf, (int)((blockIdx.x - G0) % gf.nblocks),
+                         (int)((blockIdx.x - G0) / gf.nblocks), gf.nblocks, s_red);
+    return;
+  }
   double acc = 0.0, accb = 0.0, accw = 0.0, acch = 0.0;
   const bool hold = ticket != nullptr;
   double cj[KH > 0 ? KH : 1];
   const double* zo[KH > 0 ? KH : 1];
   const double* yo[KH > 0 ? KH : 1];
   int ku = 0;
-  const bool defer = KH > 0 && g.defer != 0;
+  constexpr bool defer = KH > 0 && DEFER;
   if (KH > 0) {
     ku = min(KH, (int)g.coef[4]);
 #pragma unroll
@@ -472,7 +745,7 @@
       zo[j] = ring_pick(g.zr, sel);
       yo[j] = ring_pick(g.yr, sel);
     }
-    if (defer && blockIdx.x == 0 && threadIdx.x < 9) g.coef[GUESS_USED + threadIdx.x] = g.coef[threadIdx.x];
+    if (defer && g.used && blockIdx.x == 0 && threadIdx.x < 9) g.used[threadIdx.x] = g.coef[threadIdx.x];
   }
   int moved = 0;
   double* zw = KH > 0 ? g.znew : const_cast<double*>(z);
@@ -483,13 +756,10 @@
     accb += (d * bi) * (d * bi);
     if (c >= 0) {
       if (KH > 0) {
-        double zg = zi, corr = 0.0;
-#pragma unroll
-        for (int j = 0; j < KH; ++j) {
-          corr += cj[j] * (yv[j] - yh);
-          zg += cj[j] * (zh[j] - zi);
-        }
-        ri -= corr;
+        double zg = zi;
+#pragma unroll
+        for (int j = 0; j < KH; ++j) zg += cj[j] * (zh[j] - zi);
+        ri -= guess_corr<KH>(cj, yv, yh);
         if (!defer) zw[i] = zg;
       }
       rhat[c] = ri;
@@ -509,7 +779,7 @@
     }
   };
   const i64 npair = (n + 1) / 2;
-  for (i64 q = blockIdx.x * (i64)BLOCK + threadIdx.x; q < npair; q += (i64)gridDim.x * BLOCK) {
+  for (i64 q = blockIdx.x * (i64)BLOCK + threadIdx.x; q < npair; q += (i64)G0 * BLOCK) {
     const i64 i = 2 * q;
     double zh0[KH > 0 ? KH : 1], zh1[KH > 0 ? KH : 1], yv0[KH > 0 ? KH : 1], yv1[KH > 0 ? KH : 1];
     if (i + 1 < n) {
@@ -521,6 +791,9 @@
       const ruc2_t fx = *reinterpret_cast<const ruc2_t*>(fixed + i);
       const ruc2_t bk = *reinterpret_cast<const ruc2_t*>(isblk + i);
       const int c0 = cmap[i], c1 = cmap[i + 1];
+      rd2_t bold;
+      bold.x = 0.0; bold.y = 0.0;
+      if (bk.x | bk.y) bold = *reinterpret_cast<const rd2_t*>(b + i);
       if (KH > 0) {
 #pragma unroll
         for (int j = 0; j < KH; ++j) {
@@ -532,9 +805,6 @@
           zh0[j] = a.x; zh1[j] = a.y; yv0[j] = y2.x; yv1[j] = y2.y;
         }
       }
-      rd2_t bold;
-      bold.x = 0.0; bold.y = 0.0;
-      if (bk.x | bk.y) bold = *reinterpret_cast<const rd2_t*>(b + i);
       rd2_t bi;
       double b0, b1;
       one(i, zz.x, yh.x, d.x, ms.x, bc.x, fx.x != 0, bk.x != 0, bold.x, c0, b0, zh0, yv0);
@@ -562,25 +832,25 @@
   if (!ticket) {
     if (threadIdx.x == 0) {
       partials[blockIdx.x] = t;
-      partials[gridDim.x + blockIdx.x] = tb;
-      partials[2 * (size_t)gridDim.x + blockIdx.x] = tw;
-      if (KH > 0 && blockIdx.x == 0) g.coef[13] += (double)ku;
+      partials[G0 + blockIdx.x] = tb;
+      partials[2 * (size_t)G0 + blockIdx.x] = tw;
+      if (KH > 0 && blockIdx.x == 0) *g.count += (double)ku;
     }
     return;
   }
   if (threadIdx.x == 0) {
     pg::store_partial(partials + blockIdx.x, t);
-    pg::store_partial(partials + gridDim.x + blockIdx.x, tb);
-    pg::store_partial(partials + 2 * (size_t)gridDim.x + blockIdx.x, tw);
+    pg::store_partial(partials + G0 + blockIdx.x, tb);
+    pg::store_partial(partials + 2 * (size_t)G0 + blockIdx.x, tw);
   }
   const double th = block_sum(acch, s_red);
-  if (threadIdx.x == 0) pg::store_partial(partials + 3 * (size_t)gridDim.x + blockIdx.x, th);
-  if (!pg::last_block_arrives(ticket, gridDim.x, s_red)) return;
+  if (threadIdx.x == 0) pg::store_partial(partials + 3 * (size_t)G0 + blockIdx.x, th);
+  if (!pg::last_block_arrives(ticket, G0, s_red)) return;
   if (threadIdx.x < pg::S_COUNT) sc[threadIdx.x] = threadIdx.x == pg::S_RELTOL2 ? reltol2 : (threadIdx.x == pg::S_ABSTOL2 ? abstol2 : 0.0);
   __syncthreads();
   for (int sl = 0; sl < 4; ++sl) {
     double a = 0.0;
-    for (int i = threadIdx.x; i < (int)gridDim.x; i += BLOCK) a += pg::load_partial(partials + (size_t)sl * gridDim.x + i);
+    for (int i = threadIdx.x; i < (int)G0; i += BLOCK) a += pg::load_partial(partials + (size_t)sl * G0 + i);
     const double sum = block_sum(a, s_red);
     if (threadIdx.x == 0) sc[pg::S_RED0 + sl] = sum;
   }
@@ -596,108 +866,7 @@
         sc[pg::S_DONE] = sc[pg::S_RR] <= sc[pg::S_TOL2] ? 1.0 : 0.0;
       }
     }
-    if (KH > 0) g.coef[13] += (double)ku;
-  }
-}
-
-constexpr int GUESS_RM = 7;
-constexpr int GUESS_NS = GUESS_RM * (GUESS_RM + 1) / 2 + GUESS_RM + 2;
-struct GuessFit {
-  const double* yr[8];
-  double* partials;
-  unsigned* ticket;
-  double* coef;
-  int stride, avail, kmax;
-  double rate2, pass_cost, gain;
-  double* sums;
-};
-
-__device__ inline int guess_tri(int j, int l) { return j * GUESS_RM - j * (j - 1) / 2 + (l - j); }
-
-__device__ inline void guess_decide(const double* s_g, const GuessFit& f) {
-  constexpr int RM = GUESS_RM, NS = GUESS_NS;
-  __shared__ double s_left[128], s_net[128];
-  __shared__ double s_c[128][4];
-  const double ru = s_g[NS - 2], rw = s_g[NS - 1];
-  if (threadIdx.x < 128) {
-    const int mask = threadIdx.x, m = __popc(mask);
-    double left = ru, cc[4] = {0.0, 0.0, 0.0, 0.0};
-    if (mask != 0 && m <= f.kmax && m <= 4 && (mask >> f.avail) == 0 && ru > 0.0) {
-      int idx[4] = {0, 0, 0, 0};
-      for (int j = 0, a = 0; j < RM; ++j) if (mask >> j & 1) { if (a < 4) idx[a] = j; ++a; }
-      double L[4][4], wv[4];
-      bool ok = true;
-#pragma unroll
-      for (int a = 0; a < 4; ++a) {
-        wv[a] = 0.0;
-#pragma unroll
-        for (int e = 0; e < 4; ++e) L[a][e] = 0.0;
-      }
-#pragma unroll
-      for (int a = 0; a < 4; ++a) {
-        if (a >= m || !ok) continue;
-        const double g0 = s_g[guess_tri(idx[a], idx[a])];
-        double dj = g0;
-#pragma unroll
-        for (int e = 0; e < 4; ++e) if (e < a) dj -= L[a][e] * L[a][e];
-        if (!(g0 > 0.0) || !(dj > 1e-12 * g0)) { ok = false; continue; }
-        const double lj = sqrt(dj);
-        L[a][a] = lj;
-#pragma unroll
-        for (int l = 0; l < 4; ++l) {
-          if (l <= a || l >= m) continue;
-          double v = s_g[guess_tri(idx[a], idx[l])];
-#pragma unroll
-          for (int e = 0; e < 4; ++e) if (e < a) v -= L[l][e] * L[a][e];
-          L[l][a] = v / lj;
-        }
-        double v = s_g[RM * (RM + 1) / 2 + idx[a]];
-#pragma unroll
-        for (int e = 0; e < 4; ++e) if (e < a) v -= L[a][e] * wv[e];
-        wv[a] = v / lj;
-        left -= wv[a] * wv[a];
-      }
-      if (ok) {
-#pragma unroll
-        for (int aa = 0; aa < 4; ++aa) {
-          const int a = 3 - aa;
-          if (a >= m) continue;
-          double v = wv[a];
-#pragma unroll
-          for (int e = 0; e < 4; ++e) if (e > a && e < m) v -= L[e][a] * cc[e];
-          cc[a] = v / L[a][a];
-        }
-#pragma unroll
-        for (int a = 0; a < 4; ++a) ok = ok && isfinite(cc[a]) && fabs(cc[a]) < 256.0;
-      }
-      if (!ok) { left = ru; cc[0] = cc[1] = cc[2] = cc[3] = 0.0; }
-      if (!(left > 1e-30 * ru)) left = 1e-30 * ru;
-    }
-    s_left[threadIdx.x] = left;
-#pragma unroll
-    for (int a = 0; a < 4; ++a) s_c[threadIdx.x][a] = cc[a];
-    const bool live = ru > 0.0 && f.rate2 > 0.0 && rw <= ru * (1.0 + 1e-12) && left < ru;
-    s_net[threadIdx.x] = live ? f.gain * log(ru / left) / f.rate2 - 2.0 * m * f.pass_cost : 0.0;
-  }
-  __syncthreads();
-  if (threadIdx.x < 64) {
-    int pick = threadIdx.x;
-    double best = s_net[pick];
-    if (s_net[pick + 64] > best) { best = s_net[pick + 64]; pick += 64; }
-#pragma unroll
-    for (int off = 32; off > 0; off >>= 1) {
-      const double ob = __shfl_down(best, off, 64);
-      const int op = __shfl_down(pick, off, 64);
-      if (ob > best || (ob == best && op < pick)) { best = ob; pick = op; }
-    }
-    if (!(best > 0.0)) pick = 0;
-    if (threadIdx.x != 0) return;
-    int a = 0;
-    for (int j = 0; j < RM; ++j)
-      if (pick >> j & 1) { f.coef[a] = s_c[pick][a]; f.coef[5 + a] = (double)j; ++a; }
-    f.coef[4] = (double)a;
-    for (; a < 4; ++a) { f.coef[a] = 0.0; f.coef[5 + a] = 0.0; }
-    f.coef[9] = ru; f.coef[10] = rw; f.coef[11] = pick ? s_left[pick] : ru;
+    if (KH > 0) *g.count += (double)ku;
   }
 }
 
@@ -749,36 +918,7 @@
     }
   }
   if (!pg::last_block_arrives(f.ticket, gridDim.x, s_red)) return;
-  {
-    constexpr int PW = (NS + BLOCK / 64 - 1) / (BLOCK / 64);
-    const int lane = threadIdx.x & 63, wave = threadIdx.x >> 6, G = (int)gridDim.x;
-    double a0[PW], a1[PW];
-#pragma unroll
-    for (int k = 0; k < PW; ++k) {
-      const int sl = wave + k * (BLOCK / 64);
-      a0[k] = (sl < NS && lane < G) ? pg::load_partial(f.partials + (size_t)sl * G + lane) : 0.0;
-      a1[k] = (sl < NS && lane + 64 < G) ? pg::load_partial(f.partials + (size_t)sl * G + lane + 64) : 0.0;
-    }
-#pragma unroll
-    for (int k = 0; k < PW; ++k) a0[k] += a1[k];
-#pragma unroll
-    for (int off = 32; off > 0; off >>= 1)
-#pragma unroll
-      for (int k = 0; k < PW; ++k) a0[k] += __shfl_down(a0[k], off, 64);
-    if (lane == 0) {
-#pragma unroll
-      for (int k = 0; k < PW; ++k) {
-        const int sl = wave + k * (BLOCK / 64);
-        if (sl < NS) s_g[sl] = a0[k];
-      }
-    }
-  }
-  __syncthreads();
-  if (f.sums) {
-    if (threadIdx.x < NS) f.sums[threadIdx.x] = s_g[threadIdx.x];
-    return;
-  }
-  guess_decide(s_g, f);
+  guess_fit_last(f, (int)gridDim.x, s_g);
 }
 
 __global__ __launch_bounds__(BLOCK) void k_guess_decide(GuessFit f) {
@@ -1743,9 +1883,13 @@
   int KH = 0, R = 0, hist_had = 0;
   bool refit = true;
   GuessArgs ga{};
+  bool fit_due() const { return KH > 0 && hist_had > 0 && refit; }
 };
 
-GuessPlan guess_prepare(pg_solver* s, const void* owner, bool allowed, double last_products, hipStream_t stream) {
+inline double* guess_block(pg_solver* s) { return s->guess_coef.p + (s->guess_buf ? GUESS_USED : 0); }
+
+GuessPlan guess_prepare(pg_solver* s, const void* owner, bool allowed, double last_products, hipStream_t stream,
+                        bool two_blocks = false) {
   const Config& cfg = config();
   GuessPlan gp;
   gp.refit = last_products > 4.0 || s->steps_done % 8 == 0;
@@ -1754,6 +1898,7 @@
   gp.hist_had = (s->hist_de == owner && s->hist_k == gp.R) ? s->hist_cnt : 0;
   s->hist_cnt = 0;
   if (gp.KH == 0) return gp;
+  if (!two_blocks && s->guess_buf != 0) gp.hist_had = 0;
   const int R = gp.R;
   const i64 nva = s->z.n;
   if (s->guess_coef.n == 0) { s->guess_coef.alloc(GUESS_USED + 16); s->guess_coef.zero(); s->guess_ticket.alloc(1); s->guess_ticket.zero(); }
@@ -1761,35 +1906,49 @@
     if (j < R && s->zh[j].n != nva) { s->zh[j].alloc(nva); s->zh[j].zero(); }
     if (s->yh[j].n != nva) { s->yh[j].alloc(nva); s->yh[j].zero(); }
   }
-  if (gp.hist_had == 0) PG_HIP(hipMemsetAsync(s->guess_coef.p, 0, 12 * sizeof(double), stream));
+  if (gp.hist_had == 0) {
+    PG_HIP(hipMemsetAsync(s->guess_coef.p, 0, 12 * sizeof(double), stream));
+    PG_HIP(hipMemsetAsync(s->guess_coef.p + GUESS_USED, 0, 12 * sizeof(double), stream));
+    s->guess_buf = 0;
+  }
   for (int j = 0; j < 8; ++j) { gp.ga.zr[j] = s->zh[std::min(j, R - 1)].p; gp.ga.yr[j] = s->yh[std::min(j, R - 1)].p; }
   gp.ga.znew = s->zh[R - 1].p;
-  gp.ga.coef = s->guess_coef.p;
+  gp.ga.coef = guess_block(s);
+  gp.ga.count = s->guess_coef.p + 13;
+  gp.ga.used = nullptr;
   return gp;
 }
 
-void guess_after_rhs(pg_solver* s, const GuessPlan& gp, i64 n, const int* cmap, const double* ds, const double* rhat, bool single,
-                     KrylovWork& w, hipStream_t stream) {
-  if (gp.KH == 0) return;
+GuessFit guess_fit_args(pg_solver* s, const GuessPlan& gp, i64 n, bool single, const KrylovWork& w, int& gfit) {
   const Config& cfg = config();
   const int R = gp.R;
-  if (gp.hist_had > 0 && gp.refit) {
-    GuessFit gf{};
-    for (int j = 0; j < 8; ++j) gf.yr[j] = s->yh[std::min(j, R - 1)].p;
-    const i64 nchunk = (n + BLOCK - 1) / BLOCK;
-    gf.stride = (int)std::max<i64>(1, std::min<i64>(cfg.guess_monitor, nchunk / 128));
-    const int gfit = (int)std::min<i64>(128, (nchunk + gf.stride - 1) / gf.stride);
-    if (s->guess_partials.n != (i64)GUESS_NS * std::max(gfit, 1)) s->guess_partials.alloc((i64)GUESS_NS * std::max(gfit, 1));
-    gf.partials = s->guess_partials.p;
-    gf.ticket = s->guess_ticket.p;
-    gf.coef = s->guess_coef.p;
-    gf.avail = std::min(gp.hist_had, GUESS_RM);
-    gf.kmax = gp.KH;
-    gf.rate2 = w.last_rate2;
-    gf.pass_cost = cfg.guess_pass_cost;
-    gf.gain = cfg.guess_gain;
-    gf.sums = single ? nullptr : s->guess_coef.p + 16;
-    hipLaunchKernelGGL(k_guess_fit, dim3(std::max(gfit, 1)), dim3(BLOCK), 0, stream, n, cmap, ds, (const double*)s->b.p,
+  GuessFit gf{};
+  for (int j = 0; j < 8; ++j) gf.yr[j] = s->yh[std::min(j, R - 1)].p;
+  const i64 nchunk = (n + BLOCK - 1) / BLOCK;
+  gf.stride = (int)std::max<i64>(1, std::min<i64>(cfg.guess_monitor, nchunk / 128));
+  gfit = std::max((int)std::min<i64>(128, (nchunk + gf.stride - 1) / gf.stride), 1);
+  if (s->guess_partials.n != (i64)GUESS_NS * gfit) s->guess_partials.alloc((i64)GUESS_NS * gfit);
+  gf.partials = s->guess_partials.p;
+  gf.ticket = s->guess_ticket.p;
+  gf.coef = guess_block(s);
+  gf.avail = std::min(gp.hist_had, GUESS_RM);
+  gf.kmax = gp.KH;
+  gf.rate2 = w.last_rate2;
+  gf.pass_cost = cfg.guess_pass_cost;
+  gf.gain = cfg.guess_gain;
+  gf.sums = single ? nullptr : s->guess_coef.p + 16;
+  gf.nblocks = gfit;
+  return gf;
+}
+
+void guess_after_rhs(pg_solver* s, const GuessPlan& gp, i64 n, const int* cmap, const double* ds, const double* rhat, bool single,
+                     KrylovWork& w, hipStream_t stream, bool fit_done = false) {
+  if (gp.KH == 0) return;
+  const int R = gp.R;
+  if (gp.fit_due() && !fit_done) {
+    int gfit = 0;
+    const GuessFit gf = guess_fit_args(s, gp, n, single, w, gfit);
+    hipLaunchKernelGGL(k_guess_fit, dim3(gfit), dim3(BLOCK), 0, stream, n, cmap, ds, (const double*)s->b.p,
                        (const double*)s->y.p, rhat, gf);
     if (!single) {
       comm_allreduce_sum_f64(gf.sums, GUESS_NS, stream);
@@ -1810,7 +1969,7 @@
   if (gp.KH == 0) return;
   if (config().debug) {
     double hc[16];
-    s->guess_coef.download(hc, 16);
+    s->guess_coef.download(hc, 16, s->guess_buf ? GUESS_USED : 0);
     fprintf(stderr, "[pg_solver] extrapolated start: %d older states kept; sampled (r,r)_W plain %.3e, taken %.3e; next step: %d states",
             gp.hist_had, hc[9], hc[10], (int)hc[4]);
     for (int j = 0; j < (int)hc[4]; ++j) fprintf(stderr, " z(n-%d)*%.4f", (int)hc[5 + j] + 1, hc[j]);
@@ -1825,6 +1984,29 @@
   hipLaunchKernelGGL(k_rhs_block_mf, dim3(grid_for(A.n_blk, BLOCK)), dim3(BLOCK), 0, stream, make_params(s, scheme), make_segs(s->nb),
                      s->Mloc, A.n_blk, A.blk_rows.p, A.blk_idx.p, A.blk_coef.p, s->nb.row_cell.p, s->nb.red.p, A.ds.p,
                      (const double*)s->z.p, s->mass.p, s->bconst.p, s->fixed.p, s->b.p);
+}
+
+bool rhs_block_cached(pg_solver* s, int scheme, const CsrMatrix& A) {
+  hipStream_t stream = ctx().stream;
+  const bool blk_mf = s->nphase == 2 && scheme == PG_SCHEME_CN;
+  if (A.n_blk <= 0 || blk_mf) return false;
+  if (s->blk_cache_matrix != &A || s->blk_cache_scheme != scheme || s->blk_cache_version != s->bconst_version) {
+    if (s->blk_wz.n != A.n_blk * MAX_KINDS) s->blk_wz.alloc(A.n_blk * MAX_KINDS);
+    if (s->blk_c0.n != A.n_blk) s->blk_c0.alloc(A.n_blk);
+    hipLaunchKernelGGL(k_blk_cache, dim3(grid_for(A.n_blk, BLOCK)), dim3(BLOCK), 0, stream, A.n_blk, scheme, A.blk_idx.p,
+                       A.blk_coef.p, A.ds.p, s->mass.p, s->bconst.p, s->fixed.p, s->blk_wz.p, s->blk_c0.p);
+    s->blk_cache_matrix = &A; s->blk_cache_scheme = scheme; s->blk_cache_version = s->bconst_version;
+  }
+  return true;
+}
+
+void launch_rhs_block(pg_solver* s, int scheme, const CsrMatrix& A, hipStream_t stream) {
+  if (A.n_blk <= 0) return;
+  if (rhs_block_cached(s, scheme, A))
+    hipLaunchKernelGGL(k_rhs_block_c, dim3(grid_for(A.n_blk, BLOCK)), dim3(BLOCK), 0, stream, A.n_blk, scheme, A.blk_rows.p,
+                       BlkTables{A.blk_idx.p, s->blk_wz.p, s->blk_c0.p, A.blk_cn.p, nullptr}, (const double*)s->z.p,
+                       (const double*)s->y.p, s->b.p);
+  else launch_rhs_block_mf(s, scheme, A, stream);
 }
 
 void step_compact(pg_solver* s, int scheme, const pg_krylov_opts& o, const CsrMatrix& A, DiagElim& DE, const DiagElim*& used_de,
@@ -1837,28 +2019,40 @@
   const bool same_data = DE.snapped_version == s->bconst_version;
   const bool quiet = same_data && single;
   guess_policy(DE.guess_on, DE.last_products, DE.bytes_per_rank);
-  GuessPlan gp = guess_prepare(s, &DE, same_data && DE.guess_on, DE.last_products, stream);
+  const Config& cfg = config();
+  const bool fuse_mode = cfg.step_fuse && single && !(A.n_blk > 0 && s->nphase == 2 && scheme == PG_SCHEME_CN);
+  GuessPlan gp = guess_prepare(s, &DE, same_data && DE.guess_on, DE.last_products, stream, fuse_mode);
   const int KH = gp.KH;
-  const Config& cfg = config();
   const bool defer = KH > 0 && cfg.guess_defer && DE.last_products > 0.0;
   gp.ga.defer = defer ? 1 : 0;
+  const bool fit_rides = fuse_mode && rhs_fuses(KH, defer);
+  const bool fit_fused = fit_rides && gp.fit_due();
+  const BlkTables bt{A.blk_idx.p, s->blk_wz.p, s->blk_c0.p, A.blk_cn.p, A.n_blk > 0 ? A.blk_pos.p : nullptr};
+  int gfit = 0;
+  GuessFit gf{};
+  if (fit_fused) {
+    gf = guess_fit_args(s, gp, n, true, w, gfit);
+    s->guess_buf ^= 1;
+    gf.coef = guess_block(s);
+  }
+  gp.ga.used = (defer && !fit_rides) ? s->guess_coef.p + GUESS_USED : nullptr;
   const GuessArgs& ga = gp.ga;
   const double* zprev = s->z.p;
-#define PG_RHS_INIT_C(KHV)                                                                                                        \
-  hipLaunchKernelGGL(HIP_KERNEL_NAME(k_rhs_init_c<KHV>), dim3(w.grid), dim3(BLOCK), 0, stream, n, scheme, s->z.p, s->y.p, A.ds.p,   \
+#define PG_RHS_INIT_C(KHV, DF)                                                                                                    \
+  hipLaunchKernelGGL(HIP_KERNEL_NAME(k_rhs_init_c<KHV, DF>), dim3(w.grid + gfit * FIT_PARTS), dim3(BLOCK), 0, stream, n, scheme, s->z.p, s->y.p, A.ds.p, \
                      s->mass.p, s->bconst.p, s->fixed.p, A.isblk.p, DE.cmap.p, s->b.p, (const double*)DE.gdiag.p, DE.delta.p,     \
                      DE.flag.p, stamp, w.rhat.p, w.partials.p, quiet ? w.ticket.p : nullptr, w.sc.p, o.reltol * o.reltol,          \
-                     o.abstol * o.abstol, same_data ? 0 : 1, ga)
+                     o.abstol * o.abstol, same_data ? 0 : 1, ga, bt, gf, w.grid)
   switch (KH) {
-    case 1: PG_RHS_INIT_C(1); break;
-    case 2: PG_RHS_INIT_C(2); break;
-    case 3: PG_RHS_INIT_C(3); break;
-    case 4: PG_RHS_INIT_C(4); break;
-    default: PG_RHS_INIT_C(0); break;
+    case 1: if (defer) PG_RHS_INIT_C(1, true); else PG_RHS_INIT_C(1, false); break;
+    case 2: if (defer) PG_RHS_INIT_C(2, true); else PG_RHS_INIT_C(2, false); break;
+    case 3: if (defer) PG_RHS_INIT_C(3, true); else PG_RHS_INIT_C(3, false); break;
+    case 4: if (defer) PG_RHS_INIT_C(4, true); else PG_RHS_INIT_C(4, false); break;
+    default: PG_RHS_INIT_C(0, false); break;
   }
 #undef PG_RHS_INIT_C
   PG_HIP(hipGetLastError());
-  guess_after_rhs(s, gp, n, (const int*)DE.cmap.p, (const double*)A.ds.p, (const double*)w.rhat.p, single, w, stream);
+  guess_after_rhs(s, gp, n, (const int*)DE.cmap.p, (const double*)A.ds.p, (const double*)w.rhat.p, single, w, stream, fit_fused);
   if (!same_data) diag_fix(DE, s->nb, s->slab, stamp, !single, w.rhat.p, w.partials.p, w.grid, stream);
   KrylovCall call;
   call.preinit = call.p_in_rhat = true;
@@ -1877,7 +2071,7 @@
   if (defer) {
     call.xguess.zbase = zprev;
     for (int j = 0; j < 8; ++j) call.xguess.zr[j] = ga.zr[j];
-    call.xguess.coef = s->guess_coef.p + GUESS_USED;
+    call.xguess.coef = ga.used ? ga.used : ga.coef;
   }
   krylov_solve(DE.A, DE.nb, s->slab, nullptr, s->z.p, w, o, st, call);
   s->spec_y_valid = s->spec_pending && st.polls == 1 && st.converged && st.poly_degree >= 0;
@@ -2024,20 +2218,7 @@
     const bool have_y = s->spec_y_valid && s->spec_matrix == &A;
     s->spec_y_valid = false;
     if (!have_y) spmv_halo(A, s->nb, s->slab, s->z.p, s->y.p, stream);
-    const bool blk_mf = s->nphase == 2 && scheme == PG_SCHEME_CN;
-    if (A.n_blk > 0 && blk_mf) launch_rhs_block_mf(s, scheme, A, stream);
-    else if (A.n_blk > 0) {
-      if (s->blk_cache_matrix != &A || s->blk_cache_scheme != scheme || s->blk_cache_version != s->bconst_version) {
-        if (s->blk_wz.n != A.n_blk * MAX_KINDS) s->blk_wz.alloc(A.n_blk * MAX_KINDS);
-        if (s->blk_c0.n != A.n_blk) s->blk_c0.alloc(A.n_blk);
-        hipLaunchKernelGGL(k_blk_cache, dim3(grid_for(A.n_blk, BLOCK)), dim3(BLOCK), 0, stream, A.n_blk, scheme, A.blk_idx.p,
-                           A.blk_coef.p, A.ds.p, s->mass.p, s->bconst.p, s->fixed.p, s->blk_wz.p, s->blk_c0.p);
-        s->blk_cache_matrix = &A; s->blk_cache_scheme = scheme; s->blk_cache_version = s->bconst_version;
-      }
-      hipLaunchKernelGGL(k_rhs_block_c, dim3(grid_for(A.n_blk, BLOCK)), dim3(BLOCK), 0, stream, A.n_blk, scheme, A.blk_rows.p,
-                         A.blk_idx.p, (const double*)s->blk_wz.p, (const double*)s->blk_c0.p, A.blk_cn.p, (const double*)s->z.p,
-                         (const double*)s->y.p, s->b.p);
-    }
+    launch_rhs_block(s, scheme, A, stream);
     DiagElim& DE = (&A == &s->A_ctor) ? s->diag_ctor : s->diag_run;
     if (!mgs && !DE.tried) build_diag_elim(A, s->nb, s->slab, DE);
     if (!mgs && DE.active && krylov_uses_polynomial(DE.A, o)) step_compact(s, scheme, o, A, DE, used_de, st);
@@ -3511,7 +3692,7 @@
   for (int j = 0; j < 4; ++j) { offsets[j] = 0; coef[j] = 0.0; }
   if (s->guess_coef.n >= 16 && s->hist_cnt > 0) {
     double hc[16];
-    s->guess_coef.download(hc, 16);
+    s->guess_coef.download(hc, 16, s->guess_buf ? GUESS_USED : 0);
     *nstates = (int32_t)hc[4];
     for (int j = 0; j < *nstates && j < 4; ++j) { offsets[j] = (int32_t)hc[5 + j] + 1; coef[j] = hc[j]; }
     *rr_plain = hc[9];
diff --git a/penguin/jl_amd/csrc/pg_system.h b/penguin/jl_amd/csrc/pg_system.h
--- a/penguin/jl_amd/csrc/pg_system.h
+++ b/penguin/jl_amd/csrc/pg_system.h
@@ -73,6 +73,7 @@
   DevBuf<int> blk_rows, blk_idx;
   DevBuf<double> blk_coef, blk_cn, blk_fw;
   DevBuf<unsigned char> isblk;
+  DevBuf<int> blk_pos;
 };
 inline void poly_record_stagnation(const CsrMatrix& A) {
   CsrMatrix& M = const_cast<CsrMatrix&>(A);
```

Result: faster. 1367, median of 6 (+1.6%).
